# ArbiterMob/FluidSimulationCuda

Measured on AMD Instinct MI355X. Metric: Mcells/s per Jacobi iter, higher is better.
Workload: dtype f32

## Files before the change

fluidsimulationcuda_amd/capi.py:

```python
import ctypes as C
import os

import numpy as np

from ._build import LIB

OK, E_INVALID, E_NOMEM, E_HIP, E_COMM = 0, 1, 2, 3, 4
U, V, DENS, U_PREV, V_PREV, DENS_PREV, TMP0, TMP1, TMP2, TMP3, TMP4, TMP5 = range(12)
NFIELDS = 12
JACOBI_STREAM, JACOBI_LDS, JACOBI_NAIVE, JACOBI_TB = 0, 1, 2, 3
STORAGE_F32, STORAGE_F16 = 0, 1
PARAM_TB_MAX_SWEEPS, PARAM_TB_ROWS, PARAM_HALO, PARAM_TB_FAST_DIVISION, PARAM_TB_MIN_CELLS, PARAM_TB_EDGE_ROWS_PCT = 0, 1, 2, 3, 4, 5
PARAM_TB_LANE_COLUMNS = 6
PARAM_TB_T16_MIN_CELLS = 7
PARAM_TB_AUTOTUNE = 8
PARAM_FUSE_DIVERGENCE = 9
PARAM_SLAB_OVERLAP = 10
PARAM_EARLY_ADVECT = 11
PARAM_FUSE_ADD_SOURCE = 12
PARAM_XCHG_OVERLAP = 13
PARAM_F16_PRESSURE_SCALE = 14
PARAM_TB_FILL = 15
XCHG_HALO, XCHG_GATHER, XCHG_MAX, XCHG_MAX_BEGIN, XCHG_MAX_END = 0, 1, 2, 3, 4
RCCL_ID_BYTES = 128
FIELD_NAMES = ("u", "v", "dens", "u_prev", "v_prev", "dens_prev", "tmp0", "tmp1", "tmp2", "tmp3", "tmp4", "tmp5")


class FluidError(RuntimeError):
    def __init__(self, code, msg):
        super().__init__("libfluid_amd error %d: %s" % (code, msg))
        self.code = code


class Config(C.Structure):
    _fields_ = [("n", C.c_int), ("rank", C.c_int), ("nranks", C.c_int), ("halo", C.c_int),
                ("jacobi_variant", C.c_int), ("stream", C.c_void_p), ("arena", C.c_void_p),
                ("arena_bytes", C.c_size_t), ("storage", C.c_int)]


TIME_SOURCE, TIME_DIFFUSION, TIME_DIVERGENCE, TIME_PROJECTION, TIME_ADVECTION = range(5)
TIMING_CATEGORIES = ("source", "diffusion", "divergence", "projection", "advection")


class Timing(C.Structure):
    _fields_ = [("jacobi_ms", C.c_double), ("sweeps", C.c_longlong), ("solves", C.c_longlong),
                ("category_ms", C.c_double * 5), ("category_calls", C.c_longlong * 5),
                ("jacobi_launches", C.c_longlong), ("jacobi_field_launches", C.c_longlong),
                ("pressure_ms", C.c_double), ("pressure_sweeps", C.c_longlong)]


class RunPlan(C.Structure):
    _fields_ = [("iters", C.c_int), ("nsteps", C.c_int), ("use_sources", C.c_int), ("sources", C.c_void_p),
                ("every", C.c_int), ("fields", C.POINTER(C.c_int)), ("nfields", C.c_int),
                ("snapshots", C.c_void_p), ("capacity", C.c_size_t)]


EXCHANGE_FN = C.CFUNCTYPE(C.c_int, C.c_void_p, C.c_int, C.POINTER(C.c_int), C.c_int, C.c_int,
                          C.POINTER(C.c_float))

_HOSTF = np.ctypeslib.ndpointer(dtype=np.float32, flags="C_CONTIGUOUS")
_ctx = C.c_void_p
_i, _f = C.c_int, C.c_float
_MF = C.POINTER(C.c_float)

SIGNATURES = {
    "step": [_i, _f, _f, _f, _HOSTF, _HOSTF, _HOSTF],
    "step_src": [_i, _f, _f, _f, _i] + [_HOSTF] * 6,
    "fluid_release_cached": [],
    "fluid_coefficients": [_i, _f, _f, C.POINTER(_f), C.POINTER(_f)],
    "fluid_layout": [_i, C.POINTER(_i), C.POINTER(_i), C.POINTER(C.c_size_t)],
    "fluid_create": [_i, C.POINTER(_ctx)],
    "fluid_create_ex": [C.POINTER(Config), C.POINTER(_ctx)],
    "fluid_create_ensemble": [C.POINTER(Config), _i, C.POINTER(_ctx)],
    "fluid_members": [_ctx, C.POINTER(_i)],
    "fluid_upload_member": [_ctx, _i, _i, _HOSTF],
    "fluid_download_member": [_ctx, _i, _i, _HOSTF],
    "fluid_step_members": [_ctx, _MF, _MF, _MF, _i, _i, _i],
    "fluid_vel_step_members": [_ctx, _MF, _MF, _i],
    "fluid_dens_step_members": [_ctx, _MF, _MF, _i],
    "fluid_op_add_source_members": [_ctx, _i, _i, _MF],
    "fluid_op_jacobi_sweep_members": [_ctx, _i, _i, _i, _i, _MF, _MF],
    "fluid_op_diffuse_members": [_ctx, _i, _i, _i, _MF, _MF, _i],
    "fluid_op_advect_members": [_ctx, _i, _i, _i, _i, _i, _MF],
    "fluid_destroy": [_ctx],
    "fluid_synchronize": [_ctx],
    "fluid_owned_rows": [_ctx, C.POINTER(_i), C.POINTER(_i)],
    "fluid_field_ptr": [_ctx, _i, C.POINTER(C.c_void_p)],
    "fluid_scalar_ptr": [_ctx, C.POINTER(C.c_void_p)],
    "fluid_upload": [_ctx, _i, _HOSTF],
    "fluid_download": [_ctx, _i, _HOSTF],
    "fluid_upload_rows": [_ctx, _i, _HOSTF, _i, _i],
    "fluid_download_rows": [_ctx, _i, _HOSTF, _i, _i],
    "fluid_fill": [_ctx, _i, _f],
    "fluid_step": [_ctx, _f, _f, _f, _i, _i, _i],
    "fluid_vel_step": [_ctx, _f, _f, _i],
    "fluid_dens_step": [_ctx, _f, _f, _i],
    "fluid_op_set_bnd": [_ctx, _i, _i],
    "fluid_op_add_source": [_ctx, _i, _i, _f],
    "fluid_op_jacobi_sweep": [_ctx, _i, _i, _i, _i, _f, _f],
    "fluid_op_diffuse": [_ctx, _i, _i, _i, _f, _f, _i],
    "fluid_op_advect": [_ctx, _i, _i, _i, _i, _i, _f],
    "fluid_op_divergence": [_ctx, _i, _i, _i, _i],
    "fluid_op_subtract_gradient": [_ctx, _i, _i, _i],
    "fluid_residual": [_ctx, _i, _i, _f, _f, C.POINTER(_f)],
    "fluid_absmax_velocity": [_ctx, _i, _i, C.POINTER(_f)],
    "fluid_residual_members": [_ctx, _i, _i, _MF, _MF, _MF],
    "fluid_absmax_velocity_members": [_ctx, _i, _i, _MF],
    "fluid_member_moments": [_ctx, _i, C.POINTER(C.c_double), C.POINTER(C.c_double)],
    "fluid_ensemble_stats": [_ctx, _i, _MF, _MF],
    "fluid_ensemble_stats_ptr": [_ctx, C.POINTER(C.c_void_p), C.POINTER(C.c_void_p)],
    "fluid_pack_members": [_ctx, _i, _i, _i, C.c_void_p, C.c_size_t],
    "fluid_unpack_members": [_ctx, _i, _i, _i, C.c_void_p, C.c_size_t],
    "fluid_download_members": [_ctx, _i, _MF],
    "fluid_upload_members": [_ctx, _i, _MF],
    "fluid_run": [_ctx, _f, _f, _f, C.POINTER(RunPlan), C.POINTER(_i)],
    "fluid_run_members": [_ctx, _MF, _MF, _MF, C.POINTER(RunPlan), C.POINTER(_i)],
    "fluid_set_jacobi_variant": [_ctx, _i],
    "fluid_division_mode": [_ctx, _f, _f, C.POINTER(_i)],
    "fluid_autotune_pending": [_ctx, C.POINTER(_i)],
    "fluid_plan_sweeps": [_i, _i, _i, _i, _i, _i, _i, C.POINTER(_i), _i, C.POINTER(_i)],
    "fluid_set_param": [_ctx, _i, _i],
    "fluid_timing_enable": [_ctx, _i],
    "fluid_timing_read": [_ctx, C.POINTER(Timing), _i],
    "fluid_op_diffuse_tol": [_ctx, _i, _i, _i, _f, _f, _f, _i, _i, C.POINTER(_i), C.POINTER(_f)],
    "fluid_set_exchange": [_ctx, EXCHANGE_FN, C.c_void_p],
    "fluid_exchange_now": [_ctx, _i, C.POINTER(_i), _i, _i],
    "fluid_exchange_stream": [_ctx, C.POINTER(C.c_void_p)],
    "fluid_split_launches": [_ctx, C.POINTER(C.c_longlong)],
    "fluid_rccl_available": [],
    "fluid_rccl_unique_id": [C.c_void_p, C.c_size_t],
    "fluid_exchange_rccl_attach": [_ctx, C.c_void_p, C.c_size_t],
    "fluid_exchange_rccl_attach_comm": [_ctx, C.c_void_p],
    "fluid_exchange_rccl_detach": [_ctx],
    "fluid_exchange_rccl_calls": [_ctx, C.POINTER(C.c_longlong), C.POINTER(C.c_longlong), C.POINTER(C.c_longlong)],
}
OTHER_SYMBOLS = {"fluid_last_error": (C.c_char_p, []), "fluid_arena_bytes": (C.c_size_t, [_i]),
                 "fluid_arena_bytes_ex": (C.c_size_t, [_i, _i]),
                 "fluid_arena_bytes_ensemble": (C.c_size_t, [_i, _i, _i])}
MAX_MEMBERS = 21845

_lib = None


def lib():
    global _lib
    if _lib is None:
        if not os.path.exists(LIB):
            raise ImportError("%s not found: run `python -c 'import __graft_entry__ as g; g.build()'` "
                              "(hipcc --offload-arch=gfx950). There is no CPU fallback." % LIB)
        try:
            import torch
        except ImportError:
            pass
        L = C.CDLL(LIB)
        for name, args in SIGNATURES.items():
            fn = getattr(L, name)
            fn.restype, fn.argtypes = C.c_int, args
        for name, (res, args) in OTHER_SYMBOLS.items():
            fn = getattr(L, name)
            fn.restype, fn.argtypes = res, args
        _lib = L
    return _lib


def check(rc):
    if rc != OK:
        raise FluidError(rc, lib().fluid_last_error().decode(errors="replace"))
```

fluidsimulationcuda_amd/csrc/fluid_ctx.h:

```cpp
#pragma once
#include <hip/hip_runtime.h>

#include <string>
#include <utility>
#include <vector>

#include "../../include/fluid_amd.h"
#include "fluid_kernels.h"

namespace fluid_detail {
int fail(int code, const char* fmt, ...);
int materialize_zero(fluid_ctx* c, int f);
int refuse_ensemble(const fluid_ctx* c, const char* what);
struct RcclExchange;
void rccl_release(RcclExchange* x);
}

#define HIP_TRY(expr)                                                                                      \
    do {                                                                                                   \
        hipError_t e_ = (expr);                                                                            \
        if (e_ != hipSuccess)                                                                              \
            return fluid_detail::fail(e_ == hipErrorOutOfMemory ? FLUID_E_NOMEM : FLUID_E_HIP, "%s: %s",   \
                                      #expr, hipGetErrorString(e_));                                       \
    } while (0)

#define TRY(expr)                        \
    do {                                 \
        int rc_ = (expr);                \
        if (rc_ != FLUID_OK) return rc_; \
    } while (0)

class MemberVal {
    float s_;
    std::vector<float> v_;
    explicit MemberVal(std::vector<float>&& v) : s_(v[0]), v_(std::move(v)) {}

public:
    MemberVal(float v = 0.0f) : s_(v) {}
    MemberVal(const float* per_member, int members) : s_(per_member[0]), v_(per_member, per_member + members) {}
    bool uniform() const { return v_.empty(); }
    float at(int m) const { return v_.empty() ? s_ : v_[(size_t)m]; }
    const std::vector<float>& values() const { return v_; }
    bool operator==(const MemberVal& o) const { return s_ == o.s_ && v_ == o.v_; }
    template <class F>
    MemberVal map(const MemberVal& b, F f) const
    {
        if (uniform() && b.uniform()) return MemberVal(f(s_, b.s_));
        std::vector<float> r(uniform() ? b.v_.size() : v_.size());
        for (size_t m = 0; m < r.size(); ++m) r[m] = f(at((int)m), b.at((int)m));
        return MemberVal(std::move(r));
    }
    template <class F>
    MemberVal map(F f) const { return map(MemberVal(), [&](float x, float) { return f(x); }); }
};

struct FieldState {
    void* ptr = nullptr;
    int reach = 0;
    bool zero = false;
    bool pend = false;
    MemberVal pend_inc;
    int src_of = 0;
    MemberVal src_dt;
    float fscale = 1.0f;
};

struct ConstRing {
    char *dev = nullptr, *host = nullptr;
    size_t bytes = 0, head = 0;
    struct Blob { size_t off, len; unsigned long long hash; hipEvent_t copied; };
    std::vector<Blob> live;
    std::vector<hipEvent_t> free_events;
};

struct EnsembleReduce {
    unsigned int* d_max = nullptr;
    double2* d_moments = nullptr;
    double2* d_partials = nullptr;
    char* host = nullptr;
    float *d_mean = nullptr, *d_var = nullptr;
    bool have_stats = false;
};

struct MemberStage {
    float* dev = nullptr;
    int members = 0;
};

struct fluid_ctx {
    int n = 0, w = 0, pitch = 0;
    size_t field_floats = 0;
    int members = 1;
    char* arena = nullptr;
    bool own_arena = false;
    int st = fluid::STORAGE_F32;
    size_t esz = 4;
    hipStream_t stream = nullptr;
    bool own_stream = false;
    hipStream_t stream2 = nullptr;
    hipEvent_t ev_fork = nullptr, ev_join = nullptr;
    bool slab_overlap = true;
    hipStream_t xstream = nullptr;
    hipEvent_t ev_xbegin = nullptr, ev_xdone = nullptr;
    bool xchg_overlap = true;
    unsigned xowed = 0;
    long long split_launches = 0;
    bool early_advect = true;
    float vmax_prev[2] = {-1.0f, -1.0f};
    FieldState field[FLUID_NFIELDS];
    size_t field_bytes = 0;
    unsigned int* d_scalar = nullptr;
    float* d_partials = nullptr;
    ConstRing consts;
    EnsembleReduce red;
    MemberStage stage;
    unsigned int* tiles = nullptr;
    unsigned int* h_scalar = nullptr;
    hipEvent_t scalar_ready = nullptr;
    int variant = fluid::JACOBI_TB;
    int tb_max_t = 16, tb_rows = 0, num_cu = 256;
    long long tb_min_cells = 0;
    long long tb_t16_min_cells = -1;
    bool fuse_divergence = true;
    bool tb_fill = true;
    bool autotune = true;
    struct Trial { unsigned long long key; int cand; hipEvent_t a, b; };
    std::vector<Trial> trials;
    std::vector<hipEvent_t> free_events;
    bool defer_zero_source = true;
    bool in_halo_exchange = false;
    int tb_nv = 2;
    int tb_edge_pct = 40;
    int fast_div = 2;
    int rank = 0, nranks = 1, own0 = 1, own1 = 1, min_slab = 0, halo = 1;
    bool fuse_add_source = true;
    float pscale = 1.0f;
    fluid_exchange_fn xchg = nullptr;
    void* xchg_user = nullptr;
    fluid_detail::RcclExchange* rccl = nullptr;
    bool timing = false;
    struct Ev { hipEvent_t a, b; int cat; bool pressure; };
    std::vector<Ev> ev_pool;
    size_t ev_used = 0;
    double cat_ms[FLUID_TIMING_CATEGORIES] = {};
    long long cat_calls[FLUID_TIMING_CATEGORIES] = {};
    long long sweeps = 0, pending_sweeps = 0, launches = 0, field_launches = 0;
    double pressure_ms = 0.0;
    long long pressure_sweeps = 0, pending_pressure_sweeps = 0;
    bool in_pressure_solve = false;

    bool valid_field(int id) const { return id >= 0 && id < FLUID_NFIELDS; }
    void* ptr(int id) const { return field[id].ptr; }
    fluid::Members mb() const { return {members, field_floats}; }
    size_t all_bytes() const { return field_bytes * (size_t)members; }
    void* row(int id, int r) const { return static_cast<char*>(ptr(id)) + (size_t)r * pitch * esz; }
    int lo_all() const { return own0 - (rank == 0 ? 1 : 0); }
    int hi_all() const { return own1 + (rank == nranks - 1 ? 1 : 0); }
};
```

fluidsimulationcuda_amd/csrc/fluid_kernels.h:

```cpp
#pragma once
#include <hip/hip_runtime.h>

namespace fluid {

constexpr int XOFF = 63;

enum JacobiVariant { JACOBI_STREAM = 0, JACOBI_LDS = 1, JACOBI_NAIVE = 2, JACOBI_TB = 3, JACOBI_VARIANTS = 4 };

enum Storage { STORAGE_F32 = 0, STORAGE_F16 = 1 };
typedef _Float16 half_t;
inline size_t storage_bytes(int st) { return st == STORAGE_F16 ? 2 : 4; }

inline int pitch_for(int n) { return ((XOFF + 1 + 4 * ((n + 3) / 4) + 1) + 63) / 64 * 64; }

struct Members {
    int count = 1;
    size_t stride = 0;
};

struct TbMemberK {
    double yd;
    float alpha, beta, hi, lo;
    float x0_inc, div_scale;
    unsigned tile_thr, pad;
};

struct TbBatch {
    const void* x[3];
    const void* x0[3];
    void* out[3];
    float alpha[3], beta[3];
    double yd[3];
    float hi[3], lo[3];
    const unsigned* tiles[3];
    unsigned tile_thr[3];
    int tile_pitch;
    void* div[3];
    float div_scale;
    int b[3];
    int x_zero[3];
    float x0_inc[3];
    int count;
    int members;
    size_t mstride;
    size_t tile_mstride;
    const TbMemberK* mk;
};

void launch_set_bnd(hipStream_t s, int st, void* f, int pitch, int n, int b, Members mb = {});
void launch_add_source(hipStream_t s, int st, void* x, const void* src, int pitch, int row_lo, int row_hi, float dt, Members mb = {},
                       const float* mdt = nullptr);
void launch_jacobi(hipStream_t s, int st, int variant, const void* x, const void* x0, void* out, int pitch, int n,
                   int row_lo, int row_hi, float alpha, float beta, int b, Members mb = {}, const float2* mab = nullptr);
enum TbForm { TB_PLAIN = 0, TB_DIVSRC = 1, TB_ADDSRC = 2 };
struct TbShape { int T, divmode, nv, form; };
inline constexpr TbShape kTbShapes[] = {
    {2, 0, 2, TB_PLAIN},   {2, 2, 2, TB_PLAIN},   {2, 3, 2, TB_PLAIN},   {2, 4, 2, TB_PLAIN},   {2, 5, 2, TB_PLAIN},
    {2, 0, 4, TB_PLAIN},   {2, 2, 4, TB_PLAIN},   {2, 3, 4, TB_PLAIN},   {2, 4, 4, TB_PLAIN},   {2, 5, 4, TB_PLAIN},
    {4, 0, 2, TB_PLAIN},   {4, 2, 2, TB_PLAIN},   {4, 3, 2, TB_PLAIN},   {4, 4, 2, TB_PLAIN},   {4, 5, 2, TB_PLAIN},
    {4, 0, 4, TB_PLAIN},   {4, 2, 4, TB_PLAIN},   {4, 3, 4, TB_PLAIN},   {4, 4, 4, TB_PLAIN},   {4, 5, 4, TB_PLAIN},
    {8, 0, 2, TB_PLAIN},   {8, 2, 2, TB_PLAIN},   {8, 3, 2, TB_PLAIN},   {8, 4, 2, TB_PLAIN},   {8, 5, 2, TB_PLAIN},
    {8, 0, 4, TB_PLAIN},   {8, 2, 4, TB_PLAIN},   {8, 3, 4, TB_PLAIN},   {8, 4, 4, TB_PLAIN},   {8, 5, 4, TB_PLAIN},
    {12, 0, 2, TB_PLAIN},  {12, 2, 2, TB_PLAIN},  {12, 3, 2, TB_PLAIN},  {12, 4, 2, TB_PLAIN},  {12, 5, 2, TB_PLAIN},
    {16, 0, 2, TB_PLAIN},  {16, 2, 2, TB_PLAIN},  {16, 3, 2, TB_PLAIN},  {16, 4, 2, TB_PLAIN},  {16, 5, 2, TB_PLAIN},
    {8, 4, 2, TB_DIVSRC},  {12, 4, 2, TB_DIVSRC}, {16, 4, 2, TB_DIVSRC}, {8, 0, 2, TB_ADDSRC},  {8, 2, 2, TB_ADDSRC},  {8, 5, 2, TB_ADDSRC},
    {12, 0, 2, TB_ADDSRC}, {12, 2, 2, TB_ADDSRC}, {12, 5, 2, TB_ADDSRC}, {16, 0, 2, TB_ADDSRC}, {16, 2, 2, TB_ADDSRC}, {16, 5, 2, TB_ADDSRC},
};
constexpr int kTbShapeCount = sizeof(kTbShapes) / sizeof(kTbShapes[0]);
constexpr int jacobi_tb_index(int T, int divmode, int nv, int form)
{
    for (int i = 0; i < kTbShapeCount; ++i) {
        const TbShape& s = kTbShapes[i];
        if ((T < 0 || s.T == T) && (divmode < 0 || s.divmode == divmode) && s.nv == nv && s.form == form) return i;
    }
    return -1;
}
constexpr bool jacobi_tb_exists(int T, int divmode, int nv, int form) { return jacobi_tb_index(T, divmode, nv, form) >= 0; }
constexpr bool tb_shapes_unique(int i = 0)
{
    return i == kTbShapeCount || (jacobi_tb_index(kTbShapes[i].T, kTbShapes[i].divmode, kTbShapes[i].nv, kTbShapes[i].form) == i && tb_shapes_unique(i + 1));
}
static_assert(kTbShapeCount == 52 && tb_shapes_unique(), "52 distinct shapes: adding or removing one is a change of this table");
inline constexpr int kTbDepths[] = {16, 12, 8, 4, 2};
constexpr bool is_tb_depth(int T) { for (int d : kTbDepths) if (d == T) return true; return false; }
bool launch_jacobi_tb(hipStream_t s, int st, int T, int divmode, int nv, int form, const TbBatch& batch, int pitch, int n, int row_lo,
                      int row_hi, int rb, int rb_edge, int hole_lo = 0, int hole_hi = 0, bool fill = true);
constexpr int kTileRows = 32, kTileCols = 64;
inline int tile_rows(int n) { return (n + kTileRows - 1) / kTileRows; }
inline int tile_pitch(int n) { return (n + kTileCols - 1) / kTileCols; }
struct TileBatch {
    const void* field[3];
    unsigned* tiles[3];
    int count;
    size_t mstride, tile_mstride;
};
void launch_tile_min_abs(hipStream_t s, int st, const TileBatch& tb, int count, int pitch, int n, int row_lo, int row_hi, int tile_pitch,
                         Members mb = {}, size_t tile_mstride = 0);
void launch_validate_div(hipStream_t s, int divmode, float beta, float kbeta, double yd, float hi, float lo, unsigned long long* bad);
void launch_advect(hipStream_t s, int st, void* d, const void* d0, const void* u, const void* v, int pitch, int n,
                   int row_lo, int row_hi, float dt0, int b, Members mb = {}, const float* mdt0 = nullptr);
void launch_advect2(hipStream_t s, int st, void* da, const void* d0a, int ba, void* db, const void* d0b, int bb, const void* u,
                    const void* v, int pitch, int n, int row_lo, int row_hi, float dt0, Members mb = {}, const float* mdt0 = nullptr);
void launch_divergence(hipStream_t s, int st, const void* u, const void* v, void* p, void* div, int pitch, int n,
                       int row_lo, int row_hi, float h, int write_p, float pscale = 1.0f, Members mb = {});
void launch_scale(hipStream_t s, int st, void* x, int pitch, int row_lo, int row_hi, float factor, Members mb = {});
constexpr int kMaxPartials = 8192;
void launch_subtract_gradient(hipStream_t s, int st, void* u, void* v, const void* p, int pitch, int n, int row_lo,
                              int row_hi, float h, float* partials = nullptr, unsigned int* max_out = nullptr, float pinv = 1.0f,
                              Members mb = {});
void launch_gradient_advect(hipStream_t s, int st, void* u, void* v, const void* p, void* d, const void* d0, int pitch, int n,
                            int row_lo, int row_hi, float h, float dt0, int b, float pinv = 1.0f, Members mb = {},
                            const float* mdt0 = nullptr);
void launch_absmax2(hipStream_t s, int st, const void* u, const void* v, int pitch, int n, int row_lo, int row_hi,
                    unsigned int* result, Members mb = {}, int rstride = 0);
void launch_residual(hipStream_t s, int st, const void* x, const void* x0, int pitch, int n, int row_lo, int row_hi,
                     float alpha, float beta, unsigned int* result, Members mb = {}, int rstride = 0, const float2* mab = nullptr);
constexpr int kMomentBlocks = 4096;
int moment_blocks(int n, int members);
void launch_member_moments(hipStream_t s, int st, const void* x, int pitch, int n, Members mb, double2* partials, double2* out);
void launch_ensemble_stats(hipStream_t s, int st, const void* x, int pitch, int n, Members mb, float* mean, float* var);
void launch_pack_members(hipStream_t s, int st, const void* x, int pitch, int n, Members mb, float inv, float* dense, size_t dstride);
void launch_unpack_members(hipStream_t s, int st, void* x, int pitch, int n, Members mb, const float* dense, size_t dstride);

}
```

fluidsimulationcuda_amd/csrc/fluid_kernels.hip:

```cpp
#include <hip/hip_runtime.h>
#include <stdint.h>

#include <algorithm>
#include <array>
#include <cstdlib>
#include <utility>

#include "fluid_kernels.h"

namespace fluid {

__device__ __forceinline__ float flip_if(bool c, float v) { return c ? -v : v; }

__device__ __forceinline__ float keep_f32(float v) { asm("" : "+v"(v)); return v; }
__device__ __forceinline__ float ld1(const float* p) { return *p; }
__device__ __forceinline__ float ld1(const half_t* p) { return keep_f32((float)*p); }
__device__ __forceinline__ void st1(float* p, float v) { *p = v; }
__device__ __forceinline__ void st1(half_t* p, float v) { *p = (half_t)keep_f32(v); }
template <typename S>
__device__ __forceinline__ float as_stored(float v)
{
    if constexpr (sizeof(S) == 2) return keep_f32((float)(S)keep_f32(v));
    else return v;
}
typedef half_t half4_t __attribute__((ext_vector_type(4)));
__device__ __forceinline__ float4 ld4(const float* p) { return *reinterpret_cast<const float4*>(p); }
__device__ __forceinline__ float4 ld4(const half_t* p)
{
    const half4_t h = *reinterpret_cast<const half4_t*>(p);
    return make_float4(keep_f32((float)h.x), keep_f32((float)h.y), keep_f32((float)h.z), keep_f32((float)h.w));
}
__device__ __forceinline__ void st4(float* p, const float4& v) { *reinterpret_cast<float4*>(p) = v; }
__device__ __forceinline__ void st4(half_t* p, const float4& v)
{
    half4_t h;
    h.x = (half_t)keep_f32(v.x); h.y = (half_t)keep_f32(v.y); h.z = (half_t)keep_f32(v.z); h.w = (half_t)keep_f32(v.w);
    *reinterpret_cast<half4_t*>(p) = h;
}

constexpr unsigned kBufOff = 0x80000000u;
typedef unsigned uint4_t __attribute__((ext_vector_type(4)));
typedef unsigned uint2_t __attribute__((ext_vector_type(2)));

__device__ __forceinline__ float from_lane_below(float v, float edge)
{
    int r = __builtin_amdgcn_update_dpp(__float_as_int(edge), __float_as_int(v),
                                        0x138 , 0xf, 0xf, false);
    return __int_as_float(r);
}
__device__ __forceinline__ float from_lane_above(float v, float edge)
{
    int r = __builtin_amdgcn_update_dpp(__float_as_int(edge), __float_as_int(v),
                                        0x130 , 0xf, 0xf, false);
    return __int_as_float(r);
}

__device__ __forceinline__ float lane_below0(float v)
{
    return __int_as_float(__builtin_amdgcn_update_dpp(0, __float_as_int(v), 0x138, 0xf, 0xf, true));
}
__device__ __forceinline__ float lane_above0(float v)
{
    return __int_as_float(__builtin_amdgcn_update_dpp(0, __float_as_int(v), 0x130, 0xf, 0xf, true));
}

template <typename S>
__device__ __forceinline__ void emit_ghosts(S* __restrict__ f, size_t pitch, int n, int b, int j, int i, float val)
{
    const bool nx = (b == 1), ny = (b == 2);
    const bool left = (j == 1), right = (j == n), top = (i == 1), bot = (i == n);
    if (!(left | right | top | bot)) return;
    const float gx = flip_if(nx, val);
    const float gy = flip_if(ny, val);
    const float corner = 0.5f * (gy + gx);
    S* r0 = f + XOFF;
    S* ri = f + (size_t)i * pitch + XOFF;
    S* rn = f + (size_t)(n + 1) * pitch + XOFF;
    if (left) st1(ri, gx);
    if (right) st1(ri + n + 1, gx);
    if (top) st1(r0 + j, gy);
    if (bot) st1(rn + j, gy);
    if (top & left) st1(r0, corner);
    if (top & right) st1(r0 + n + 1, corner);
    if (bot & left) st1(rn, corner);
    if (bot & right) st1(rn + n + 1, corner);
}

template <typename S>
__global__ __launch_bounds__(256) void k_set_bnd(S* __restrict__ f, int pitch, int n, int b, size_t ms)
{
    const int k = 1 + blockIdx.x * 256 + threadIdx.x;
    if (k > n) return;
    f += blockIdx.y * ms;
    const size_t P = (size_t)pitch;
    const bool nx = (b == 1), ny = (b == 2);
    S* r0 = f + XOFF;
    S* rk = f + (size_t)k * P + XOFF;
    S* r1 = f + P + XOFF;
    S* rN = f + (size_t)n * P + XOFF;
    S* rn = f + (size_t)(n + 1) * P + XOFF;
    const float gl = flip_if(nx, ld1(rk + 1));
    const float gr = flip_if(nx, ld1(rk + n));
    const float gt = flip_if(ny, ld1(r1 + k));
    const float gb = flip_if(ny, ld1(rN + k));
    st1(rk, gl);
    st1(rk + n + 1, gr);
    st1(r0 + k, gt);
    st1(rn + k, gb);
    if (k == 1) {
        st1(r0, 0.5f * (gt + gl));
        st1(rn, 0.5f * (gb + flip_if(nx, ld1(rN + 1))));
    }
    if (k == n) {
        st1(r0 + n + 1, 0.5f * (gt + flip_if(nx, ld1(r1 + n))));
        st1(rn + n + 1, 0.5f * (gb + gr));
    }
}

template <typename S>
__global__ __launch_bounds__(256) void k_add_source(S* __restrict__ x, const S* __restrict__ s, int pitch, int row_lo,
                                                    int row_hi, float dt, size_t ms, const float* __restrict__ mdt)
{
    if (mdt) dt = mdt[blockIdx.y];
    const int nvec = pitch >> 2;
    const size_t total = (size_t)(row_hi - row_lo) * nvec;
    S* xv = x + blockIdx.y * ms + (size_t)row_lo * pitch;
    const S* sv = s + blockIdx.y * ms + (size_t)row_lo * pitch;
    for (size_t t = (size_t)blockIdx.x * 256 + threadIdx.x; t < total; t += (size_t)gridDim.x * 256) {
        float4 a = ld4(xv + 4 * t);
        const float4 c = ld4(sv + 4 * t);
        a.x = a.x + dt * c.x;
        a.y = a.y + dt * c.y;
        a.z = a.z + dt * c.z;
        a.w = a.w + dt * c.w;
        st4(xv + 4 * t, a);
    }
}

template <typename S>
__global__ __launch_bounds__(256) void k_add_zero_source(S* __restrict__ x, int pitch, int row_lo, int row_hi, float inc, size_t ms,
                                                         const float* __restrict__ minc)
{
    if (minc) inc = minc[blockIdx.y];
    const int nvec = pitch >> 2;
    const size_t total = (size_t)(row_hi - row_lo) * nvec;
    S* xv = x + blockIdx.y * ms + (size_t)row_lo * pitch;
    for (size_t t = (size_t)blockIdx.x * 256 + threadIdx.x; t < total; t += (size_t)gridDim.x * 256) {
        float4 a = ld4(xv + 4 * t);
        a.x = a.x + inc;
        a.y = a.y + inc;
        a.z = a.z + inc;
        a.w = a.w + inc;
        st4(xv + 4 * t, a);
    }
}

template <typename S>
__global__ __launch_bounds__(256) void k_scale(S* __restrict__ x, int pitch, int row_lo, int row_hi, float factor, size_t ms)
{
    const int nvec = pitch >> 2;
    const size_t total = (size_t)(row_hi - row_lo) * nvec;
    S* xv = x + blockIdx.y * ms + (size_t)row_lo * pitch;
    for (size_t t = (size_t)blockIdx.x * 256 + threadIdx.x; t < total; t += (size_t)gridDim.x * 256) {
        float4 a = ld4(xv + 4 * t);
        a.x = a.x * factor;
        a.y = a.y * factor;
        a.z = a.z * factor;
        a.w = a.w * factor;
        st4(xv + 4 * t, a);
    }
}


template <typename S>
__global__ __launch_bounds__(256) void k_jacobi_naive(const S* __restrict__ x, const S* __restrict__ x0,
// ... 164 lines not shown
        const uint4_t u = __builtin_amdgcn_raw_buffer_load_b128(r, off, 0, 0);
        v.c[0] = __uint_as_float(u.x); v.c[1] = __uint_as_float(u.y); v.c[2] = __uint_as_float(u.z); v.c[3] = __uint_as_float(u.w);
    } else {
        const uint2_t u = __builtin_amdgcn_raw_buffer_load_b64(r, off, 0, 0);
        v.c[0] = __uint_as_float(u.x); v.c[1] = __uint_as_float(u.y);
    }
    return v;
}
template <int NV>
__device__ __forceinline__ Vec<NV> buf_ldv(const half_t*, __amdgpu_buffer_rsrc_t r, unsigned off)
{
    Vec<NV> v;
    if constexpr (NV == 4) {
        const uint2_t u = __builtin_amdgcn_raw_buffer_load_b64(r, off, 0, 0);
        half4_t h;
        __builtin_memcpy(&h, &u, 8);
        v.c[0] = keep_f32((float)h.x); v.c[1] = keep_f32((float)h.y); v.c[2] = keep_f32((float)h.z); v.c[3] = keep_f32((float)h.w);
    } else {
        const unsigned u = __builtin_amdgcn_raw_buffer_load_b32(r, off, 0, 0);
        half2_t h;
        __builtin_memcpy(&h, &u, 4);
        v.c[0] = keep_f32((float)h.x); v.c[1] = keep_f32((float)h.y);
    }
    return v;
}
template <int NV>
__device__ __forceinline__ void buf_stv(float*, __amdgpu_buffer_rsrc_t r, unsigned off, const Vec<NV>& v)
{
    if constexpr (NV == 4) {
        uint4_t u;
        u.x = __float_as_uint(v.c[0]); u.y = __float_as_uint(v.c[1]); u.z = __float_as_uint(v.c[2]); u.w = __float_as_uint(v.c[3]);
        __builtin_amdgcn_raw_buffer_store_b128(u, r, off, 0, 0);
    } else {
        uint2_t u;
        u.x = __float_as_uint(v.c[0]); u.y = __float_as_uint(v.c[1]);
        __builtin_amdgcn_raw_buffer_store_b64(u, r, off, 0, 0);
    }
}
template <int NV>
__device__ __forceinline__ void buf_stv(half_t*, __amdgpu_buffer_rsrc_t r, unsigned off, const Vec<NV>& v)
{
    if constexpr (NV == 4) {
        half4_t h;
        h.x = (half_t)keep_f32(v.c[0]); h.y = (half_t)keep_f32(v.c[1]); h.z = (half_t)keep_f32(v.c[2]); h.w = (half_t)keep_f32(v.c[3]);
        uint2_t u;
        __builtin_memcpy(&u, &h, 8);
        __builtin_amdgcn_raw_buffer_store_b64(u, r, off, 0, 0);
    } else {
        half2_t h;
        h.x = (half_t)keep_f32(v.c[0]); h.y = (half_t)keep_f32(v.c[1]);
        unsigned u;
        __builtin_memcpy(&u, &h, 4);
        __builtin_amdgcn_raw_buffer_store_b32(u, r, off, 0, 0);
    }
}

struct DivK {
    float beta;
    double yd;
    float hi, lo;
};
constexpr float kDiv5NegScale = -0x1p24f;

template <typename S, int NV>
struct TbArgs {
    const S* xc;
    const S* rc;
    S* oc;
    __amdgpu_buffer_rsrc_t bx, br, bo;
    unsigned ld_off;
    unsigned st_off;
    unsigned row_bytes;
    unsigned m_lg;
    unsigned m_r[NV];
    int n, q_lo, q_hi, cg;
    float alpha;
    DivK k;
    S* dc;
    __amdgpu_buffer_rsrc_t bd;
    float div_scale;
    int s_lo, s_hi;
    unsigned sx, sy;
    float x0_inc;
    bool st_rg_lane, is_lg;
    bool fill;
};

__device__ __forceinline__ float fxor(float v, unsigned m) { return __uint_as_float(__float_as_uint(v) ^ m); }
template <int NV>
__device__ __forceinline__ Vec<NV> fxorv(const Vec<NV>& v, unsigned m)
{
    Vec<NV> o;
#pragma unroll
    for (int c = 0; c < NV; ++c) o.c[c] = fxor(v.c[c], m);
    return o;
}

template <int DIVMODE>
__device__ __forceinline__ float tb_div(float num, const DivK& k)
{
    if (DIVMODE == 0) return num / k.beta;
    if (DIVMODE == 4) return num * k.beta;
    if (DIVMODE == 3) return __builtin_fmaf(num, k.hi, num * k.lo);
    if (DIVMODE == 5) {
        const float q0 = num * k.beta;
        const float e = __builtin_fmaf(q0, k.hi, num * kDiv5NegScale);
        return __builtin_fmaf(e, k.lo, q0);
    }
    return (float)((double)num * k.yd);
}
template <int DIVMODE>
__device__ __forceinline__ v2f tb_div2(v2f num, const DivK& k)
{
    if constexpr (DIVMODE == 4) return num * k.beta;
    else if constexpr (DIVMODE == 3) {
        const v2f p = num * k.lo;
        return __builtin_elementwise_fma(num, (v2f){k.hi, k.hi}, p);
    } else if constexpr (DIVMODE == 5) {
        const v2f ds = num * kDiv5NegScale;
        const v2f q0 = num * k.beta;
        const v2f e = __builtin_elementwise_fma(q0, (v2f){k.hi, k.hi}, ds);
        return __builtin_elementwise_fma(e, (v2f){k.lo, k.lo}, q0);
    } else return (v2f){tb_div<DIVMODE>(num.x, k), tb_div<DIVMODE>(num.y, k)};
}

template <int DIVMODE, int NV>
__device__ __forceinline__ Vec<NV> tb_stencil(const Vec<NV>& up, const Vec<NV>& me, const Vec<NV>& dn, const Vec<NV>& r,
                                              float alpha, const DivK& k)
{
    float h[NV];
    h[0] = lane_below0(me.c[NV - 1]) + me.c[1];
#pragma unroll
    for (int c = 1; c < NV - 1; ++c) h[c] = me.c[c - 1] + me.c[c + 1];
    h[NV - 1] = me.c[NV - 2] + lane_above0(me.c[0]);
    Vec<NV> G;
#pragma unroll
    for (int p = 0; p < NV; p += 2) {
        v2f s = {h[p], h[p + 1]};
        s = s + (v2f){up.c[p], up.c[p + 1]};
        s = s + (v2f){dn.c[p], dn.c[p + 1]};
        if constexpr (DIVMODE != 4) s = s * alpha;
        s = (v2f){r.c[p], r.c[p + 1]} + s;
        s = tb_div2<DIVMODE>(s, k);
        G.c[p] = s.x;
        G.c[p + 1] = s.y;
    }
    return G;
}

template <int DIVMODE>
__global__ __launch_bounds__(256) void k_validate_div(float beta, DivK k, unsigned long long* __restrict__ bad)
{
    unsigned long long n = 0;
    const unsigned long long stride = (unsigned long long)gridDim.x * 256;
    auto differs = [](float got, float ref) { return (ref != ref) ? !(got != got) : (__float_as_uint(got) != __float_as_uint(ref)); };
    DivK k2 = k;
    for (unsigned long long i = (unsigned long long)blockIdx.x * 256 + threadIdx.x; i < (1ull << 32); i += stride) {
        const float a = __uint_as_float((unsigned)i);
        const float ref = a / beta;
        if constexpr (DIVMODE == 3) {
            const bool in_range = a == 0.0f || !(__builtin_fabsf(a) < beta * 0x1p-98f);
            n += differs(tb_div<2>(a, k2), ref) || (in_range && differs(tb_div<3>(a, k), ref));
        } else if constexpr (DIVMODE == 5) {
            const float got = tb_div<5>(a, k);
            const bool finite = __builtin_fabsf(got) < __builtin_inff();
            const bool must_be_exact = __builtin_fabsf(a) < 0x1p100f;
            n += differs(got, ref) && (finite || must_be_exact);
        } else {
            n += differs(tb_div<DIVMODE>(a, k), ref);
        }
    }
    if (n) atomicAdd(bad, n);
}

__device__ __forceinline__ float bitsel(unsigned mask, float a, float b)
{
    return __uint_as_float((__float_as_uint(a) & mask) | (__float_as_uint(b) & ~mask));
}

template <typename S, int NV>
__device__ __forceinline__ void tb_fix_columns(Vec<NV>& G, const TbArgs<S, NV>& a, float& v1, float& vn, bool need_corners)
{
    float o[NV];
#pragma unroll
    for (int c = 0; c < NV; ++c) o[c] = G.c[c];
    const float from_right = lane_above0(o[0]);
    const float from_left = lane_below0(o[NV - 1]);
    G.c[0] = bitsel(a.m_r[0], fxor(from_left, a.sx), o[0]);
#pragma unroll
    for (int c = 1; c < NV - 1; ++c) G.c[c] = bitsel(a.m_r[c], fxor(o[c - 1], a.sx), o[c]);
    G.c[NV - 1] = bitsel(a.m_lg, fxor(from_right, a.sx), bitsel(a.m_r[NV - 1], fxor(o[NV - 2], a.sx), o[NV - 1]));
    if (need_corners) {
        v1 = from_right;
        unsigned bits = __float_as_uint(from_left) & a.m_r[0];
#pragma unroll
        for (int c = 1; c < NV; ++c) bits |= __float_as_uint(o[c - 1]) & a.m_r[c];
        vn = __uint_as_float(bits);
    }
}

template <bool EDGE, bool WALL, typename S, int NV>
__device__ __forceinline__ void tb_store_to(S* oc, __amdgpu_buffer_rsrc_t bo, const Vec<NV>& G, int q, bool mine, const TbArgs<S, NV>& a,
                                            float v1, float vn)
{
    auto on = [](bool c, unsigned off) { return c ? off : kBufOff; };
    buf_stv<NV>(oc, bo, on(mine, a.st_off) + (unsigned)q * a.row_bytes, G);
    if (WALL) {
        Vec<NV> g = fxorv<NV>(G, a.sy);
        if (EDGE) {
            const float cl = 0.5f * (fxor(v1, a.sy) + fxor(v1, a.sx));
            const float cr = 0.5f * (fxor(vn, a.sy) + fxor(vn, a.sx));
            if (a.is_lg) g.c[NV - 1] = cl;
#pragma unroll
            for (int c = 0; c < NV; ++c)
                if (a.st_rg_lane && a.cg == c) g.c[c] = cr;
        }
        buf_stv<NV>(oc, bo, on(mine & (q == 1), a.st_off), g);
        buf_stv<NV>(oc, bo, on(mine & (q == a.n), a.st_off) + (unsigned)(a.n + 1) * a.row_bytes, g);
    }
}
template <bool EDGE, bool WALL, typename S, int NV>
__device__ __forceinline__ void tb_store(const Vec<NV>& G, int q, bool mine, const TbArgs<S, NV>& a, float v1, float vn)
{
    tb_store_to<EDGE, WALL, S, NV>(a.oc, a.bo, G, q, mine, a, v1, vn);
}

template <int NV>
__device__ __forceinline__ Vec<NV> tb_divergence(const Vec<NV>& u, const Vec<NV>& v_up, const Vec<NV>& v_dn, float scale)
{
    float g[NV];
#pragma unroll
    for (int c = 0; c < NV; ++c) {
        const float ur = c < NV - 1 ? u.c[c + 1] : lane_above0(u.c[0]);
        const float ul = c > 0 ? u.c[c - 1] : lane_below0(u.c[NV - 1]);
        g[c] = ur - ul;
    }
    Vec<NV> d;
#pragma unroll
    for (int p = 0; p < NV; p += 2) {
        v2f s = {g[p], g[p + 1]};
        s = s + (v2f){v_dn.c[p], v_dn.c[p + 1]};
        s = s - (v2f){v_up.c[p], v_up.c[p + 1]};
        s = s * scale;
        d.c[p] = s.x;
        d.c[p + 1] = s.y;
    }
    return d;
}

template <int NV>
__device__ __forceinline__ Vec<NV> take(const Vec<NV>& v)
{
    Vec<NV> o;
#pragma unroll
    for (int p = 0; p < NV; p += 2) {
        v2f in = {v.c[p], v.c[p + 1]}, out;
        asm("v_mov_b64 %0, %1" : "=v"(out) : "v"(in));
        o.c[p] = out.x;
        o.c[p + 1] = out.y;
    }
    return o;
}

template <int K, int N, int NV>
__device__ __forceinline__ void tb_qshift(Vec<NV> (&Q)[N])
{
    if constexpr (K >= 1) {
        Q[K] = Q[K - 1];
        tb_qshift<K - 1, N, NV>(Q);
    }
}

template <int DIVMODE, int NV>
__device__ __forceinline__ void tb_sticky(const Vec<NV>& G, v2f& nf)
{
    if constexpr (DIVMODE == 5) {
#pragma unroll
        for (int p = 0; p < NV; p += 2) nf = __builtin_elementwise_fma((v2f){G.c[p], G.c[p + 1]}, (v2f){0.f, 0.f}, nf);
    }
}

template <int T, int DIVMODE, bool EDGE, bool WALL, bool GEN, int PH, typename S, int NV, bool DIVSRC = false, bool ADDSRC = false,
          bool PART = false>
__device__ __forceinline__ void tb_step(int t, Vec<NV> (&W)[T][3], Vec<NV> (&Q)[T + 1], Vec<NV> (&PX)[3], Vec<NV> (&PQ)[3],
                                        const TbArgs<S, NV>& a, Vec<NV> (&UR)[3], Vec<NV> (&VR)[3], v2f& nf, int smax = T)
{
    static_assert(!(PART && GEN), "the general body runs every stage");
    constexpr int UP = PH % 3, ME = (PH + 1) % 3, FR = (PH + 2) % 3;
    __builtin_amdgcn_sched_barrier(0);
    if constexpr (DIVSRC) {
        UR[FR] = take<NV>(PX[PH]);
        VR[FR] = take<NV>(PQ[PH]);
    } else {
        W[0][FR] = take<NV>(PX[PH]);
        Q[0] = take<NV>(PQ[PH]);
        if constexpr (ADDSRC) {
#pragma unroll
            for (int p = 0; p < NV; p += 2) {
                const v2f ds = (v2f){W[0][FR].c[p], W[0][FR].c[p + 1]} * a.div_scale;
                const v2f q = (v2f){Q[0].c[p], Q[0].c[p + 1]} + ds;
                Q[0].c[p] = as_stored<S>(q.x);
                Q[0].c[p + 1] = as_stored<S>(q.y);
            }
            buf_stv<NV>(a.dc, a.bd, (((t >= a.s_lo) & (t < a.s_hi)) ? a.st_off : kBufOff) + (unsigned)t * a.row_bytes, Q[0]);
        } else {
#pragma unroll
            for (int p = 0; p < NV; p += 2) {
                const v2f q = (v2f){Q[0].c[p], Q[0].c[p + 1]} + a.x0_inc;
                Q[0].c[p] = q.x;
                Q[0].c[p + 1] = q.y;
            }
        }
    }
    {
        const unsigned off = a.ld_off + (unsigned)(t + 3) * a.row_bytes;
        PX[PH] = buf_ldv<NV>(a.xc, a.bx, off);
        PQ[PH] = buf_ldv<NV>(a.rc, a.br, off);
    }
    __builtin_amdgcn_sched_barrier(0);
    if constexpr (DIVSRC) {
        const int q = t - 1;
        Vec<NV> D = tb_divergence<NV>(UR[ME], VR[UP], VR[FR], a.div_scale);
#pragma unroll
        for (int c = 0; c < NV; ++c) D.c[c] = as_stored<S>(D.c[c]);
        Q[1] = D;
        float v1 = 0.f, vn = 0.f;
        if (EDGE) tb_fix_columns<S, NV>(D, a, v1, vn, WALL);
        tb_store_to<EDGE, (WALL || GEN), S, NV>(a.dc, a.bd, D, q, (q >= 1) & (q <= a.n) & (q >= a.q_lo) & (q < a.q_hi), a, v1, vn);
    }
    if constexpr (!GEN) {
#pragma unroll
        for (int s = 1; s <= T; ++s) {
            const bool run = !PART || s <= smax;
            const int q = t - s;
            Vec<NV> G;
            float v1 = 0.f, vn = 0.f;
            if (run) {
                G = tb_stencil<DIVMODE, NV>(W[s - 1][UP], W[s - 1][ME], W[s - 1][FR], Q[s], a.alpha, a.k);
                if (EDGE) tb_fix_columns<S, NV>(G, a, v1, vn, WALL && s == T);
                if (s == T) tb_sticky<DIVMODE, NV>(G, nf);
            } else {
#pragma unroll
                for (int c = 0; c < NV; ++c) G.c[c] = __builtin_nondeterministic_value(W[s - 1][FR].c[c]);
            }
            if (s < T) W[s][FR] = G;
            else tb_store<EDGE, WALL, S, NV>(G, q, run & (q >= a.q_lo) & (q < a.q_hi), a, v1, vn);
        }
    } else {
#pragma unroll
        for (int s = 1; s <= T; ++s) {
            const int q = t - s;
            const bool interior = (q >= 1 && q <= a.n);
            Vec<NV> G = tb_stencil<DIVMODE, NV>(W[s - 1][UP], W[s - 1][ME], W[s - 1][FR], Q[s], a.alpha, a.k);
            float v1 = 0.f, vn = 0.f;
            if (EDGE) tb_fix_columns<S, NV>(G, a, v1, vn, s == T);
            if (s < T) {
                const Vec<NV> me = W[s][ME];
                const Vec<NV> flipped_me = fxorv<NV>(me, a.sy);
                const Vec<NV> flipped_g = fxorv<NV>(G, a.sy);
                const bool bot_ghost = (q == a.n + 1), top_ghost = (q == 1);
#pragma unroll
                for (int c = 0; c < NV; ++c) {
                    W[s][FR].c[c] = bot_ghost ? flipped_me.c[c] : G.c[c];
                    W[s][ME].c[c] = top_ghost ? flipped_g.c[c] : me.c[c];
                }
            } else {
                tb_sticky<DIVMODE, NV>(G, nf);
                tb_store<EDGE, true, S, NV>(G, q, interior & (q >= a.q_lo) & (q < a.q_hi), a, v1, vn);
            }
        }
    }
    tb_qshift<T, T + 1, NV>(Q);
}

template <int T, int DIVMODE, bool EDGE, bool WALL, typename S, int NV, bool DIVSRC = false, bool ADDSRC = false>
__device__ __forceinline__ bool tb_march(int t0, int t1, const TbArgs<S, NV>& a)
{
    Vec<NV> W[T][3], Q[T + 1], PX[3], PQ[3], UR[3], VR[3];
    v2f nf = {0.f, 0.f};
    Vec<NV> zero;
#pragma unroll
    for (int c = 0; c < NV; ++c) zero.c[c] = 0.f;
#pragma unroll
    for (int s = 0; s < T; ++s) { W[s][0] = zero; W[s][1] = zero; W[s][2] = zero; }
#pragma unroll
    for (int s = 0; s <= T; ++s) Q[s] = zero;
#pragma unroll
    for (int d = 0; d < 3; ++d) { UR[d] = zero; VR[d] = zero; }
#pragma unroll
    for (int d = 0; d < 3; ++d) {
        const unsigned off = a.ld_off + (unsigned)(t0 + d) * a.row_bytes;
        PX[d] = buf_ldv<NV>(a.xc, a.bx, off);
        PQ[d] = buf_ldv<NV>(a.rc, a.br, off);
        buf_stv<NV>(a.oc, a.bo, kBufOff, zero);
        if constexpr (DIVSRC || ADDSRC) buf_stv<NV>(a.dc, a.bd, kBufOff, zero);
        __builtin_amdgcn_sched_barrier(0);
    }
    int t = t0;
    if constexpr (WALL) {
        for (; t <= t1 && t < T + 1; t += 3) {
            tb_step<T, DIVMODE, EDGE, WALL, true, 0, S, NV, DIVSRC, ADDSRC>(t, W, Q, PX, PQ, a, UR, VR, nf);
            tb_step<T, DIVMODE, EDGE, WALL, true, 1, S, NV, DIVSRC, ADDSRC>(t + 1, W, Q, PX, PQ, a, UR, VR, nf);
            tb_step<T, DIVMODE, EDGE, WALL, true, 2, S, NV, DIVSRC, ADDSRC>(t + 2, W, Q, PX, PQ, a, UR, VR, nf);
        }
    }
    const int fill_end = (a.fill && t0 == a.q_lo - T) ? t0 + 3 * ((2 * T + 2) / 3) : t0;
    const int full_end = a.fill ? t1 - 2 : t1;
    auto stages = [&](int u) { return u > t1 ? 0 : u < fill_end ? (u - t0) >> 1 : T; };
    for (; t <= t1 && t < fill_end && (!WALL || t + 1 <= a.n); t += 3) {
        tb_step<T, DIVMODE, EDGE, WALL, false, 0, S, NV, DIVSRC, ADDSRC, true>(t, W, Q, PX, PQ, a, UR, VR, nf, stages(t));
        tb_step<T, DIVMODE, EDGE, WALL, false, 1, S, NV, DIVSRC, ADDSRC, true>(t + 1, W, Q, PX, PQ, a, UR, VR, nf, stages(t + 1));
        tb_step<T, DIVMODE, EDGE, WALL, false, 2, S, NV, DIVSRC, ADDSRC, true>(t + 2, W, Q, PX, PQ, a, UR, VR, nf, stages(t + 2));
    }
    for (; t <= full_end && (!WALL || t + 1 <= a.n); t += 3) {
        tb_step<T, DIVMODE, EDGE, WALL, false, 0, S, NV, DIVSRC, ADDSRC>(t, W, Q, PX, PQ, a, UR, VR, nf);
        tb_step<T, DIVMODE, EDGE, WALL, false, 1, S, NV, DIVSRC, ADDSRC>(t + 1, W, Q, PX, PQ, a, UR, VR, nf);
        tb_step<T, DIVMODE, EDGE, WALL, false, 2, S, NV, DIVSRC, ADDSRC>(t + 2, W, Q, PX, PQ, a, UR, VR, nf);
    }
    for (; t <= t1 && (!WALL || t + 1 <= a.n); t += 3) {
        tb_step<T, DIVMODE, EDGE, WALL, false, 0, S, NV, DIVSRC, ADDSRC, true>(t, W, Q, PX, PQ, a, UR, VR, nf, stages(t));
        tb_step<T, DIVMODE, EDGE, WALL, false, 1, S, NV, DIVSRC, ADDSRC, true>(t + 1, W, Q, PX, PQ, a, UR, VR, nf, stages(t + 1));
        tb_step<T, DIVMODE, EDGE, WALL, false, 2, S, NV, DIVSRC, ADDSRC, true>(t + 2, W, Q, PX, PQ, a, UR, VR, nf, stages(t + 2));
    }
    if constexpr (WALL) {
        for (; t <= t1; t += 3) {
            tb_step<T, DIVMODE, EDGE, WALL, true, 0, S, NV, DIVSRC, ADDSRC>(t, W, Q, PX, PQ, a, UR, VR, nf);
            tb_step<T, DIVMODE, EDGE, WALL, true, 1, S, NV, DIVSRC, ADDSRC>(t + 1, W, Q, PX, PQ, a, UR, VR, nf);
            tb_step<T, DIVMODE, EDGE, WALL, true, 2, S, NV, DIVSRC, ADDSRC>(t + 2, W, Q, PX, PQ, a, UR, VR, nf);
        }
    }
    if constexpr (DIVMODE == 5) return __builtin_amdgcn_ballot_w64((nf.x != nf.x) | (nf.y != nf.y)) != 0ull;
    else return false;
}

template <int T, int DIVMODE, typename S, int NV, bool DIVSRC = false, bool ADDSRC = false>
__device__ __forceinline__ bool tb_march_any(bool edge, bool wall, int t0, int t1, const TbArgs<S, NV>& a)
{
    if (edge) {
        if (wall) return tb_march<T, DIVMODE, true, true, S, NV, DIVSRC, ADDSRC>(t0, t1, a);
        return tb_march<T, DIVMODE, true, false, S, NV, DIVSRC, ADDSRC>(t0, t1, a);
    }
    if (wall) return tb_march<T, DIVMODE, false, true, S, NV, DIVSRC, ADDSRC>(t0, t1, a);
    return tb_march<T, DIVMODE, false, false, S, NV, DIVSRC, ADDSRC>(t0, t1, a);
}

struct TbGrid {
    int inner_wins, inner_blocks, edge_wins, edge_blocks, first_right;
    int hole_lo, hole_hi;
};

constexpr int tb_waves_per_simd(int T, int NV) { return NV == 2 ? (T <= 8 ? 4 : T <= 12 ? 3 : 2) : (T <= 4 ? 3 : 2); }

template <int T, int DIVMODE, int NV, typename S, bool DIVSRC = false, bool ADDSRC = false>
__global__ __launch_bounds__(256, tb_waves_per_simd(T, NV)) void k_jacobi_tb(TbBatch batch, int pitch, int n, int row_lo,
                                                                             int row_hi, int rb, int rb_edge, TbGrid g, int fill)
{
    static_assert(!DIVSRC || DIVMODE == 4, "the divergence-sourced launch is the first launch of a pressure solve");
    static_assert(!(DIVSRC && ADDSRC) && (!ADDSRC || DIVMODE != 3), "one second store per launch; mode 3's tiles are taken from the summed field");
    const unsigned per_xcd = gridDim.x >> 3;
    unsigned vid = (blockIdx.x & 7u) * per_xcd + (blockIdx.x >> 3);
    if (vid >= (unsigned)(g.inner_blocks + g.edge_blocks)) return;
    int win, strip_group;
    if (vid < (unsigned)g.inner_blocks) {
        win = 1 + (int)(vid % (unsigned)g.inner_wins);
        strip_group = (int)(vid / (unsigned)g.inner_wins);
    } else {
        vid -= (unsigned)g.inner_blocks;
        const int e = (int)(vid % (unsigned)g.edge_wins);
        strip_group = (int)(vid / (unsigned)g.edge_wins);
        win = e == 0 ? 0 : g.first_right + e - 1;
    }
    const unsigned member = batch.count == 3 ? blockIdx.z / 3u : batch.count == 2 ? blockIdx.z >> 1 : blockIdx.z;
    const unsigned sv = blockIdx.z - member * (unsigned)batch.count;
    const size_t mofs = (size_t)member * batch.mstride;
    const S* __restrict__ x = static_cast<const S*>(batch.x[sv]) + mofs;
    const S* __restrict__ x0 = static_cast<const S*>(batch.x0[sv]) + mofs;
    S* __restrict__ out = static_cast<S*>(batch.out[sv]) + mofs;
    float alpha = batch.alpha[sv], beta = batch.beta[sv];
    double yd = batch.yd[sv];
    float k_hi = batch.hi[sv], k_lo = batch.lo[sv], x0_inc = batch.x0_inc[sv], div_scale = batch.div_scale;
    unsigned tile_thr = batch.tile_thr[sv];
    if (batch.mk != nullptr) {
        typedef const TbMemberK __attribute__((address_space(4))) * MemberKPtr;
        const MemberKPtr mk = (MemberKPtr)(uintptr_t)batch.mk + ((size_t)sv * (unsigned)batch.members + member);
        alpha = mk->alpha;
        beta = mk->beta;
        yd = mk->yd;
        k_hi = mk->hi;
        k_lo = mk->lo;
        x0_inc = mk->x0_inc;
        if (ADDSRC) div_scale = mk->div_scale;
        if (DIVMODE == 3) tile_thr = mk->tile_thr;
    }
    const int b = batch.b[sv];
    constexpr int HL = (T + NV - 1) / NV;
    constexpr int VS = 64 - 2 * HL;
    constexpr int C0 = (XOFF + 1) / NV;
    static_assert((XOFF + 1) % NV == 0 && HL <= C0, "window overlap must fit the row's left pad");
    const int lane = threadIdx.x & 63;
    const int strip = strip_group * 4 + __builtin_amdgcn_readfirstlane(threadIdx.x >> 6);
    const int kg = n / NV;
    const bool left_edge = (win == 0);
    const bool right_edge = (kg >= win * VS - HL) && (kg < win * VS - HL + 64);
    const bool edge = left_edge || right_edge;
    const int rbw = edge ? rb_edge : rb;
    TbArgs<S, NV> a;
    a.k.yd = yd;
    a.k.lo = k_lo;
    a.k.hi = k_hi;
    a.x0_inc = x0_inc;
    int seg_hi = row_hi;
    a.q_lo = row_lo + strip * rbw;
    if (g.hole_lo < g.hole_hi) {
        const int top = (g.hole_lo - row_lo + rbw - 1) / rbw;
        if (strip < top) seg_hi = g.hole_lo;
        else a.q_lo = g.hole_hi + (strip - top) * rbw;
    }
    if (a.q_lo >= seg_hi) return;
    a.q_hi = min(a.q_lo + rbw, seg_hi);
    a.s_lo = a.q_lo == 1 ? 0 : a.q_lo;
    a.s_hi = a.q_hi == n + 1 ? n + 2 : a.q_hi;
    const int k = win * VS - HL + lane;
    const int nvec = (n + NV - 1) / NV;
    const bool ld_ok = k <= pitch / NV - C0 - 1;
    const ptrdiff_t cofs = (ptrdiff_t)(XOFF + 1) + NV * (ptrdiff_t)(ld_ok ? k : 0);
    a.xc = x + cofs;
    a.rc = x0 + cofs;
    a.oc = out + cofs;
    {
        const unsigned field_bytes = (unsigned)((size_t)(n + 2) * (size_t)pitch * sizeof(S));
        a.bx = __builtin_amdgcn_make_buffer_rsrc(const_cast<S*>(x), 0, (batch.x_zero[sv] && !DIVSRC) ? 0u : field_bytes, 0x00020000);
        a.br = __builtin_amdgcn_make_buffer_rsrc(const_cast<S*>(x0), 0, field_bytes, 0x00020000);
        a.bo = __builtin_amdgcn_make_buffer_rsrc(out, 0, field_bytes, 0x00020000);
        S* dv = (DIVSRC || ADDSRC) ? static_cast<S*>(batch.div[sv]) + mofs : out;
        a.dc = dv + cofs;
        a.bd = __builtin_amdgcn_make_buffer_rsrc(dv, 0, field_bytes, 0x00020000);
        a.div_scale = div_scale;
        a.row_bytes = (unsigned)((size_t)pitch * sizeof(S));
        const unsigned col = (unsigned)((XOFF + 1 + NV * (ptrdiff_t)k) * (ptrdiff_t)sizeof(S));
        a.ld_off = ld_ok ? col : kBufOff;
    }
    a.n = n;
    a.cg = n % NV;
    a.is_lg = (k == -1);
    const bool is_rg = (k == kg);
    const bool own = (lane >= HL) && (lane < 64 - HL);
    const bool st_int = own && k >= 0 && k < nvec;
    a.st_rg_lane = is_rg && (own || k == nvec);
    a.m_lg = a.is_lg ? 0xFFFFFFFFu : 0u;
#pragma unroll
    for (int c = 0; c < NV; ++c) a.m_r[c] = (is_rg && a.cg == c) ? 0xFFFFFFFFu : 0u;
    a.st_off = (ld_ok && (st_int || a.is_lg || a.st_rg_lane)) ? a.ld_off : kBufOff;
    a.sx = (b == 1) ? 0x80000000u : 0u;
    a.sy = (b == 2) ? 0x80000000u : 0u;
    a.alpha = alpha;
    a.k.beta = beta;
    a.fill = fill != 0;
    const int t0 = max(0, a.q_lo - T), t1 = a.q_hi - 1 + T;
    const bool wall = (a.q_lo < T) || (a.q_hi - 1 + T > n + 1);
    constexpr int DM = DIVMODE == 3 ? 2 : DIVMODE;
    bool two_term = false;
    if constexpr (DIVMODE == 3) {
        const unsigned* __restrict__ tiles = batch.tiles[sv] ? batch.tiles[sv] + (size_t)member * batch.tile_mstride : nullptr;
        const unsigned thr = tile_thr;
        const int tr0 = (max(1, a.q_lo - T + 1) - 1) / kTileRows, tr1 = (min(n, a.q_hi + T - 2) - 1) / kTileRows;
        const int c0 = max(1, 1 + NV * (win * VS - HL)), c1 = min(n, NV * (win * VS - HL + 64));
        const int tc0 = (c0 - 1) / kTileCols, tc1 = (c1 - 1) / kTileCols, ntc = tc1 - tc0 + 1;
        const int count = (tr1 - tr0 + 1) * ntc;
        bool low = false;
        if (tiles != nullptr)
            for (int i = lane; i < count; i += 64)
                low |= tiles[(size_t)(tr0 + i / ntc) * batch.tile_pitch + (tc0 + i % ntc)] < thr;
        two_term = tiles != nullptr && __builtin_amdgcn_ballot_w64(low) == 0ull;
    }
    if (two_term) {
        tb_march_any<T, DIVMODE, S, NV>(edge, wall, t0, t1, a);
    } else {
        const bool again = tb_march_any<T, DM, S, NV, DIVSRC, ADDSRC>(edge, wall, t0, t1, a);
        if constexpr (DIVMODE == 5) {
            if (again) tb_march_any<T, 2, S, NV, false, ADDSRC>(edge, wall, t0, t1, a);
        }
    }
}

template <typename S>
__global__ __launch_bounds__(256) void k_tile_min_abs(TileBatch tb, int pitch, int n, int row_lo, int row_hi, int tile_row0, int tile_pitch)
{
    const unsigned member = blockIdx.z / (unsigned)tb.count, sv = blockIdx.z - member * (unsigned)tb.count;
    const S* __restrict__ f = static_cast<const S*>(tb.field[sv]) + (size_t)member * tb.mstride;
    unsigned* __restrict__ out = tb.tiles[sv] + (size_t)member * tb.tile_mstride;
    const int lane = threadIdx.x & 63, wave = threadIdx.x >> 6;
    const int tr = tile_row0 + blockIdx.y;
    const int j = 1 + 4 * (lane + 64 * (blockIdx.x * 4 + wave));
    const int i0 = max(row_lo, 1 + tr * kTileRows), i1 = min(row_hi, 1 + (tr + 1) * kTileRows);
    const size_t P = (size_t)pitch;
    float m = __builtin_inff();
    if (j <= n)
        for (int i = i0; i < i1; ++i) {
            const float4 v = ld4(f + (size_t)i * P + XOFF + j);
            m = fminf(m, fabsf(v.x));
            if (j + 1 <= n) m = fminf(m, fabsf(v.y));
            if (j + 2 <= n) m = fminf(m, fabsf(v.z));
            if (j + 3 <= n) m = fminf(m, fabsf(v.w));
        }
#pragma unroll
    for (int off = 8; off > 0; off >>= 1) m = fminf(m, __shfl_xor(m, off, 16));
    const bool whole = row_lo <= 1 + tr * kTileRows && row_hi >= min(n + 1, 1 + (tr + 1) * kTileRows);
    if ((lane & 15) == 0 && j <= n) out[(size_t)tr * tile_pitch + (j - 1) / kTileCols] = whole ? __float_as_uint(m) : 0u;
}

template <typename S, typename IDX>
__device__ __forceinline__ const S* at(const S* base, IDX byte_off) { return reinterpret_cast<const S*>(reinterpret_cast<const char*>(base) + byte_off); }
template <typename S, typename IDX>
__device__ __forceinline__ S* at(S* base, IDX byte_off) { return reinterpret_cast<S*>(reinterpret_cast<char*>(base) + byte_off); }

template <typename IDX>
struct AdvectTap {
    IDX o;
    float s0, s1, t0, t1;
};

template <typename IDX>
__device__ __forceinline__ AdvectTap<IDX> advect_trace(int j, int i, float uu, float vv, float dt0, int n, IDX P, IDX E)
{
    float px = (float)j - dt0 * uu;
    float py = (float)i - dt0 * vv;
    const float hi = (float)n + 0.5f;
    px = __builtin_fminf(__builtin_fmaxf(px, 0.5f), hi);
    py = __builtin_fminf(__builtin_fmaxf(py, 0.5f), hi);
    const int j0 = (int)px, i0 = (int)py;
    AdvectTap<IDX> t;
    t.s1 = px - (float)j0;
    t.s0 = 1.0f - t.s1;
    t.t1 = py - (float)i0;
    t.t0 = 1.0f - t.t1;
    t.o = (IDX)i0 * P + (IDX)(XOFF + j0) * E;
    return t;
}

struct __attribute__((packed, aligned(4))) FloatPair { float a, b; };
__device__ __forceinline__ void ld_pair(const float* p, float& a, float& b)
{
    const FloatPair v = *reinterpret_cast<const FloatPair*>(p);
    a = v.a;
    b = v.b;
}
__device__ __forceinline__ void ld_pair(const half_t* p, float& a, float& b)
{
    a = ld1(p);
    b = ld1(p + 1);
}

template <typename S, typename IDX>
__device__ __forceinline__ float advect_sample(const S* __restrict__ d0, IDX P, const AdvectTap<IDX>& t)
{
    float q00, q10, q01, q11;
    ld_pair(at(d0, t.o), q00, q10);
    ld_pair(at(d0, t.o + P), q01, q11);
    const float a = t.t0 * q00 + t.t1 * q01;
    const float e = t.t0 * q10 + t.t1 * q11;
    return t.s0 * a + t.s1 * e;
// ... 484 lines not shown
            f[0] = a.x; f[1] = a.y; f[2] = a.z; f[3] = a.w;
        } else {
            typedef half_t half8_t __attribute__((ext_vector_type(8)));
            const half8_t h = *reinterpret_cast<const half8_t*>(x + at);
#pragma unroll
            for (int e = 0; e < VW; ++e) f[e] = keep_f32((float)h[e]) * inv;
        }
#pragma unroll
        for (int e = 0; e < VW; e += 4) {
            dense4_t d;
            d.x = f[e]; d.y = f[e + 1]; d.z = f[e + 2]; d.w = f[e + 3];
            *reinterpret_cast<dense4_t*>(dense + (I)(dat + (I)e)) = d;
        }
    } else {
#pragma unroll
        for (int e = 0; e < VW; ++e)
            if ((valid >> e) & 1) {
                if constexpr (sizeof(S) == 4) dense[(I)(dat + (I)e)] = x[(I)(at + (I)e)];
                else dense[(I)(dat + (I)e)] = ld1(x + (I)(at + (I)e)) * inv;
            }
    }
}

template <typename S, typename I>
__global__ __launch_bounds__(256) void k_unpack_members(S* __restrict__ x, int pitch, int n, size_t ms, int vecs,
                                                        const float* __restrict__ dense, size_t dstride)
{
    constexpr int VW = StatsVec<S>::VW;
    I at, dat;
    int valid;
    if (!member_vector<S, I>(pitch, n, vecs, &at, &dat, &valid)) return;
    x += blockIdx.y * ms;
    dense += blockIdx.y * dstride;
    if (valid == (1 << VW) - 1) {
        float f[VW];
#pragma unroll
        for (int e = 0; e < VW; e += 4) {
            const dense4_t d = *reinterpret_cast<const dense4_t*>(dense + (I)(dat + (I)e));
            f[e] = d.x; f[e + 1] = d.y; f[e + 2] = d.z; f[e + 3] = d.w;
        }
        if constexpr (sizeof(S) == 4) {
            *reinterpret_cast<float4*>(x + at) = make_float4(f[0], f[1], f[2], f[3]);
        } else {
            typedef half_t half8_t __attribute__((ext_vector_type(8)));
            half8_t h;
#pragma unroll
            for (int e = 0; e < VW; ++e) h[e] = (half_t)keep_f32(f[e]);
            *reinterpret_cast<half8_t*>(x + at) = h;
        }
    } else {
#pragma unroll
        for (int e = 0; e < VW; ++e)
            if ((valid >> e) & 1) st1(x + (I)(at + (I)e), dense[(I)(dat + (I)e)]);
    }
}

static inline unsigned cdiv(unsigned a, unsigned b) { return (a + b - 1) / b; }

static inline bool narrow_index(int st, int pitch, int n) { return (size_t)(n + 2) * (size_t)pitch * storage_bytes(st) < (1ull << 32); }

#define FLUID_BY_STORAGE(st, ...)             \
    do {                                      \
        if ((st) == STORAGE_F16) {            \
            using S = half_t;                 \
            __VA_ARGS__;                      \
        } else {                              \
            using S = float;                  \
            __VA_ARGS__;                      \
        }                                     \
    } while (0)
#define FLUID_BY_STORAGE_INDEX(st, pitch, n, ...)                                                  \
    do {                                                                                           \
        if (narrow_index(st, pitch, n)) { using I = unsigned; FLUID_BY_STORAGE(st, __VA_ARGS__); } \
        else { using I = size_t; FLUID_BY_STORAGE(st, __VA_ARGS__); }                              \
    } while (0)

static inline unsigned stride_blocks(int pitch, int row_lo, int row_hi)
{
    return (unsigned)std::clamp<size_t>(((size_t)(row_hi - row_lo) * (pitch >> 2) + 255) / 256, 1, 8192);
}

void launch_set_bnd(hipStream_t s, int st, void* f, int pitch, int n, int b, Members mb)
{
    FLUID_BY_STORAGE(st, hipLaunchKernelGGL(k_set_bnd<S>, dim3(cdiv(n, 256), mb.count), dim3(256), 0, s, (S*)f, pitch, n, b, mb.stride));
}

void launch_add_source(hipStream_t s, int st, void* x, const void* src, int pitch, int row_lo, int row_hi, float dt, Members mb,
                       const float* mdt)
{
    const dim3 grid(stride_blocks(pitch, row_lo, row_hi), mb.count);
    if (!src) {
        FLUID_BY_STORAGE(st, hipLaunchKernelGGL(k_add_zero_source<S>, grid, dim3(256), 0, s, (S*)x, pitch, row_lo, row_hi, dt, mb.stride, mdt));
        return;
    }
    FLUID_BY_STORAGE(st, hipLaunchKernelGGL(k_add_source<S>, grid, dim3(256), 0, s, (S*)x, (const S*)src, pitch, row_lo, row_hi, dt, mb.stride,
                                            mdt));
}

void launch_scale(hipStream_t s, int st, void* x, int pitch, int row_lo, int row_hi, float factor, Members mb)
{
    FLUID_BY_STORAGE(st, hipLaunchKernelGGL(k_scale<S>, dim3(stride_blocks(pitch, row_lo, row_hi), mb.count), dim3(256), 0, s, (S*)x, pitch,
                                            row_lo, row_hi, factor, mb.stride));
}

void launch_jacobi(hipStream_t s, int st, int variant, const void* x, const void* x0, void* out, int pitch, int n,
                   int row_lo, int row_hi, float alpha, float beta, int b, Members mb, const float2* mab)
{
    const int rows = row_hi - row_lo;
    if (rows <= 0) return;
    switch (variant) {
    case JACOBI_NAIVE:
        FLUID_BY_STORAGE(st, hipLaunchKernelGGL(k_jacobi_naive<S>, dim3(cdiv(n, 64), cdiv(rows, 4), mb.count), dim3(256), 0, s,
                                                (const S*)x, (const S*)x0, (S*)out, pitch, n, row_lo, row_hi, alpha,
                                                beta, b, mb.stride, mab));
        break;
    case JACOBI_LDS:
        FLUID_BY_STORAGE(st, hipLaunchKernelGGL(k_jacobi_lds<S>, dim3(cdiv(n, LT_X), cdiv(rows, LT_Y), mb.count), dim3(256), 0, s,
                                                (const S*)x, (const S*)x0, (S*)out, pitch, n, row_lo, row_hi, alpha,
                                                beta, b, mb.stride, mab));
        break;
    default: {
        constexpr int RB = 8;
        const unsigned nvec = (n + 3) / 4;
        FLUID_BY_STORAGE(st, hipLaunchKernelGGL((k_jacobi_stream<RB, S>), dim3(cdiv(nvec, 256), cdiv(rows, RB), mb.count), dim3(256),
                                                0, s, (const S*)x, (const S*)x0, (S*)out, pitch, n, row_lo, row_hi,
                                                alpha, beta, b, mb.stride, mab));
    }
    }
}

using TbKernel = void (*)(TbBatch, int, int, int, int, int, int, TbGrid, int);
template <typename S, size_t... I>
static std::array<TbKernel, kTbShapeCount> tb_kernels(std::index_sequence<I...>)
{
    return {&k_jacobi_tb<kTbShapes[I].T, kTbShapes[I].divmode, kTbShapes[I].nv, S, kTbShapes[I].form == TB_DIVSRC,
                         kTbShapes[I].form == TB_ADDSRC>...};
}

bool launch_jacobi_tb(hipStream_t s, int st, int T, int divmode, int nv, int form, const TbBatch& batch, int pitch, int n, int row_lo,
                      int row_hi, int rb, int rb_edge, int hole_lo, int hole_hi, bool fill)
{
    static const auto f32 = tb_kernels<float>(std::make_index_sequence<kTbShapeCount>());
    static const auto f16 = tb_kernels<half_t>(std::make_index_sequence<kTbShapeCount>());
    const int shape = jacobi_tb_index(T, divmode, nv, form);
    if (shape < 0) return false;
    const int rows = row_hi - row_lo;
    if (rows <= 0 || batch.count <= 0 || batch.members <= 0) return true;
    if (hole_lo < row_lo) hole_lo = row_lo;
    if (hole_hi > row_hi) hole_hi = row_hi;
    const bool hole = hole_lo < hole_hi;
    if (hole && hole_lo == row_lo && hole_hi == row_hi) return true;
    const int HL = (T + nv - 1) / nv, VS = 64 - 2 * HL;
    const unsigned nvec = (n + nv - 1) / nv;
    rb_edge = rb_edge < 1 ? rb : (rb_edge > rb ? rb : rb_edge);
    const int nwin = (int)cdiv(nvec, VS), kg = n / nv;
    int first_right = nwin - 1;
    while (first_right > 1 && kg < (first_right - 1) * VS - HL + 64) --first_right;
    if (first_right < 1) first_right = 1;
    TbGrid g;
    g.first_right = first_right;
    g.inner_wins = first_right - 1;
    g.edge_wins = 1 + (nwin - first_right);
    auto strips = [&](int r) { return hole ? cdiv(hole_lo - row_lo, r) + cdiv(row_hi - hole_hi, r) : cdiv(rows, r); };
    g.hole_lo = hole ? hole_lo : 0;
    g.hole_hi = hole ? hole_hi : 0;
    g.inner_blocks = g.inner_wins * (int)cdiv(strips(rb), 4);
    g.edge_blocks = g.edge_wins * (int)cdiv(strips(rb_edge), 4);
    const dim3 grid(8 * cdiv(g.inner_blocks + g.edge_blocks, 8), 1, batch.count * batch.members), block(256);
    const TbKernel k = (st == STORAGE_F16 ? f16 : f32)[shape];
    hipLaunchKernelGGL(k, grid, block, 0, s, batch, pitch, n, row_lo, row_hi, rb, rb_edge, g, fill ? 1 : 0);
    return true;
}

void launch_tile_min_abs(hipStream_t s, int st, const TileBatch& tiles, int count, int pitch, int n, int row_lo, int row_hi, int tile_pitch,
                         Members mb, size_t tile_mstride)
{
    if (row_lo < 1) row_lo = 1;
    if (row_hi > n + 1) row_hi = n + 1;
    if (row_hi <= row_lo || count <= 0) return;
    const int tr0 = (row_lo - 1) / kTileRows, tr1 = (row_hi - 2) / kTileRows;
    const dim3 grid(cdiv(cdiv(n, 4), 256), tr1 - tr0 + 1, count * mb.count);
    TileBatch tb = tiles;
    tb.count = count;
    tb.mstride = mb.stride;
    tb.tile_mstride = tile_mstride;
    FLUID_BY_STORAGE(st, hipLaunchKernelGGL(k_tile_min_abs<S>, grid, dim3(256), 0, s, tb, pitch, n, row_lo, row_hi, tr0, tile_pitch));
}

void launch_validate_div(hipStream_t s, int divmode, float beta, float kbeta, double yd, float hi, float lo, unsigned long long* bad)
{
    DivK k;
    k.beta = kbeta;
    k.yd = yd;
    k.hi = hi;
    k.lo = lo;
    const auto f = divmode == 4 ? k_validate_div<4> : divmode == 5 ? k_validate_div<5> : divmode == 3 ? k_validate_div<3> : k_validate_div<2>;
    hipLaunchKernelGGL(f, dim3(8192), dim3(256), 0, s, beta, k, bad);
}

void launch_advect(hipStream_t s, int st, void* d, const void* d0, const void* u, const void* v, int pitch, int n,
                   int row_lo, int row_hi, float dt0, int b, Members mb, const float* mdt0)
{
    if (row_hi <= row_lo) return;
    const dim3 grid(cdiv(n, 1024), row_hi - row_lo, mb.count);
    FLUID_BY_STORAGE_INDEX(st, pitch, n, hipLaunchKernelGGL((k_advect<S, I>), grid, dim3(256), 0, s, (S*)d, (const S*)d0, (const S*)u,
                                                            (const S*)v, pitch, n, row_lo, row_hi, dt0, b, mb.stride, mdt0));
}

void launch_advect2(hipStream_t s, int st, void* da, const void* d0a, int ba, void* db, const void* d0b, int bb, const void* u,
                    const void* v, int pitch, int n, int row_lo, int row_hi, float dt0, Members mb, const float* mdt0)
{
    if (row_hi <= row_lo) return;
    const dim3 grid(cdiv(n, 1024), row_hi - row_lo, mb.count);
    FLUID_BY_STORAGE_INDEX(st, pitch, n, hipLaunchKernelGGL((k_advect2<S, I>), grid, dim3(256), 0, s, (S*)da, (const S*)d0a, ba, (S*)db,
                                                            (const S*)d0b, bb, (const S*)u, (const S*)v, pitch, n, row_lo, row_hi, dt0, mb.stride,
                                                            mdt0));
}

void launch_divergence(hipStream_t s, int st, const void* u, const void* v, void* p, void* div, int pitch, int n,
                       int row_lo, int row_hi, float h, int write_p, float pscale, Members mb)
{
    if (row_hi <= row_lo) return;
    FLUID_BY_STORAGE(st, hipLaunchKernelGGL(k_divergence<S>, dim3(cdiv(n, 256), row_hi - row_lo, mb.count), dim3(256), 0, s,
                                            (const S*)u, (const S*)v, (S*)p, (S*)div, pitch, n, row_lo, row_hi, h,
                                            write_p, pscale, mb.stride));
}

void launch_subtract_gradient(hipStream_t s, int st, void* u, void* v, const void* p, int pitch, int n, int row_lo,
                              int row_hi, float h, float* partials, unsigned int* max_out, float pinv, Members mb)
{
    if (row_hi <= row_lo) return;
    if (max_out && mb.count == 1) {
        const unsigned per_col = cdiv(n, 256), rows = (unsigned)(row_hi - row_lo);
        const unsigned gy = std::max(1u, std::min(rows, (unsigned)kMaxPartials / per_col));
        FLUID_BY_STORAGE(st, hipLaunchKernelGGL(k_subtract_gradient_max<S>, dim3(per_col, gy), dim3(256), 0, s, (S*)u, (S*)v,
                                                (const S*)p, pitch, n, row_lo, row_hi, h, partials, pinv));
        hipLaunchKernelGGL(k_max_partials, dim3(1), dim3(256), 0, s, partials, (int)(per_col * gy), max_out);
        return;
    }
    FLUID_BY_STORAGE(st, hipLaunchKernelGGL(k_subtract_gradient<S>, dim3(cdiv(n, 256), row_hi - row_lo, mb.count), dim3(256), 0, s,
                                            (S*)u, (S*)v, (const S*)p, pitch, n, row_lo, row_hi, h, pinv, mb.stride));
}

void launch_gradient_advect(hipStream_t s, int st, void* u, void* v, const void* p, void* d, const void* d0, int pitch, int n,
                            int row_lo, int row_hi, float h, float dt0, int b, float pinv, Members mb, const float* mdt0)
{
    if (row_hi <= row_lo) return;
    const dim3 grid(cdiv(n, 1024), row_hi - row_lo, mb.count);
    FLUID_BY_STORAGE_INDEX(st, pitch, n, hipLaunchKernelGGL((k_gradient_advect<S, I>), grid, dim3(256), 0, s, (S*)u, (S*)v, (const S*)p,
                                                            (S*)d, (const S*)d0, pitch, n, row_lo, row_hi, h, dt0, b, pinv, mb.stride,
                                                            mdt0));
}

// ... 64 lines not shown
```

fluidsimulationcuda_amd/csrc/fluid_solver.hip:

```cpp
#include <hip/hip_runtime.h>

#include <algorithm>
#include <cmath>
#include <cstdarg>
#include <cstdio>
#include <cstring>
#include <functional>
#include <mutex>
#include <new>
#include <string>
#include <unordered_map>
#include <vector>

#include "fluid_ctx.h"

namespace fluid_detail {

thread_local std::string g_err;

int fail(int code, const char* fmt, ...)
{
    char buf[512];
    va_list ap;
    va_start(ap, fmt);
    vsnprintf(buf, sizeof buf, fmt, ap);
    va_end(ap);
    g_err = buf;
    return code;
}

int materialize_zero(fluid_ctx* c, int f)
{
    if (!c->field[f].zero) return FLUID_OK;
    HIP_TRY(hipMemsetAsync(c->ptr(f), 0, c->all_bytes(), c->stream));
    c->field[f].zero = false;
    return FLUID_OK;
}

int refuse_ensemble(const fluid_ctx* c, const char* what)
{
    if (c && c->members > 1) return fail(FLUID_E_INVALID, "%s: not available on an ensemble (this context has %d members)", what, c->members);
    return FLUID_OK;
}

}

namespace {

using fluid_detail::fail;
using fluid_detail::g_err;
using fluid_detail::materialize_zero;

constexpr size_t kControlBytes = 256;
constexpr int kMaxMembers = 21845;
constexpr int kMaxN = 65533;

}

namespace {

using fluid::XOFF;

int check_ctx(const fluid_ctx* c)
{
    if (!c) return fail(FLUID_E_INVALID, "null context");
    return FLUID_OK;
}

int check_fields(const fluid_ctx* c, std::initializer_list<int> ids)
{
    for (int id : ids)
        if (!c->valid_field(id)) return fail(FLUID_E_INVALID, "bad field id %d", id);
    return FLUID_OK;
}

int check_iters(int iters)
{
    if (iters < 0 || (iters & 1)) return fail(FLUID_E_INVALID, "sweep count must be even and >= 0 (got %d)", iters);
    return FLUID_OK;
}

int check_b(int b)
{
    if (b < 0 || b > 2) return fail(FLUID_E_INVALID, "b must be 0, 1 or 2");
    return FLUID_OK;
}

constexpr size_t kConstAlign = 256, kConstSlots = 8, kConstBlobs = 64;
size_t const_pad(size_t len) { return (len + kConstAlign - 1) / kConstAlign * kConstAlign; }

// ... 185 lines not shown

struct DivPlan {
    int mode = 0;
    float arg = 0.f;
    float hi = 0.f, lo = 0.f;
    unsigned tile_thr = 0;
    double yd = 0.0;
};

float round_down_to_float(double v)
{
    float f = (float)v;
    if ((double)f > v) f = std::nextafterf(f, -INFINITY);
    return f;
}

DivPlan division_mode(fluid_ctx* c, float beta, float alpha, int force = 0)
{
    DivPlan plan;
    plan.arg = beta;
    plan.yd = 1.0 / (double)beta;
    if (c->fast_div == 0 || !(beta > 0.f) || !std::isfinite(beta)) return plan;
    int e2 = 0;
    const float rbeta = 1.0f / beta;
    const bool pow2 = std::frexp(beta, &e2) == 0.5f && std::isnormal(rbeta) && rbeta * beta == 1.0f;
    const float hi = round_down_to_float(plan.yd), lo = (float)(plan.yd - (double)hi);
    const bool two_term = c->fast_div == 1 && c->tiles && beta >= 1.0f && beta <= 0x1p24f && std::isnormal(hi) && std::isnormal(lo) && lo > 0.f;
    const bool residual = c->fast_div == 2 && beta >= 0x1p-60f && beta <= 0x1p60f;
    const float r5_hi = beta * 0x1p24f, r5_lo = -(rbeta * 0x1p-24f);
    int want = force ? force : (pow2 && alpha == 1.0f) ? 4 : two_term ? 3 : residual ? 5 : 2;
    unsigned bits;
    std::memcpy(&bits, &beta, sizeof bits);
    int dev = 0;
    (void)hipGetDevice(&dev);
    DivProofs& proofs = div_proofs();
    std::lock_guard<std::mutex> lock(proofs.mu);
    int mode = 0;
    while (want != 0) {
        const unsigned long long key = ((unsigned long long)(dev & 0xFF) << 40) | ((unsigned long long)want << 32) | bits;
        auto it = proofs.proven.find(key);
        if (it != proofs.proven.end()) {
            mode = it->second;
        } else {
            unsigned long long* bad = reinterpret_cast<unsigned long long*>(c->d_scalar) + 1;
            unsigned long long* hbad = reinterpret_cast<unsigned long long*>(c->h_scalar) + 1;
            if (hipMemsetAsync(bad, 0, sizeof *bad, c->stream) != hipSuccess) return plan;
            fluid::launch_validate_div(c->stream, want, beta, (want == 4 || want == 5) ? rbeta : beta, plan.yd, want == 5 ? r5_hi : hi,
                                       want == 5 ? r5_lo : lo, bad);
            if (hipMemcpyAsync(hbad, bad, sizeof *bad, hipMemcpyDeviceToHost, c->stream) != hipSuccess ||
                hipStreamSynchronize(c->stream) != hipSuccess)
                return plan;
            mode = *hbad == 0 ? want : 0;
            proofs.proven.emplace(key, mode);
        }
        if (mode != 0) break;
        want = want == 2 ? 0 : 2;
    }
    plan.mode = mode;
    if (mode == 4 || mode == 5) plan.arg = rbeta;
    if (mode == 5) {
        plan.hi = r5_hi;
        plan.lo = r5_lo;
    }
    if (mode == 3) {
        plan.hi = hi;
        plan.lo = lo;
        const float thr = beta * 0x1p-72f;
        std::memcpy(&plan.tile_thr, &thr, sizeof thr);
    }
    return plan;
}

constexpr int kEverywhere = 1 << 28;

int exchange_cap(const fluid_ctx* c) { return c->min_slab - 1; }

void wrote(fluid_ctx* c, int f, int reach)
{
    c->field[f].reach = c->nranks > 1 ? reach : kEverywhere;
    c->field[f].zero = false;
    c->field[f].pend = false;
    c->field[f].src_of = 0;
    c->field[f].fscale = 1.0f;
}

void trade(fluid_ctx* c, int a, int b) { std::swap(c->field[a], c->field[b]); }

int need_list(fluid_ctx* c, const std::vector<int>& fields, int reach, bool async = false)
{
    if (c->nranks == 1 || reach <= 0) return FLUID_OK;
    if (reach > exchange_cap(c)) return fail(FLUID_E_COMM, "halo of %d rows exceeds the slab height", reach);
    std::vector<int> ids;
    for (int f : fields)
        if (c->field[f].reach < reach) ids.push_back(f);
    if (ids.empty()) return FLUID_OK;
    if (!c->xchg) return fail(FLUID_E_COMM, "multi-GPU context without an exchange callback");
    std::sort(ids.begin(), ids.end());
    ids.erase(std::unique(ids.begin(), ids.end()), ids.end());
    c->in_halo_exchange = true;
    const int rc = call_exchange(c, FLUID_XCHG_HALO, ids.data(), (int)ids.size(), reach, nullptr, async);
    c->in_halo_exchange = false;
    if (rc != 0) return fail(FLUID_E_COMM, "halo exchange failed (rc %d)", rc);
    for (int f : ids) c->field[f].reach = reach;
    return FLUID_OK;
}

int need(fluid_ctx* c, std::initializer_list<int> fields, int reach, bool async = false)
{
    return need_list(c, std::vector<int>(fields), reach, async);
}

void rows(const fluid_ctx* c, int reach, int* lo, int* hi)
{
    *lo = std::max(1, c->own0 - reach);
    *hi = std::min(c->n + 1, c->own1 + reach);
}

void rows_with_walls(const fluid_ctx* c, int reach, int* lo, int* hi)
{
    rows(c, reach, lo, hi);
    if (*lo == 1) *lo = 0;
    if (*hi == c->n + 1) *hi = c->n + 2;
}

int settle_source(fluid_ctx* c, int f);

int unscale(fluid_ctx* c, int f)
{
    if (c->field[f].fscale == 1.0f) return FLUID_OK;
    const float inv = 1.0f / c->field[f].fscale;
    c->field[f].fscale = 1.0f;
    if (c->field[f].zero) return FLUID_OK;
    fluid::launch_scale(c->stream, c->st, c->ptr(f), c->pitch, 0, c->n + 2, inv, c->mb());
    return FLUID_OK;
}

int add_source_now(fluid_ctx* c, int x, const void* src, int lo, int hi, const MemberVal& amount)
{
    const float* per_member = nullptr;
    TRY(member_floats(c, amount, &per_member));
    TIMED(c, FLUID_TIME_SOURCE,
          fluid::launch_add_source(c->stream, c->st, c->ptr(x), src, c->pitch, lo, hi, amount.at(0), c->mb(), per_member));
    return FLUID_OK;
}

int settle(fluid_ctx* c, int f, bool keep_scale = false)
{
    if (!keep_scale) TRY(unscale(c, f));
    if (c->field[f].src_of) return settle_source(c, f);
    if (!c->field[f].pend) return FLUID_OK;
    const int reach = c->nranks > 1 ? std::min(c->field[f].reach, exchange_cap(c)) : 0;
    int lo, hi;
    rows_with_walls(c, reach, &lo, &hi);
    TRY(add_source_now(c, f, nullptr, lo, hi, c->field[f].pend_inc));
    c->field[f].pend = false;
    return FLUID_OK;
}

int settle_source(fluid_ctx* c, int f)
{
    if (!c->field[f].src_of) return FLUID_OK;
    const int s = c->field[f].src_of - 1;
    const int reach = c->nranks > 1 ? std::min({c->field[f].reach, c->field[s].reach, exchange_cap(c)}) : 0;
    int lo, hi;
    rows_with_walls(c, reach, &lo, &hi);
    TRY(add_source_now(c, f, c->ptr(s), lo, hi, c->field[f].src_dt));
    wrote(c, f, reach);
    return FLUID_OK;
}

int materialize(fluid_ctx* c, int f, bool keep_scale = false)
{
    TRY(materialize_zero(c, f));
    return settle(c, f, keep_scale);
}

int materialize(fluid_ctx* c, std::initializer_list<int> fs)
{
    for (int f : fs) TRY(materialize(c, f));
    return FLUID_OK;
}

void mark_zero(fluid_ctx* c, int f) { wrote(c, f, kEverywhere); c->field[f].zero = true; }

int op_add_source(fluid_ctx* c, int x, int s, const MemberVal& dt, bool defer = false)
{
    const int reach = c->nranks > 1 ? std::min({c->field[x].reach, c->field[s].reach, exchange_cap(c)}) : 0;
    int lo, hi;
    rows_with_walls(c, reach, &lo, &hi);
    TRY(materialize(c, x));
    if (c->field[s].zero) {
        volatile float z = 0.0f;
        const MemberVal inc = dt.map([&](float d) { return d * z; });
        if (c->variant == fluid::JACOBI_TB && c->defer_zero_source) {
            c->field[x].pend = true;
            c->field[x].pend_inc = inc;
            return FLUID_OK;
        }
        TRY(add_source_now(c, x, nullptr, lo, hi, inc));
    } else {
        TRY(settle(c, s));
        if (defer && c->fuse_add_source && c->variant == fluid::JACOBI_TB && fluid::jacobi_tb_exists(-1, -1, c->tb_nv, fluid::TB_ADDSRC)) {
            c->field[x].src_of = 1 + s;
            c->field[x].src_dt = dt;
            return FLUID_OK;
        }
        TRY(add_source_now(c, x, c->ptr(s), lo, hi, dt));
    }
    wrote(c, x, reach);
    return FLUID_OK;
}

struct RbTuner {
    struct Entry {
        std::vector<int> cand;
        std::vector<float> best_ms;
        std::vector<int> samples, issued;
        int fixed = 0;
        std::string what;
    };
    std::mutex mu;
    std::unordered_map<unsigned long long, Entry> table;
};
RbTuner& rb_tuner()
{
    static RbTuner t;
    return t;
}
constexpr int kTuneSamples = 2;

// ... 95 lines not shown
            *ev = c->free_events.back();
            c->free_events.pop_back();
        } else {
            HIP_TRY(hipEventCreate(ev));
        }
    }
    HIP_TRY(hipEventRecord(tr.a, c->stream));
    c->trials.push_back(tr);
    return FLUID_OK;
}

int tune_end(fluid_ctx* c)
{
    HIP_TRY(hipEventRecord(c->trials.back().b, c->stream));
    return FLUID_OK;
}

struct SweepShape {
    bool canonical, small;
    long long slab_cells;
};

SweepShape sweep_shape(const fluid_ctx* c, int count)
{
    const bool canonical = c->st == fluid::STORAGE_F16;
    const long long slab_cells = (long long)(c->nranks > 1 ? c->min_slab : c->n) * c->n;
    return {canonical, (canonical ? (long long)c->n * c->n : slab_cells * count) < c->tb_min_cells, slab_cells};
}

int pick_sweeps(const fluid_ctx* c, int remaining, int room, const SweepShape& shape, bool all_mode4)
{
    const long long slab_cells = shape.slab_cells;
    if (c->variant != fluid::JACOBI_TB || shape.small || c->field_bytes >= 0x7F000000ull) return 1;
    room = std::min(room, remaining);
    const int greedy = (room >= 8 && c->tb_max_t >= 8) ? 8 : (room >= 4 && c->tb_max_t >= 4) ? 4 : room >= 2 ? 2 : 1;
    if (shape.canonical || !fluid::jacobi_tb_exists(12, -1, c->tb_nv, fluid::TB_PLAIN) || c->tb_max_t < 12 || room < 12 || (remaining & 1)) return greedy;
    const bool forced = c->tb_t16_min_cells >= 0;
    const bool big = forced ? slab_cells >= c->tb_t16_min_cells : slab_cells >= (8ll << 20);
    if (!big) return greedy;
    const long long slab_rows = slab_cells / std::max(c->n, 1);
    const bool pays16 = forced || ((all_mode4 || (unsigned long long)slab_cells * c->esz > (96ull << 20)) && slab_rows >= 3000);
    const int* depth = fluid::kTbDepths;
    constexpr int nd = (int)std::size(fluid::kTbDepths);
    static const double per_sweep[] = {1.00, 1.04, 1.30, 2.6, 5.0};
    static_assert(std::size(per_sweep) == nd, "one cost per depth");
    const double per_launch = 0.5;
    bool allowed[nd];
    for (int k = 0; k < nd; ++k)
        allowed[k] = depth[k] <= c->tb_max_t && (depth[k] != 16 || pays16) && fluid::jacobi_tb_exists(depth[k], -1, c->tb_nv, fluid::TB_PLAIN);
    std::vector<double> cost(remaining + 1, 1e300);
    cost[0] = 0.0;
    for (int r = 2; r <= remaining; r += 2)
        for (int k = 0; k < nd; ++k) {
            if (!allowed[k] || depth[k] > r) continue;
            const double v = cost[r - depth[k]] + depth[k] * per_sweep[k] + per_launch;
            if (v < cost[r] - 1e-9) cost[r] = v;
        }
    int best = 0;
    for (int r = remaining; r > 0;) {
        int pickd = 0;
        for (int k = 0; k < nd && !pickd; ++k)
            if (allowed[k] && depth[k] <= r && std::fabs(cost[r - depth[k]] + depth[k] * per_sweep[k] + per_launch - cost[r]) < 1e-9)
                pickd = depth[k];
        if (!pickd) break;
        if (pickd <= room) best = std::max(best, pickd);
        r -= pickd;
    }
    return best ? best : greedy;
}

struct Coeffs {
    MemberVal alpha, beta;
};

struct Solve {
    int b, x, x0;
    const Coeffs* k;
};

struct DivSource {
    int u, v;
    float scale;
};

struct Batch {
    const Solve* sv;
    int count, iters, final_reach;
    const DivSource* ds;
    int scratch_base;
    const int* scratch;
    const int* sum;
    int cur[3], nxt[3];
    std::vector<DivPlan> plan[3];
    bool same_mode, all_mode4, add_src;
    float out_scale[3];
    SweepShape shape;
};

size_t tile_words(const fluid_ctx* c) { return (size_t)fluid::tile_rows(c->n) * fluid::tile_pitch(c->n); }
unsigned* solve_tiles(const fluid_ctx* c, int slot) { return c->tiles + (size_t)slot * c->members * tile_words(c); }

void plan_members(fluid_ctx* c, const Coeffs& k, std::vector<DivPlan>& out)
{
    const int M = c->members;
    const MemberVal &alpha = k.alpha, &beta = k.beta;
    out.resize(M);
    bool same = true;
    for (int m = 0; m < M; ++m) {
        out[m] = (m > 0 && beta.at(m) == beta.at(m - 1) && alpha.at(m) == alpha.at(m - 1)) ? out[m - 1] : division_mode(c, beta.at(m), alpha.at(m));
        same = same && out[m].mode == out[0].mode;
    }
    if (same) return;
    bool all2 = true;
    for (int m = 0; m < M; ++m) {
        out[m] = division_mode(c, beta.at(m), alpha.at(m), 2);
        all2 = all2 && out[m].mode == 2;
    }
    if (all2) return;
    for (int m = 0; m < M; ++m) {
        out[m] = DivPlan{};
        out[m].arg = beta.at(m);
        out[m].yd = 1.0 / (double)beta.at(m);
    }
}

int batch_prepare(fluid_ctx* c, Batch& B)
{
    static const int kScratch[3] = {FLUID_TMP0, FLUID_TMP1, FLUID_TMP2};
    static const int kSum[3] = {FLUID_TMP3, FLUID_TMP4, FLUID_TMP5};
    const Solve* sv = B.sv;
    if (B.scratch_base < 0 || B.scratch_base + B.count > 3) return fail(FLUID_E_INVALID, "a batch holds 1 to 3 solves");
    B.scratch = kScratch + B.scratch_base;
    B.sum = kSum + B.scratch_base;
    TRY(check_iters(B.iters));
    if (B.count < 1 || B.count > 3) return fail(FLUID_E_INVALID, "a batch holds 1 to 3 solves");
    for (int k = 0; k < B.count; ++k) {
        if (sv[k].x == sv[k].x0 || sv[k].x >= FLUID_TMP0 || sv[k].x0 >= FLUID_TMP0)
            return fail(FLUID_E_INVALID, "diffuse: x and x0 must be distinct non-scratch fields");
        for (int j = 0; j < k; ++j)
            if (sv[j].x == sv[k].x || sv[j].x == sv[k].x0 || sv[j].x0 == sv[k].x)
                return fail(FLUID_E_INVALID, "diffuse: the solves of a batch must not share fields");
    }
    for (int k = 0; k < B.count; ++k) {
        const FieldState &x = c->field[sv[k].x], &x0 = c->field[sv[k].x0];
        if ((x.zero ? x0.fscale : x.fscale) != x0.fscale || x0.src_of) {
            if (x.fscale != 1.0f || x0.fscale != 1.0f) TRY(xchg_join(c));
            TRY(unscale(c, sv[k].x));
            TRY(unscale(c, sv[k].x0));
        }
        B.out_scale[k] = x0.fscale;
    }
    if (B.iters == 0) {
        TRY(xchg_join(c));
        for (int k = 0; k < B.count; ++k) TRY(settle_source(c, sv[k].x0));
        return FLUID_OK;
    }
    for (int k = 0; k < B.count; ++k) TRY(materialize_zero(c, sv[k].x0));
    for (int k = 0; k < B.count; ++k)
        if (c->field[sv[k].x].pend) {
            TRY(xchg_join(c));
            TRY(settle(c, sv[k].x, true));
        }
    return FLUID_OK;
}

int batch_plan(fluid_ctx* c, Batch& B)
{
    const Solve* sv = B.sv;
    B.same_mode = B.all_mode4 = true;
    for (int k = 0; k < B.count; ++k) {
        B.cur[k] = sv[k].x;
// ... 57 lines not shown
    const DivPlan& p = B.plan[j][B.plan[j].size() > 1 ? (size_t)m : 0];
    return {p.yd, B.sv[j].k->alpha.at(m), p.arg, p.hi, p.lo, x0_inc.at(m), div_scale.at(m), p.tile_thr, 0};
}

int fill_batch(fluid_ctx* c, const Batch& B, int first, int last, bool divsrc, bool addsrc, fluid::TbBatch* out)
{
    static const MemberVal nothing_pending(-0.0f);
    const MemberVal own_scale(divsrc ? B.ds->scale : 0.0f);
    const MemberVal& div_scale = addsrc ? c->field[B.sv[first].x0].src_dt : own_scale;
    const MemberVal* x0_inc[3];
    fluid::TbBatch bt{};
    bool per_member = !div_scale.uniform();
    for (int j = first; j < last; ++j) {
        const int q = j - first;
        const FieldState& x0 = c->field[B.sv[j].x0];
        x0_inc[q] = x0.pend && !addsrc && !divsrc ? &x0.pend_inc : &nothing_pending;
        per_member = per_member || B.plan[j].size() > 1 || !x0_inc[q]->uniform();
        const fluid::TbMemberK k0 = solve_constants(B, j, 0, *x0_inc[q], div_scale);
        bt.x[q] = c->ptr(B.cur[j]);
        bt.x0[q] = x0.ptr;
        bt.out[q] = c->ptr(B.nxt[j]);
        bt.alpha[q] = k0.alpha;
        bt.beta[q] = k0.beta;
        bt.yd[q] = k0.yd;
        bt.hi[q] = k0.hi;
        bt.lo[q] = k0.lo;
        bt.tiles[q] = B.plan[j][0].mode == 3 ? solve_tiles(c, B.scratch_base + j) : nullptr;
        bt.tile_thr[q] = k0.tile_thr;
        bt.b[q] = B.sv[j].b;
        bt.x_zero[q] = c->field[B.cur[j]].zero ? 1 : 0;
        bt.x0_inc[q] = k0.x0_inc;
        if (addsrc) bt.div[q] = c->ptr(B.sum[j]);
    }
    bt.count = last - first;
    bt.members = c->members;
    bt.mstride = c->field_floats;
    bt.tile_mstride = tile_words(c);
    bt.tile_pitch = fluid::tile_pitch(c->n);
    bt.div_scale = div_scale.at(0);
    if (divsrc) {
        bt.x[0] = c->ptr(B.ds->u);
        bt.x0[0] = c->ptr(B.ds->v);
        bt.div[0] = c->ptr(B.sv[0].x0);
    }
    if (per_member && c->members > 1) {
        const int M = c->members;
        std::vector<fluid::TbMemberK> rec((size_t)bt.count * M);
        for (int j = first; j < last; ++j)
            for (int m = 0; m < M; ++m) rec[(size_t)(j - first) * M + m] = solve_constants(B, j, m, *x0_inc[j - first], div_scale);
        const void* dev = nullptr;
        TRY(member_consts(c, rec.data(), rec.size() * sizeof rec[0], &dev));
        bt.mk = static_cast<const fluid::TbMemberK*>(dev);
    }
    *out = bt;
    return FLUID_OK;
}

int edge_rows(const fluid_ctx* c, int T, int rb) { return std::max(2 * T, rb * (c->tb_edge_pct > 0 ? c->tb_edge_pct : 100) / 100); }

int strip_rows(const fluid_ctx* c, int T, int m, long long rows_n)
{
    const int nv = c->tb_nv;
    const int HL = (T + nv - 1) / nv, VS = 64 - 2 * HL;
    const long long windows = ((c->n + nv - 1) / nv + VS - 1) / VS;
    const long long inner = windows > 2 ? windows - 2 : 0, outer = windows - inner;
    const int resident = nv == 2 ? (T >= 16 ? 2 : 4) : (T >= 8 ? 2 : 3);
    const long long room = (long long)c->num_cu * resident * 92 / 100;
    const int cap = T >= 16 ? 192 : (T >= 8 ? 80 : 96) * (m > 1 ? 2 : 1);
    int rb = c->tb_fill ? T : 2 * T;
    auto fits = [&](int r) {
        const long long si = (rows_n + r - 1) / r, se = (rows_n + edge_rows(c, T, r) - 1) / edge_rows(c, T, r);
        return (inner * ((si + 3) / 4) + outer * ((se + 3) / 4)) * m <= room;
    };
    for (; rb < cap; rb += 2)
        if (fits(rb)) break;
    if (rows_n <= 1100) {
        const int low = std::max(2, std::min(rb, (int)(rows_n / 64) & ~1));
        if (c->members == 1 || fits(low)) rb = low;
        else rb = (int)std::min<long long>(rb, std::max<long long>(low, (rows_n + 1) & ~1ll));
    }
    return rb;
}

int launch_fused(fluid_ctx* c, const fluid::TbBatch& bt, int T, int divmode, bool divsrc, bool addsrc, int lo, int hi)
{
    const bool owed = c->nranks > 1 && (c->xowed & stream_bit(c));
    const int in_lo = owed && c->rank > 0 ? std::max(lo, c->own0 + T) : lo;
    const int in_hi = owed && c->rank < c->nranks - 1 ? std::min(hi, c->own1 - T) : hi;
    const bool split = owed && in_hi - in_lo >= 2 * T && (in_lo > lo || in_hi < hi);
    const int form = divsrc ? fluid::TB_DIVSRC : addsrc ? fluid::TB_ADDSRC : fluid::TB_PLAIN;
    for (int part = split ? 0 : 1; part < 2; ++part) {
        const int plo = part ? lo : in_lo, phi = part ? hi : in_hi;
        const int hole_lo = part && split ? in_lo : 0, hole_hi = part && split ? in_hi : 0;
        if (part) TRY(xchg_join(c));
        const long long rows_n = (phi - plo) - std::max(0, hole_hi - hole_lo);
        int rb = c->tb_rows > 0 ? c->tb_rows : strip_rows(c, T, bt.count * c->members, rows_n);
        int trial = -1;
        unsigned long long key = 0;
        if (c->tb_rows <= 0 && c->autotune) {
            key = tune_key(c, T, bt.count + (divsrc ? 8 : 0) + (addsrc ? 16 : 0) + (hole_hi > hole_lo ? 32 : 0), divmode, rows_n);
            rb = tune_pick(c, key, rb, T, rows_n, &trial, bt.count, form, divmode);
        }
        if (trial >= 0) TRY(tune_begin(c, key, trial));
        if (!fluid::launch_jacobi_tb(c->stream, c->st, T, divmode, c->tb_nv, form, bt, c->pitch, c->n, plo, phi, rb,
                                     std::min(rb, edge_rows(c, T, rb)), hole_lo, hole_hi, c->tb_fill))
            return fail(FLUID_E_INVALID, "no fused Jacobi kernel: %d sweeps, division mode %d, %d-column lanes, form %d", T, divmode, c->tb_nv, form);
        if (trial >= 0) TRY(tune_end(c));
    }
    if (split) c->split_launches += 1;
    return FLUID_OK;
}

void commit_launch(fluid_ctx* c, Batch& B, bool first, int r)
{
    if (B.ds && first && c->nranks > 1)
        c->field[B.sv[0].x0].reach = std::max(0, std::min(c->field[B.sv[0].x0].reach, r));
    if (B.add_src && first) {
        for (int j = 0; j < B.count; ++j) {
            trade(c, B.sv[j].x0, B.sum[j]);
            wrote(c, B.sum[j], 0);
            wrote(c, B.sv[j].x0, std::max(0, r));
        }
        B.add_src = false;
    }
    for (int j = 0; j < B.count; ++j) {
        c->field[B.cur[j]].zero = false;
        wrote(c, B.nxt[j], r);
        std::swap(B.cur[j], B.nxt[j]);
    }
}

int batch_sweep(fluid_ctx* c, Batch& B)
{
    const Solve* sv = B.sv;
    const bool multi = c->nranks > 1, canonical = B.shape.canonical;
    int r = multi ? batch_reach(c, B) : kEverywhere;
    for (int k = 0; k < B.iters;) {
        const int remaining = B.iters - k;
        const int wantT = canonical ? pick_sweeps(c, remaining, remaining, B.shape, B.all_mode4) : 1;
        if (r < wantT) {
            const int depth = std::max(wantT, std::min(c->halo, remaining + B.final_reach));
            std::vector<int> ids;
            for (int j = 0; j < B.count; ++j) {
                ids.push_back(B.cur[j]);
                if (c->field[sv[j].x0].reach < depth - 1) ids.push_back(sv[j].x0);
            }
            TRY(xchg_join(c));
            TRY(need_list(c, ids, depth, true));
            r = batch_reach(c, B);
        }
        const int T = canonical ? wantT : pick_sweeps(c, remaining, std::min(r, remaining), B.shape, B.all_mode4);
        if (B.add_src && k == 0 && !fluid::jacobi_tb_exists(T, B.plan[0][0].mode, c->tb_nv, fluid::TB_ADDSRC)) {
            B.add_src = false;
            TRY(xchg_join(c));
            for (int j = 0; j < B.count; ++j) TRY(settle_source(c, sv[j].x0));
        }
        int lo, hi;
        rows(c, multi ? std::min(r - T, exchange_cap(c)) : 0, &lo, &hi);
        if (T == 1) {
            const int v = c->variant == fluid::JACOBI_TB ? (B.shape.small ? fluid::JACOBI_NAIVE : fluid::JACOBI_STREAM) : c->variant;
            TRY(xchg_join(c));
            for (int j = 0; j < B.count; ++j) TRY(materialize(c, B.cur[j], true));
            for (int j = 0; j < B.count; ++j) TRY(settle(c, sv[j].x0, true));
            for (int j = 0; j < B.count; ++j) {
                const float2* mab = nullptr;
                TRY(member_pairs(c, sv[j].k->alpha, sv[j].k->beta, &mab));
                fluid::launch_jacobi(c->stream, c->st, v, c->ptr(B.cur[j]), c->ptr(sv[j].x0), c->ptr(B.nxt[j]), c->pitch, c->n, lo, hi,
                                     sv[j].k->alpha.at(0), sv[j].k->beta.at(0), sv[j].b, c->mb(), mab);
            }
            if (c->timing) {
                c->launches += B.count;
                c->field_launches += (long long)B.count * c->members;
            }
        } else {
            for (int first = 0, last; first < B.count; first = last) {
                last = B.same_mode ? B.count : first + 1;
                const bool divsrc = B.ds != nullptr && k == 0, addsrc = B.add_src && k == 0;
                fluid::TbBatch bt;
                TRY(fill_batch(c, B, first, last, divsrc, addsrc, &bt));
                TRY(launch_fused(c, bt, T, B.plan[first][0].mode, divsrc, addsrc, lo, hi));
                if (c->timing) {
                    c->launches += 1;
                    c->field_launches += (long long)(last - first) * c->members;
                }
            }
        }
        r = multi ? std::min(r - T, exchange_cap(c)) : kEverywhere;
        commit_launch(c, B, k == 0, r);
        k += T;
    }
    return FLUID_OK;
}

int op_diffuse_batch(fluid_ctx* c, const Solve* sv, int count, int iters, int final_reach = 0, const DivSource* ds = nullptr,
                     int scratch_base = 0)
{
    Batch B{sv, count, iters, final_reach, ds, scratch_base};
    TRY(batch_prepare(c, B));
    if (iters == 0) return FLUID_OK;
    hipEvent_t stop;
    TRY(timing_begin(c, FLUID_TIME_DIFFUSION, &stop));
    TRY(batch_plan(c, B));
    TRY(batch_sweep(c, B));
    HIP_TRY(hipGetLastError());
    for (int j = 0; j < count; ++j) {
        if (B.cur[j] != sv[j].x) trade(c, sv[j].x, B.scratch[j]);
        wrote(c, B.scratch[j], 0);
        c->field[sv[j].x].fscale = B.out_scale[j];
    }
    return timing_end(c, stop, iters * count * c->members);
}

int op_diffuse(fluid_ctx* c, int b, int x, int x0, const Coeffs& k, int iters, int final_reach = 0, const DivSource* ds = nullptr)
{
    const Solve one{b, x, x0, &k};
    return op_diffuse_batch(c, &one, 1, iters, final_reach, ds);
}

int vmax_begin(fluid_ctx* c, int u, int v, bool have_max = false)
{
    if (c->nranks == 1) return FLUID_OK;
    if (!have_max) {
        TRY(materialize(c, {u, v}));
        HIP_TRY(hipMemsetAsync(c->d_scalar, 0, sizeof(unsigned), c->stream));
        fluid::launch_absmax2(c->stream, c->st, c->ptr(u), c->ptr(v), c->pitch, c->n, c->own0, c->own1, c->d_scalar, c->mb());
    }
    TRY(exchange(c, FLUID_XCHG_MAX_BEGIN, {}, 0));
    HIP_TRY(hipMemcpyAsync(c->h_scalar, c->d_scalar, sizeof(unsigned), hipMemcpyDeviceToHost, c->stream));
    HIP_TRY(hipEventRecord(c->scalar_ready, c->stream));
    return FLUID_OK;
}

int advect_rows(fluid_ctx* c, std::initializer_list<int> sources, float dt0, int have, float* vmax, bool* fetched)
{
    HIP_TRY(hipEventSynchronize(c->scalar_ready));
    std::memcpy(vmax, c->h_scalar, sizeof *vmax);
    TRY(exchange(c, FLUID_XCHG_MAX_END, {}, 0, vmax));
    const double reach = std::ceil((double)std::fabs(dt0) * (double)*vmax) + 2.0;
    *fetched = !(have > 0 && reach <= (double)have);
    if (!*fetched) return FLUID_OK;
    if (reach <= (double)exchange_cap(c)) return need(c, sources, (int)reach);
    TRY(exchange(c, FLUID_XCHG_GATHER, sources, 0));
    for (int f : sources) c->field[f].reach = kEverywhere;
    return FLUID_OK;
}

int advect_bounded(fluid_ctx* c, int slot, std::initializer_list<int> sources, float dt0, const std::function<int()>& run)
{
    if (c->nranks == 1) return run();
    int guess = 0;
    const float prev = c->vmax_prev[slot];
    if (c->early_advect && prev >= 0.0f) {
        const double g = std::ceil((double)std::fabs(dt0) * (double)prev * 1.25) + 2.0;
        if (g <= (double)exchange_cap(c)) {
            guess = (int)g;
            TRY(need(c, sources, guess));
            TRY(run());
        }
    }
    float vmax = 0.f;
    bool fetched = false;
    TRY(advect_rows(c, sources, dt0, guess, &vmax, &fetched));
    c->vmax_prev[slot] = std::isfinite(vmax) ? vmax : -1.0f;
    return fetched ? run() : FLUID_OK;
}

int member_dt0(fluid_ctx* c, const MemberVal& dt, const float** dev)
{
    return member_floats(c, dt.map([&](float d) { return d * (float)c->n; }), dev);
}

int op_advect(fluid_ctx* c, int b, int d, int d0, int u, int v, const MemberVal& dt)
{
    if (d == d0 || d == u || d == v) return fail(FLUID_E_INVALID, "advect: output must not alias an input");
    const float dt0 = dt.at(0) * (float)c->n;
    TRY(materialize(c, {d0, u, v}));
    const float* mdt0 = nullptr;
    TRY(member_dt0(c, dt, &mdt0));
    TIMED(c, FLUID_TIME_ADVECTION,
          fluid::launch_advect(c->stream, c->st, c->ptr(d), c->ptr(d0), c->ptr(u), c->ptr(v), c->pitch, c->n, c->own0, c->own1, dt0, b, c->mb(),
                               mdt0));
    wrote(c, d, 0);
    return FLUID_OK;
}

int op_advect2(fluid_ctx* c, int ba, int da, int d0a, int bb, int db, int d0b, int u, int v, const MemberVal& dt)
{
    for (int d : {da, db})
        if (d == d0a || d == d0b || d == u || d == v) return fail(FLUID_E_INVALID, "advect: output must not alias an input");
    if (da == db) return fail(FLUID_E_INVALID, "advect: outputs must be distinct");
    const float dt0 = dt.at(0) * (float)c->n;
    TRY(materialize(c, {d0a, d0b, u, v}));
    const float* mdt0 = nullptr;
    TRY(member_dt0(c, dt, &mdt0));
    TIMED(c, FLUID_TIME_ADVECTION,
          fluid::launch_advect2(c->stream, c->st, c->ptr(da), c->ptr(d0a), ba, c->ptr(db), c->ptr(d0b), bb, c->ptr(u), c->ptr(v), c->pitch,
                                c->n, c->own0, c->own1, dt0, c->mb(), mdt0));
    wrote(c, da, 0);
    wrote(c, db, 0);
    return FLUID_OK;
}

int op_divergence(fluid_ctx* c, int u, int v, int p, int div, int want = 0, float pscale = 1.0f)
{
    if (p == u || p == v || div == u || div == v || p == div)
        return fail(FLUID_E_INVALID, "divergence: outputs must not alias inputs");
    const float h = 1.0f / (float)c->n;
    int reach = 0;
    TRY(materialize(c, {u, v}));
    if (c->nranks > 1) {
        reach = std::max(0, std::min(want, exchange_cap(c) - 1));
        TRY(need(c, {u, v}, reach + 1));
    }
    int lo, hi;
    rows(c, reach, &lo, &hi);
    TIMED(c, FLUID_TIME_DIVERGENCE,
          fluid::launch_divergence(c->stream, c->st, c->ptr(u), c->ptr(v), c->ptr(p), c->ptr(div), c->pitch, c->n, lo, hi, h,
                                   0, pscale, c->mb()));
    wrote(c, div, reach);
    c->field[div].fscale = pscale;
    mark_zero(c, p);
    return FLUID_OK;
}

int op_subtract_gradient(fluid_ctx* c, int u, int v, int p, bool with_max = false)
{
    if (p == u || p == v || u == v) return fail(FLUID_E_INVALID, "subtract_gradient: fields must be distinct");
    const float h = 1.0f / (float)c->n;
    TRY(materialize(c, {u, v}));
    TRY(materialize(c, p, true));
    TRY(need(c, {p}, 1));
    with_max = with_max && c->nranks > 1 && c->d_partials;
    TIMED(c, FLUID_TIME_PROJECTION,
          fluid::launch_subtract_gradient(c->stream, c->st, c->ptr(u), c->ptr(v), c->ptr(p), c->pitch, c->n, c->own0, c->own1, h,
                                          c->d_partials, with_max ? c->d_scalar : nullptr, 1.0f / c->field[p].fscale, c->mb()));
    wrote(c, u, 0);
    wrote(c, v, 0);
    return FLUID_OK;
}

int op_gradient_advect(fluid_ctx* c, int u, int v, int p, int b, int d, int d0, const MemberVal& dt)
{
    if (p == u || p == v || u == v) return fail(FLUID_E_INVALID, "subtract_gradient: fields must be distinct");
    if (d == d0 || d == u || d == v || d == p || d0 == u || d0 == v)
        return fail(FLUID_E_INVALID, "advect: output must not alias an input");
    if (c->nranks != 1) return fail(FLUID_E_INVALID, "op_gradient_advect is a one-GPU operator");
    const float h = 1.0f / (float)c->n;
    TRY(materialize(c, {u, v, d0}));
    TRY(materialize(c, p, true));
    const float* mdt0 = nullptr;
    TRY(member_dt0(c, dt, &mdt0));
    TIMED(c, FLUID_TIME_PROJECTION,
          fluid::launch_gradient_advect(c->stream, c->st, c->ptr(u), c->ptr(v), c->ptr(p), c->ptr(d), c->ptr(d0), c->pitch, c->n, c->own0,
                                        c->own1, h, dt.at(0) * (float)c->n, b, 1.0f / c->field[p].fscale, c->mb(), mdt0));
    wrote(c, u, 0);
    wrote(c, v, 0);
    wrote(c, d, 0);
    return FLUID_OK;
}

void coefficients(int n, float dt, float coef, float* alpha, float* beta)
{
    volatile float a = dt * coef;
    a = a * (float)n;
    a = a * (float)n;
    volatile float four_a = 4.0f * a;
    *alpha = a;
    *beta = 1.0f + four_a;
}

Coeffs diffusion_coeffs(const fluid_ctx* c, const MemberVal& dt, const MemberVal& coef)
{
    auto part = [&](bool want_beta) {
        return dt.map(coef, [&](float d, float k) {
            float alpha, beta;
            coefficients(c->n, d, k, &alpha, &beta);
            return want_beta ? beta : alpha;
        });
    };
    return {part(false), part(true)};
}

struct AdvectAfter {
    int b, d, d0;
    const MemberVal& dt;
};

bool divergence_fuses(fluid_ctx* c, int iters, int reach)
{
    if (c->variant != fluid::JACOBI_TB || !c->fuse_divergence) return false;
    const SweepShape shape = sweep_shape(c, 1);
    if (shape.small) return false;
    const int room = c->nranks > 1 ? std::min(reach + 1, iters) : iters;
    if (!fluid::jacobi_tb_exists(pick_sweeps(c, iters, room, shape, true), 4, c->tb_nv, fluid::TB_DIVSRC)) return false;
    return division_mode(c, 4.0f, 1.0f).mode == 4;
}

int project(fluid_ctx* c, int u, int v, int p, int div, int iters, const AdvectAfter* then_advect = nullptr, bool with_max = false)
{
    const int reach = c->nranks > 1 ? std::max(0, std::min(std::min(iters, c->halo - 1), exchange_cap(c) - 1)) : 0;
    const bool fused = divergence_fuses(c, iters, reach);
    const DivSource ds{u, v, (-0.5f * (1.0f / (float)c->n)) * c->pscale};
    if (fused) {
        if (p == u || p == v || div == u || div == v || p == div)
            return fail(FLUID_E_INVALID, "divergence: outputs must not alias inputs");
        TRY(materialize(c, {u, v}));
        if (c->nranks > 1) TRY(need(c, {u, v}, reach + 1, true));
        mark_zero(c, p);
        wrote(c, div, reach);
        c->field[div].fscale = c->pscale;
    } else {
        TRY(op_divergence(c, u, v, p, div, std::min(iters, c->halo - 1), c->pscale));
    }
    c->in_pressure_solve = true;
    const Coeffs pressure{1.0f, 4.0f};
    const int rc_solve = op_diffuse(c, 0, p, div, pressure, iters, 1, fused ? &ds : nullptr);
    c->in_pressure_solve = false;
    TRY(rc_solve);
    if (fused) {
        TRY(xchg_join(c));
        wrote(c, div, 0);
        c->field[div].fscale = c->pscale;
    }
    if (then_advect) return op_gradient_advect(c, u, v, p, then_advect->b, then_advect->d, then_advect->d0, then_advect->dt);
    return op_subtract_gradient(c, u, v, p, with_max);
}

int vel_step(fluid_ctx* c, const MemberVal& dt, const MemberVal& visc, int iters)
{
    const int U = FLUID_U, V = FLUID_V, U0 = FLUID_U_PREV, V0 = FLUID_V_PREV;
    TRY(op_add_source(c, U, U0, dt, true));
    TRY(op_add_source(c, V, V0, dt, true));
    const Coeffs cv = diffusion_coeffs(c, dt, visc);
    const int h = std::min(iters, c->halo);
    TRY(need(c, {U, V, U0, V0}, h, true));
    const Solve uv[2] = {{1, U0, U, &cv}, {2, V0, V, &cv}};
    TRY(op_diffuse_batch(c, uv, 2, iters));
    TRY(xchg_join(c));
    TRY(project(c, U0, V0, U, V, iters, nullptr, true));
    const float dt0 = dt.at(0) * (float)c->n;
    TRY(vmax_begin(c, U0, V0, true));
    TRY(advect_bounded(c, 0, {U0, V0}, dt0, [&] { return op_advect2(c, 1, U, U0, 2, V, V0, U0, V0, dt); }));
    return project(c, U, V, U0, V0, iters);
}

int dens_step(fluid_ctx* c, const MemberVal& dt, const MemberVal& diff, int iters)
{
    const int X = FLUID_DENS, X0 = FLUID_DENS_PREV;
    TRY(op_add_source(c, X, X0, dt, true));
    const Coeffs cd = diffusion_coeffs(c, dt, diff);
    const Solve one{0, X0, X, &cd};
    TRY(op_diffuse_batch(c, &one, 1, iters));
    TRY(vmax_begin(c, FLUID_U, FLUID_V));
    return advect_bounded(c, 1, {X0}, dt.at(0) * (float)c->n, [&] { return op_advect(c, 0, X, X0, FLUID_U, FLUID_V, dt); });
}

int full_step(fluid_ctx* c, const MemberVal& dt, const MemberVal& diff, const MemberVal& visc, int iters)
{
    const int U = FLUID_U, V = FLUID_V, D = FLUID_DENS, U0 = FLUID_U_PREV, V0 = FLUID_V_PREV, D0 = FLUID_DENS_PREV;
    TRY(op_add_source(c, U, U0, dt, true));
    TRY(op_add_source(c, V, V0, dt, true));
    TRY(op_add_source(c, D, D0, dt, true));
    TRY(need(c, {U, V, D, U0, V0, D0}, std::min(iters, c->halo), true));
    const Coeffs cv = diffusion_coeffs(c, dt, visc), cd = diffusion_coeffs(c, dt, diff);
    const float dt0 = dt.at(0) * (float)c->n;
    const Solve all[3] = {{1, U0, U, &cv}, {2, V0, V, &cv}, {0, D0, D, &cd}};
    if (c->nranks == 1) {
        TRY(op_diffuse_batch(c, all, 3, iters));
        TRY(project(c, U0, V0, U, V, iters));
        TRY(op_advect2(c, 1, U, U0, 2, V, V0, U0, V0, dt));
        const AdvectAfter dens{0, D, D0, dt};
        return project(c, U, V, U0, V0, iters, &dens);
    }
    int fill1 = 0, fill2 = 0;
    {
        const SweepShape shape = sweep_shape(c, 1);
        std::vector<int> launches;
        for (int left = iters; left > 0;) {
            launches.push_back(pick_sweeps(c, left, left, shape, false));
            left -= launches.back();
        }
        for (int* fill : {&fill2, &fill1})
            while (*fill < 8 && !launches.empty()) {
                *fill += launches.back();
                launches.pop_back();
            }
        if (fill1 == 0) std::swap(fill1, fill2);
    }
    if (c->stream2 && c->slab_overlap && std::min(iters, c->halo) >= iters) {
        HIP_TRY(hipEventRecord(c->ev_fork, c->stream));
        HIP_TRY(hipStreamWaitEvent(c->stream2, c->ev_fork, 0));
        c->xowed = (c->xowed & 1u) ? 3u : 0u;
        hipStream_t main_stream = c->stream;
        c->stream = c->stream2;
        const int rc_dens = op_diffuse_batch(c, all + 2, 1, iters, 0, nullptr, 2);
        hipError_t e_join = rc_dens == FLUID_OK ? hipEventRecord(c->ev_join, c->stream2) : hipSuccess;
        c->stream = main_stream;
        TRY(rc_dens);
        HIP_TRY(e_join);
        TRY(op_diffuse_batch(c, all, 2, iters));
        TRY(project(c, U0, V0, U, V, iters, nullptr, true));
        TRY(vmax_begin(c, U0, V0, true));
        TRY(advect_bounded(c, 0, {U0, V0}, dt0, [&] { return op_advect2(c, 1, U, U0, 2, V, V0, U0, V0, dt); }));
        TRY(project(c, U, V, U0, V0, iters, nullptr, true));
        TRY(vmax_begin(c, U, V, true));
        HIP_TRY(hipStreamWaitEvent(c->stream, c->ev_join, 0));
        return advect_bounded(c, 1, {D0}, dt0, [&] { return op_advect(c, 0, D, D0, U, V, dt); });
    }
    const int rest = fill1 + fill2, head = iters - rest;
    if (head > 0) TRY(op_diffuse_batch(c, all, 3, head));
    if (rest > 0) TRY(op_diffuse_batch(c, all, 2, rest));
    TRY(xchg_join(c));
    TRY(project(c, U0, V0, U, V, iters, nullptr, true));
    TRY(vmax_begin(c, U0, V0, true));
    if (fill1 > 0) TRY(op_diffuse_batch(c, all + 2, 1, fill1));
    TRY(advect_bounded(c, 0, {U0, V0}, dt0, [&] { return op_advect2(c, 1, U, U0, 2, V, V0, U0, V0, dt); }));
    TRY(project(c, U, V, U0, V0, iters, nullptr, true));
    TRY(vmax_begin(c, U, V, true));
    if (fill2 > 0) TRY(op_diffuse_batch(c, all + 2, 1, fill2));
    return advect_bounded(c, 1, {D0}, dt0, [&] { return op_advect(c, 0, D, D0, U, V, dt); });
}

int zero_sources(fluid_ctx* c)
{
    for (int id : {FLUID_U_PREV, FLUID_V_PREV, FLUID_DENS_PREV}) mark_zero(c, id);
    return FLUID_OK;
}

int copy_rows(fluid_ctx* c, int field, float* host, const float* chost, int row_lo, int row_hi, bool to_device, bool wait = true,
              int member = 0)
{
    if (row_lo < 0 || row_hi > c->w || row_lo > row_hi) return fail(FLUID_E_INVALID, "bad row range");
    if (row_lo == row_hi) return FLUID_OK;
    const float host_scale = (!to_device && c->st != fluid::STORAGE_F32) ? 1.0f / c->field[field].fscale : 1.0f;
    TRY(materialize(c, field, host_scale != 1.0f));
    char* dev = static_cast<char*>(c->row(field, row_lo)) + (size_t)member * c->field_bytes + (size_t)XOFF * c->esz;
    const size_t rows = (size_t)(row_hi - row_lo), w = (size_t)c->w;
    const size_t dp = (size_t)c->pitch * c->esz;
    if (to_device) c->field[field].reach = 0;
    if (c->st == fluid::STORAGE_F32) {
        const size_t hp = w * sizeof(float);
        if (to_device)
            HIP_TRY(hipMemcpy2DAsync(dev, dp, chost + (size_t)row_lo * w, hp, hp, rows, hipMemcpyHostToDevice, c->stream));
        else
            HIP_TRY(hipMemcpy2DAsync(host + (size_t)row_lo * w, hp, dev, dp, hp, rows, hipMemcpyDeviceToHost, c->stream));
        if (wait) HIP_TRY(hipStreamSynchronize(c->stream));
        return FLUID_OK;
    }
    std::vector<fluid::half_t> stage(rows * w);
    const size_t hp = w * sizeof(fluid::half_t);
    if (to_device) {
// ... 156 lines not shown
}

int fluid_create(int N, fluid_ctx** out)
{
    fluid_config cfg;
    std::memset(&cfg, 0, sizeof cfg);
    cfg.n = N;
    cfg.nranks = 1;
    cfg.jacobi_variant = FLUID_JACOBI_TB;
    return fluid_create_ex(&cfg, out);
}

int fluid_destroy(fluid_ctx* c)
{
    if (!c) return FLUID_OK;
    if (c->stream) (void)hipStreamSynchronize(c->stream);
    if (c->stream2) (void)hipStreamSynchronize(c->stream2);
    if (c->xstream) (void)hipStreamSynchronize(c->xstream);
    for (auto& p : c->ev_pool) {
        (void)hipEventDestroy(p.a);
        (void)hipEventDestroy(p.b);
    }
    if (!c->trials.empty()) {
        RbTuner& t = rb_tuner();
        std::lock_guard<std::mutex> lock(t.mu);
        for (auto& tr : c->trials) {
            auto it = t.table.find(tr.key);
            if (it != t.table.end() && !it->second.fixed && it->second.issued[tr.cand] > 0) it->second.issued[tr.cand] -= 1;
            (void)hipEventDestroy(tr.a);
            (void)hipEventDestroy(tr.b);
        }
    }
    for (hipEvent_t ev : c->free_events) (void)hipEventDestroy(ev);
    fluid_detail::rccl_release(c->rccl);
    c->rccl = nullptr;
    if (c->h_scalar) (void)hipHostFree(c->h_scalar);
    if (c->tiles) (void)hipFree(c->tiles);
    for (auto& b : c->consts.live) (void)hipEventDestroy(b.copied);
    for (hipEvent_t ev : c->consts.free_events) (void)hipEventDestroy(ev);
    if (c->consts.dev) (void)hipFree(c->consts.dev);
    if (c->consts.host) (void)hipHostFree(c->consts.host);
    if (c->red.d_max) (void)hipFree(c->red.d_max);
    if (c->red.d_moments) (void)hipFree(c->red.d_moments);
    if (c->red.d_partials) (void)hipFree(c->red.d_partials);
    if (c->red.host) (void)hipHostFree(c->red.host);
    if (c->red.d_mean) (void)hipFree(c->red.d_mean);
    if (c->red.d_var) (void)hipFree(c->red.d_var);
    if (c->stage.dev) (void)hipFree(c->stage.dev);
    if (c->d_partials) (void)hipFree(c->d_partials);
    if (c->scalar_ready) (void)hipEventDestroy(c->scalar_ready);
    if (c->own_arena && c->arena) (void)hipFree(c->arena);
    if (c->stream2) (void)hipStreamDestroy(c->stream2);
    if (c->xstream) (void)hipStreamDestroy(c->xstream);
    if (c->ev_xbegin) (void)hipEventDestroy(c->ev_xbegin);
    if (c->ev_xdone) (void)hipEventDestroy(c->ev_xdone);
    if (c->ev_fork) (void)hipEventDestroy(c->ev_fork);
    if (c->ev_join) (void)hipEventDestroy(c->ev_join);
    if (c->own_stream && c->stream) (void)hipStreamDestroy(c->stream);
    if (g_cached == c) g_cached = nullptr;
    delete c;
    return FLUID_OK;
}

int fluid_synchronize(fluid_ctx* c)
{
    TRY(check_ctx(c));
    HIP_TRY(hipStreamSynchronize(c->stream));
    return FLUID_OK;
}

int fluid_exchange_stream(fluid_ctx* c, void** stream)
{
    TRY(check_ctx(c));
    if (!stream) return fail(FLUID_E_INVALID, "null pointer");
    *stream = c->stream;
    return FLUID_OK;
}

int fluid_split_launches(fluid_ctx* c, long long* count)
{
    TRY(check_ctx(c));
    if (!count) return fail(FLUID_E_INVALID, "null pointer");
    *count = c->split_launches;
    return FLUID_OK;
}

int fluid_owned_rows(fluid_ctx* c, int* row_lo, int* row_hi)
{
    TRY(check_ctx(c));
    if (row_lo) *row_lo = c->own0;
    if (row_hi) *row_hi = c->own1;
    return FLUID_OK;
}

int fluid_field_ptr(fluid_ctx* c, int field, void** dev_ptr)
{
    TRY(check_ctx(c));
    TRY(check_fields(c, {field}));
    if (!dev_ptr) return fail(FLUID_E_INVALID, "null pointer");
    if (c->in_halo_exchange) TRY(materialize_zero(c, field));
    else TRY(materialize(c, field));
    *dev_ptr = c->ptr(field);
    return FLUID_OK;
}

int fluid_scalar_ptr(fluid_ctx* c, void** dev_ptr)
{
    TRY(check_ctx(c));
    if (!dev_ptr) return fail(FLUID_E_INVALID, "null pointer");
    *dev_ptr = c->d_scalar;
    return FLUID_OK;
}

int fluid_members(fluid_ctx* c, int* members)
{
    TRY(check_ctx(c));
    if (!members) return fail(FLUID_E_INVALID, "null pointer");
    *members = c->members;
    return FLUID_OK;
}

static int refuse_plain_copy(const fluid_ctx* c, const char* what)
{
    if (c->members > 1)
        return fail(FLUID_E_INVALID, "%s: this context has %d members -- use fluid_upload_member / fluid_download_member", what, c->members);
    return FLUID_OK;
}

static int check_member(const fluid_ctx* c, int member)
{
    if (member < 0 || member >= c->members) return fail(FLUID_E_INVALID, "member %d outside [0, %d)", member, c->members);
    return FLUID_OK;
}

int fluid_upload_member(fluid_ctx* c, int member, int field, const float* host)
{
    TRY(check_ctx(c));
    TRY(check_fields(c, {field}));
    TRY(check_member(c, member));
    if (!host) return fail(FLUID_E_INVALID, "null host pointer");
    return copy_rows(c, field, nullptr, host, 0, c->w, true, true, member);
}

int fluid_download_member(fluid_ctx* c, int member, int field, float* host)
{
    TRY(check_ctx(c));
    TRY(check_fields(c, {field}));
    TRY(check_member(c, member));
    if (!host) return fail(FLUID_E_INVALID, "null host pointer");
    return copy_rows(c, field, host, nullptr, 0, c->w, false, true, member);
}

int fluid_upload_rows(fluid_ctx* c, int field, const float* host, int row_lo, int row_hi)
{
    TRY(check_ctx(c));
    TRY(refuse_plain_copy(c, "fluid_upload_rows"));
    TRY(check_fields(c, {field}));
    if (!host) return fail(FLUID_E_INVALID, "null host pointer");
    return copy_rows(c, field, nullptr, host, row_lo, row_hi, true);
}

int fluid_download_rows(fluid_ctx* c, int field, float* host, int row_lo, int row_hi)
{
    TRY(check_ctx(c));
    TRY(refuse_plain_copy(c, "fluid_download_rows"));
    TRY(check_fields(c, {field}));
    if (!host) return fail(FLUID_E_INVALID, "null host pointer");
    return copy_rows(c, field, host, nullptr, row_lo, row_hi, false);
}

int fluid_upload(fluid_ctx* c, int field, const float* host)
{
    TRY(check_ctx(c));
    TRY(refuse_plain_copy(c, "fluid_upload"));
    return fluid_upload_rows(c, field, host, 0, c->w);
}

int fluid_download(fluid_ctx* c, int field, float* host)
{
    TRY(check_ctx(c));
    TRY(refuse_plain_copy(c, "fluid_download"));
    return fluid_download_rows(c, field, host, 0, c->w);
}

int fluid_fill(fluid_ctx* c, int field, float value)
{
    TRY(check_ctx(c));
    TRY(check_fields(c, {field}));
    if (value == 0.0f && !std::signbit(value)) {
        HIP_TRY(hipMemsetAsync(c->ptr(field), 0, c->all_bytes(), c->stream));
        wrote(c, field, kEverywhere);
        return FLUID_OK;
    }
    std::vector<float> row((size_t)c->w * c->w, value);
    for (int m = 0; m < c->members; ++m) TRY(fluid_upload_member(c, m, field, row.data()));
    wrote(c, field, kEverywhere);
    return FLUID_OK;
}

int fluid_set_jacobi_variant(fluid_ctx* c, int variant)
{
    TRY(check_ctx(c));
    if (variant < 0 || variant >= fluid::JACOBI_VARIANTS) return fail(FLUID_E_INVALID, "unknown Jacobi variant %d", variant);
    c->variant = variant;
    return FLUID_OK;
}

int fluid_set_param(fluid_ctx* c, int key, int value)
{
    TRY(check_ctx(c));
    switch (key) {
    case FLUID_PARAM_TB_MAX_SWEEPS:
        if (!fluid::is_tb_depth(value)) return fail(FLUID_E_INVALID, "TB_MAX_SWEEPS must be 16, 12, 8, 4 or 2");
        c->tb_max_t = value;
        return FLUID_OK;
    case FLUID_PARAM_TB_ROWS:
        if (value < 0) return fail(FLUID_E_INVALID, "TB_ROWS must be >= 0");
        c->tb_rows = value;
        return FLUID_OK;
    case FLUID_PARAM_TB_EDGE_ROWS_PCT:
        if (value < 0 || value > 100) return fail(FLUID_E_INVALID, "TB_EDGE_ROWS_PCT must be in [0,100]");
        c->tb_edge_pct = value;
        return FLUID_OK;
    case FLUID_PARAM_TB_MIN_CELLS:
        if (value < 0) return fail(FLUID_E_INVALID, "TB_MIN_CELLS must be >= 0");
        c->tb_min_cells = value;
        return FLUID_OK;
    case FLUID_PARAM_TB_FAST_DIVISION:
        if (value < 0 || value > 3) return fail(FLUID_E_INVALID, "TB_FAST_DIVISION must be 0, 1, 2 or 3");
        c->fast_div = value;
        return FLUID_OK;
    case FLUID_PARAM_TB_AUTOTUNE:
        c->autotune = value != 0;
        return FLUID_OK;
    case FLUID_PARAM_TB_FILL:
        c->tb_fill = value != 0;
        return FLUID_OK;
    case FLUID_PARAM_SLAB_OVERLAP:
        c->slab_overlap = value != 0;
        return FLUID_OK;
    case FLUID_PARAM_FUSE_DIVERGENCE:
        c->fuse_divergence = value != 0;
        return FLUID_OK;
    case FLUID_PARAM_EARLY_ADVECT:
        c->early_advect = value != 0;
        return FLUID_OK;
    case FLUID_PARAM_FUSE_ADD_SOURCE:
        c->fuse_add_source = value != 0;
        return FLUID_OK;
    case FLUID_PARAM_F16_PRESSURE_SCALE: {
        for (int f = 0; f < FLUID_NFIELDS; ++f) TRY(unscale(c, f));
        int e = 0;
        (void)std::frexp((float)c->n, &e);
        c->pscale = (value != 0 && c->st == fluid::STORAGE_F16 && c->n >= 16) ? std::ldexp(1.0f, e - 3) : 1.0f;
        return FLUID_OK;
    }
    case FLUID_PARAM_XCHG_OVERLAP:
        TRY(xchg_join(c));
        c->xchg_overlap = value != 0;
        return FLUID_OK;
    case FLUID_PARAM_TB_T16_MIN_CELLS:
        if (value < -1) return fail(FLUID_E_INVALID, "TB_T16_MIN_CELLS must be >= 0, or -1 for the default rule");
        c->tb_t16_min_cells = value;
        return FLUID_OK;
    case FLUID_PARAM_TB_LANE_COLUMNS:
        if (value != 2 && value != 4) return fail(FLUID_E_INVALID, "TB_LANE_COLUMNS must be 2 or 4");
        c->tb_nv = value;
        return FLUID_OK;
    case FLUID_PARAM_HALO:
        if (value < 1) return fail(FLUID_E_INVALID, "HALO must be >= 1");
        c->halo = c->nranks > 1 ? std::max(c->st == fluid::STORAGE_F16 ? 8 : 1, std::min(value, c->min_slab - 1)) : 1;
        return FLUID_OK;
    default:
        return fail(FLUID_E_INVALID, "unknown parameter %d", key);
    }
}

int fluid_plan_sweeps(int N, int rows, int storage, int pressure_form, int iters, int max_sweeps, int t16_min_cells, int* depths,
                      int capacity, int* count)
{
    if (N < 1 || N > kMaxN || rows < 1 || rows > N || iters < 0 || (iters & 1) || !depths || !count || capacity < 0)
        return fail(FLUID_E_INVALID, "fluid_plan_sweeps: bad argument");
    if (storage != FLUID_STORAGE_F32 && storage != FLUID_STORAGE_F16) return fail(FLUID_E_INVALID, "unknown storage type %d", storage);
    if (!fluid::is_tb_depth(max_sweeps)) return fail(FLUID_E_INVALID, "max_sweeps must be 16, 12, 8, 4 or 2");
    fluid_ctx c;
    c.n = N;
    c.st = storage;
    c.esz = fluid::storage_bytes(storage);
    c.field_bytes = (size_t)(N + 2) * fluid::pitch_for(N) * c.esz;
    c.tb_max_t = max_sweeps;
    c.tb_t16_min_cells = t16_min_cells;
    const SweepShape shape{storage == FLUID_STORAGE_F16, false, (long long)rows * N};
    int k = 0;
    for (int left = iters; left > 0;) {
        const int t = pick_sweeps(&c, left, left, shape, pressure_form != 0);
        if (k < capacity) depths[k] = t;
        ++k;
        left -= t;
    }
    *count = k;
    return FLUID_OK;
}

int fluid_autotune_pending(fluid_ctx* c, int* shapes_open)
{
    TRY(check_ctx(c));
    if (!shapes_open) return fail(FLUID_E_INVALID, "null pointer");
    tune_harvest(c);
    RbTuner& t = rb_tuner();
    std::lock_guard<std::mutex> lock(t.mu);
    int open = 0;
    for (auto& kv : t.table) open += kv.second.fixed ? 0 : 1;
    *shapes_open = open;
    return FLUID_OK;
}

int fluid_division_mode(fluid_ctx* c, float alpha, float beta, int* mode)
{
    TRY(check_ctx(c));
    if (!mode) return fail(FLUID_E_INVALID, "null pointer");
    *mode = c->variant == fluid::JACOBI_TB ? division_mode(c, beta, alpha).mode : 0;
    return FLUID_OK;
}

int fluid_set_exchange(fluid_ctx* c, fluid_exchange_fn fn, void* user)
{
    TRY(check_ctx(c));
    TRY(fluid_detail::refuse_ensemble(c, "fluid_set_exchange"));
    c->xchg = fn;
    c->xchg_user = user;
    return FLUID_OK;
}
// ... 140 lines not shown
int fluid_op_jacobi_sweep_members(fluid_ctx* c, int b, int x, int x0, int out, const float* alpha, const float* beta)
{
    TRY(check_member_args(c, "fluid_op_jacobi_sweep_members", {{"alpha", alpha}, {"beta", beta}}));
    if (c->members == 1) return fluid_op_jacobi_sweep(c, b, x, x0, out, alpha[0], beta[0]);
    TRY(ensure_consts(c));
    return jacobi_sweep_body(c, b, x, x0, out, {alpha, c->members}, {beta, c->members});
}

static int diffuse_body(fluid_ctx* c, int b, int x, int x0, const Coeffs& k, int iters)
{
    TRY(check_ctx(c));
    TRY(check_fields(c, {x, x0}));
    TRY(check_b(b));
    return op_diffuse(c, b, x, x0, k, iters);
}

int fluid_op_diffuse(fluid_ctx* c, int b, int x, int x0, float alpha, float beta, int iters) { return diffuse_body(c, b, x, x0, {alpha, beta}, iters); }

int fluid_op_diffuse_members(fluid_ctx* c, int b, int x, int x0, const float* alpha, const float* beta, int iters)
{
    TRY(check_member_args(c, "fluid_op_diffuse_members", {{"alpha", alpha}, {"beta", beta}}));
    if (c->members == 1) return fluid_op_diffuse(c, b, x, x0, alpha[0], beta[0], iters);
    TRY(ensure_consts(c));
    return diffuse_body(c, b, x, x0, {{alpha, c->members}, {beta, c->members}}, iters);
}

static int advect_body(fluid_ctx* c, int b, int d, int d0, int u, int v, const MemberVal& dt)
{
    TRY(check_ctx(c));
    TRY(check_fields(c, {d, d0, u, v}));
    TRY(check_b(b));
    if (d == d0 || d == u || d == v) return fail(FLUID_E_INVALID, "advect: output must not alias an input");
    if (c->nranks > 1) {
        float vmax = 0.f;
        bool fetched = false;
        TRY(vmax_begin(c, u, v));
        TRY(advect_rows(c, {d0}, dt.at(0) * (float)c->n, 0, &vmax, &fetched));
    }
    TRY(op_advect(c, b, d, d0, u, v, dt));
    HIP_TRY(hipGetLastError());
    return FLUID_OK;
}

int fluid_op_advect(fluid_ctx* c, int b, int d, int d0, int u, int v, float dt) { return advect_body(c, b, d, d0, u, v, dt); }

int fluid_op_advect_members(fluid_ctx* c, int b, int d, int d0, int u, int v, const float* dt)
{
    TRY(check_member_args(c, "fluid_op_advect_members", {{"dt", dt}}));
    if (c->members == 1) return fluid_op_advect(c, b, d, d0, u, v, dt[0]);
    TRY(ensure_consts(c));
    return advect_body(c, b, d, d0, u, v, {dt, c->members});
}

int fluid_op_set_bnd(fluid_ctx* c, int b, int x)
{
    TRY(check_ctx(c));
    TRY(check_fields(c, {x}));
    TRY(check_b(b));
    if (c->nranks != 1) return fail(FLUID_E_INVALID, "fluid_op_set_bnd is a whole-grid operator (1 GPU)");
    TRY(materialize(c, x));
    fluid::launch_set_bnd(c->stream, c->st, c->ptr(x), c->pitch, c->n, b, c->mb());
    HIP_TRY(hipGetLastError());
    return FLUID_OK;
}

int fluid_op_divergence(fluid_ctx* c, int u, int v, int p, int div)
{
    TRY(check_ctx(c));
    TRY(check_fields(c, {u, v, p, div}));
    TRY(op_divergence(c, u, v, p, div));
    HIP_TRY(hipGetLastError());
    return FLUID_OK;
}

int fluid_op_subtract_gradient(fluid_ctx* c, int u, int v, int p)
{
    TRY(check_ctx(c));
    TRY(check_fields(c, {u, v, p}));
    TRY(op_subtract_gradient(c, u, v, p));
    HIP_TRY(hipGetLastError());
    return FLUID_OK;
}

int fluid_residual(fluid_ctx* c, int x, int x0, float alpha, float beta, float* out)
{
    TRY(check_ctx(c));
    TRY(check_fields(c, {x, x0}));
    if (!out) return fail(FLUID_E_INVALID, "null pointer");
    TRY(materialize(c, {x, x0}));
    TRY(need(c, {x}, 1));
    HIP_TRY(hipMemsetAsync(c->d_scalar, 0, sizeof(unsigned), c->stream));
    fluid::launch_residual(c->stream, c->st, c->ptr(x), c->ptr(x0), c->pitch, c->n, c->own0, c->own1, alpha, beta, c->d_scalar,
                           c->mb());
    TRY(reduce_to_host(c, out));
    return exchange(c, FLUID_XCHG_MAX, {}, 0, out);
}

int fluid_absmax_velocity(fluid_ctx* c, int u, int v, float* out)
{
    TRY(check_ctx(c));
    TRY(check_fields(c, {u, v}));
    if (!out) return fail(FLUID_E_INVALID, "null pointer");
    TRY(materialize(c, {u, v}));
    HIP_TRY(hipMemsetAsync(c->d_scalar, 0, sizeof(unsigned), c->stream));
    fluid::launch_absmax2(c->stream, c->st, c->ptr(u), c->ptr(v), c->pitch, c->n, c->own0, c->own1, c->d_scalar, c->mb());
    TRY(reduce_to_host(c, out));
    return exchange(c, FLUID_XCHG_MAX, {}, 0, out);
}

static int ensure_member_results(fluid_ctx* c)
{
    EnsembleReduce& r = c->red;
    if (r.d_max) return FLUID_OK;
    const size_t m = (size_t)c->members;
    const size_t parts = m * (size_t)fluid::moment_blocks(c->n, c->members);
    unsigned int* d_max = nullptr;
    double2 *d_mom = nullptr, *d_part = nullptr;
    char* host = nullptr;
    hipError_t e = hipMalloc((void**)&d_max, m * sizeof(unsigned));
    if (e == hipSuccess) e = hipMalloc((void**)&d_mom, m * sizeof(double2));
    if (e == hipSuccess) e = hipMalloc((void**)&d_part, parts * sizeof(double2));
    if (e == hipSuccess) e = hipHostMalloc((void**)&host, m * sizeof(double2), hipHostMallocDefault);
    if (e != hipSuccess) {
        if (d_max) (void)hipFree(d_max);
        if (d_mom) (void)hipFree(d_mom);
        if (d_part) (void)hipFree(d_part);
        (void)hipGetLastError();
        return fail(e == hipErrorOutOfMemory ? FLUID_E_NOMEM : FLUID_E_HIP, "ensemble diagnostics: allocating the results of %d members: %s",
                    c->members, hipGetErrorString(e));
    }
    r.d_max = d_max;
    r.d_moments = d_mom;
    r.d_partials = d_part;
    r.host = host;
    return FLUID_OK;
}

static int ensure_stats(fluid_ctx* c)
{
    EnsembleReduce& r = c->red;
    if (r.d_mean) return FLUID_OK;
    const size_t bytes = c->field_floats * sizeof(float);
    float *mean = nullptr, *var = nullptr;
    hipError_t e = hipMalloc((void**)&mean, bytes);
    if (e == hipSuccess) e = hipMalloc((void**)&var, bytes);
    if (e == hipSuccess) e = hipMemsetAsync(mean, 0, bytes, c->stream);
    if (e == hipSuccess) e = hipMemsetAsync(var, 0, bytes, c->stream);
    if (e != hipSuccess) {
        if (mean) (void)hipFree(mean);
        if (var) (void)hipFree(var);
        (void)hipGetLastError();
        return fail(e == hipErrorOutOfMemory ? FLUID_E_NOMEM : FLUID_E_HIP, "fluid_ensemble_stats: allocating two fields of %zu bytes: %s", bytes,
                    hipGetErrorString(e));
    }
    r.d_mean = mean;
    r.d_var = var;
    return FLUID_OK;
}

static int member_words_to_host(fluid_ctx* c, float* out)
{
    const size_t bytes = (size_t)c->members * sizeof(unsigned);
    HIP_TRY(hipMemcpyAsync(c->red.host, c->red.d_max, bytes, hipMemcpyDeviceToHost, c->stream));
    HIP_TRY(hipStreamSynchronize(c->stream));
    std::memcpy(out, c->red.host, bytes);
    return FLUID_OK;
// ... 419 lines not shown
```

fluidsimulationcuda_amd/solver.py:

```python
import ctypes as C
import sys

import numpy as np

from . import capi

DT, VIS, DIFF, ITERS = 0.016, 0.0025, 0.1, 40

_ID = {name: k for k, name in enumerate(capi.FIELD_NAMES)}


def _fid(f):
    if isinstance(f, str):
        return _ID[f]
    return int(f)


def _host(a, n):
    a = np.ascontiguousarray(a, dtype=np.float32)
    if a.shape != (n + 2, n + 2):
        raise ValueError("field must have shape (%d, %d), got %s" % (n + 2, n + 2, a.shape))
    return a


# ... 135 lines not shown
                out = torch.empty((count, len(ids), self.members, w, w), dtype=torch.float32, device="cuda")
            capacity = device_floats(out, count * len(ids) * self.members * w * w)
        plan = capi.RunPlan(iters=int(iters), nsteps=nsteps, use_sources=1 if use_sources else 0,
                            sources=device_address(sources) if sources is not None else None, every=every,
                            fields=(C.c_int * len(ids))(*ids) if ids else None, nfields=len(ids),
                            snapshots=device_address(out) if every > 0 else None, capacity=capacity)
        written = C.c_int()
        mv = member_values(self.members, dt=dt, diff=diff, visc=visc)
        self._handover(wait)
        if mv is None:
            capi.check(capi.lib().fluid_run(self._h, dt, diff, visc, C.byref(plan), C.byref(written)))
        else:
            capi.check(capi.lib().fluid_run_members(self._h, *[_mf(a) for a in mv.values()], C.byref(plan), C.byref(written)))
        if wait:
            self.synchronize()
        return (out if every > 0 else None), written.value

    def member_count(self):
        m = C.c_int()
        capi.check(capi.lib().fluid_members(self._h, C.byref(m)))
        return m.value

    def upload_rows(self, field, arr, row_lo, row_hi):
        capi.check(capi.lib().fluid_upload_rows(self._h, _fid(field), _host(arr, self.n), row_lo, row_hi))

    def download(self, field, out=None, member=None):
        if out is None:
            out = np.empty((self.n + 2, self.n + 2), dtype=np.float32)
        if member is None:
            capi.check(capi.lib().fluid_download(self._h, _fid(field), _host(out, self.n)))
        else:
            capi.check(capi.lib().fluid_download_member(self._h, int(member), _fid(field), _host(out, self.n)))
        return out

    def download_rows(self, field, out, row_lo, row_hi):
        capi.check(capi.lib().fluid_download_rows(self._h, _fid(field), out, row_lo, row_hi))
        return out

    def fill(self, field, value=0.0):
        capi.check(capi.lib().fluid_fill(self._h, _fid(field), value))

    def synchronize(self):
        capi.check(capi.lib().fluid_synchronize(self._h))

    def field_ptr(self, field):
        p = C.c_void_p()
        capi.check(capi.lib().fluid_field_ptr(self._h, _fid(field), C.byref(p)))
        return p.value

    def scalar_ptr(self):
        p = C.c_void_p()
        capi.check(capi.lib().fluid_scalar_ptr(self._h, C.byref(p)))
        return p.value

    def set_bnd(self, b, x):
        capi.check(capi.lib().fluid_op_set_bnd(self._h, b, _fid(x)))

    def _call(self, name, before, params, after=()):
        mv = member_values(self.members, **params)
        if mv is None:
            fn, values = getattr(capi.lib(), "fluid_" + name), params.values()
        else:
            fn, values = getattr(capi.lib(), "fluid_" + name + "_members"), [_mf(a) for a in mv.values()]
        capi.check(fn(self._h, *before, *values, *after))

    def add_source(self, x, s, dt=DT):
        self._call("op_add_source", (_fid(x), _fid(s)), dict(dt=dt))

    def jacobi_sweep(self, b, x, x0, out, alpha, beta):
        self._call("op_jacobi_sweep", (b, _fid(x), _fid(x0), _fid(out)), dict(alpha=alpha, beta=beta))

    def diffuse(self, b, x, x0, alpha, beta, iters=ITERS):
        self._call("op_diffuse", (b, _fid(x), _fid(x0)), dict(alpha=alpha, beta=beta), (iters,))

    def advect(self, b, d, d0, u, v, dt=DT):
        self._call("op_advect", (b, _fid(d), _fid(d0), _fid(u), _fid(v)), dict(dt=dt))

    def computeDivergenceAndPressure(self, u, v, p, div):
        capi.check(capi.lib().fluid_op_divergence(self._h, _fid(u), _fid(v), _fid(p), _fid(div)))

    def lastProject(self, u, v, p, div=None):
        capi.check(capi.lib().fluid_op_subtract_gradient(self._h, _fid(u), _fid(v), _fid(p)))

    def vel_step(self, visc=VIS, dt=DT, iters=ITERS):
        self._call("vel_step", (), dict(dt=dt, visc=visc), (iters,))

    def dens_step(self, diff=DIFF, dt=DT, iters=ITERS):
        self._call("dens_step", (), dict(dt=dt, diff=diff), (iters,))

    def step(self, nsteps=1, use_sources=False, dt=DT, diff=DIFF, visc=VIS, iters=ITERS):
        self._call("step", (), dict(dt=dt, diff=diff, visc=visc), (iters, nsteps, 1 if use_sources else 0))

    def residual(self, x, x0, alpha, beta):
        out = C.c_float()
        capi.check(capi.lib().fluid_residual(self._h, _fid(x), _fid(x0), alpha, beta, C.byref(out)))
        return out.value

    def absmax_velocity(self, u="u", v="v"):
        out = C.c_float()
        capi.check(capi.lib().fluid_absmax_velocity(self._h, _fid(u), _fid(v), C.byref(out)))
        return out.value

    def residual_members(self, x, x0, alpha, beta):
        mv = member_values(self.members, alpha=alpha, beta=beta)
        if mv is None:
            mv = {"alpha": np.full(self.members, alpha, np.float32), "beta": np.full(self.members, beta, np.float32)}
        out = np.empty(self.members, np.float32)
        capi.check(capi.lib().fluid_residual_members(self._h, _fid(x), _fid(x0), _mf(mv["alpha"]), _mf(mv["beta"]), _mf(out)))
        return out

    def absmax_velocity_members(self, u="u", v="v"):
        out = np.empty(self.members, np.float32)
        capi.check(capi.lib().fluid_absmax_velocity_members(self._h, _fid(u), _fid(v), _mf(out)))
        return out

    def member_moments(self, field):
        s, q = np.empty(self.members, np.float64), np.empty(self.members, np.float64)
        dp = C.POINTER(C.c_double)
        capi.check(capi.lib().fluid_member_moments(self._h, _fid(field), s.ctypes.data_as(dp), q.ctypes.data_as(dp)))
        return s, q

    def ensemble_stats(self, field, mean=True, variance=True):
        w = self.n + 2
        mu = np.empty((w, w), np.float32) if mean else None
        var = np.empty((w, w), np.float32) if variance else None
        capi.check(capi.lib().fluid_ensemble_stats(self._h, _fid(field), _mf(mu) if mean else None, _mf(var) if variance else None))
        return mu, var

    def ensemble_stats_ptr(self):
        mu, var = C.c_void_p(), C.c_void_p()
        capi.check(capi.lib().fluid_ensemble_stats_ptr(self._h, C.byref(mu), C.byref(var)))
        return mu.value, var.value

    def set_jacobi_variant(self, variant):
        capi.check(capi.lib().fluid_set_jacobi_variant(self._h, variant))

    def division_mode(self, alpha, beta):
        m = C.c_int()
        capi.check(capi.lib().fluid_division_mode(self._h, alpha, beta, C.byref(m)))
        return m.value

    def autotune_pending(self):
        m = C.c_int()
        capi.check(capi.lib().fluid_autotune_pending(self._h, C.byref(m)))
        return m.value

    def set_param(self, key, value):
        capi.check(capi.lib().fluid_set_param(self._h, key, value))

    def timing_enable(self, on=True):
        capi.check(capi.lib().fluid_timing_enable(self._h, 1 if on else 0))

    def timing_read(self, reset=True):
        t = capi.Timing()
        capi.check(capi.lib().fluid_timing_read(self._h, C.byref(t), 1 if reset else 0))
        out = {"jacobi_ms": t.jacobi_ms, "sweeps": t.sweeps, "solves": t.solves,
               "jacobi_launches": t.jacobi_launches, "jacobi_field_launches": t.jacobi_field_launches,
               "pressure_ms": t.pressure_ms, "pressure_sweeps": t.pressure_sweeps}
        for k, name in enumerate(capi.TIMING_CATEGORIES):
            out[name + "_ms"] = t.category_ms[k]
            out[name + "_calls"] = t.category_calls[k]
        return out

    def diffuse_tol(self, b, x, x0, alpha, beta, tol, max_iters=10000, check_every=8):
        it, res = C.c_int(), C.c_float()
        capi.check(capi.lib().fluid_op_diffuse_tol(self._h, b, _fid(x), _fid(x0), alpha, beta, tol, max_iters,
                                                   check_every, C.byref(it), C.byref(res)))
        return it.value, res.value

    def split_launches(self):
        m = C.c_longlong()
        capi.check(capi.lib().fluid_split_launches(self._h, C.byref(m)))
        return m.value

    def exchange_stream(self):
        p = C.c_void_p()
        capi.check(capi.lib().fluid_exchange_stream(self._h, C.byref(p)))
        return p.value or 0

    def set_exchange(self, fn):
        if fn is None:
            self._cb = None
            capi.check(capi.lib().fluid_set_exchange(self._h, C.cast(None, capi.EXCHANGE_FN), None))
            return

        def tramp(_user, kind, fields, nfields, depth, scalar):
            try:
                ids = [fields[k] for k in range(nfields)]
                if kind in (capi.XCHG_MAX, capi.XCHG_MAX_END):
                    scalar[0] = float(fn(kind, ids, depth, float(scalar[0])))
                else:
                    fn(kind, ids, depth, None)
                return 0
            except Exception:
                import traceback
                traceback.print_exc()
                return 1

        self._cb = capi.EXCHANGE_FN(tramp)
        capi.check(capi.lib().fluid_set_exchange(self._h, self._cb, None))


def coefficients(n, dt, coef):
    a, b = C.c_float(), C.c_float()
    capi.check(capi.lib().fluid_coefficients(n, dt, coef, C.byref(a), C.byref(b)))
    return a.value, b.value


def step(N, dt, diff, visc, u, v, dens):
    for a in (u, v, dens):
        if a.dtype != np.float32 or not a.flags.c_contiguous or a.shape != (N + 2, N + 2):
            raise ValueError("fields must be C-contiguous float32 of shape (N+2, N+2)")
    capi.check(capi.lib().step(N, dt, diff, visc, u, v, dens))


def step_src(N, dt, diff, visc, iters, u, v, dens, u_prev, v_prev, dens_prev):
    for a in (u, v, dens, u_prev, v_prev, dens_prev):
        if a.dtype != np.float32 or not a.flags.c_contiguous or a.shape != (N + 2, N + 2):
            raise ValueError("fields must be C-contiguous float32 of shape (N+2, N+2)")
    capi.check(capi.lib().step_src(N, dt, diff, visc, iters, u, v, dens, u_prev, v_prev, dens_prev))
```

include/fluid_amd.h:

```cpp
#ifndef FLUID_AMD_H
#define FLUID_AMD_H

#include <stddef.h>

#ifdef __cplusplus
extern "C" {
#endif

#define FLUID_OK        0
#define FLUID_E_INVALID 1
#define FLUID_E_NOMEM   2
#define FLUID_E_HIP     3
#define FLUID_E_COMM    4

enum {
    FLUID_U = 0, FLUID_V = 1, FLUID_DENS = 2,
    FLUID_U_PREV = 3, FLUID_V_PREV = 4, FLUID_DENS_PREV = 5,
    FLUID_TMP0 = 6, FLUID_TMP1 = 7, FLUID_TMP2 = 8,
    FLUID_TMP3 = 9, FLUID_TMP4 = 10, FLUID_TMP5 = 11,
    FLUID_NFIELDS = 12
};

enum { FLUID_JACOBI_STREAM = 0, FLUID_JACOBI_LDS = 1, FLUID_JACOBI_NAIVE = 2, FLUID_JACOBI_TB = 3 };

enum {
    FLUID_PARAM_TB_MAX_SWEEPS = 0,
    FLUID_PARAM_TB_ROWS = 1,
    FLUID_PARAM_HALO = 2,
    FLUID_PARAM_TB_FAST_DIVISION = 3
    ,FLUID_PARAM_TB_EDGE_ROWS_PCT = 5
    ,FLUID_PARAM_TB_LANE_COLUMNS = 6
    ,FLUID_PARAM_TB_T16_MIN_CELLS = 7
    ,FLUID_PARAM_TB_AUTOTUNE = 8
    ,FLUID_PARAM_SLAB_OVERLAP = 10
    ,FLUID_PARAM_EARLY_ADVECT = 11
    ,FLUID_PARAM_FUSE_DIVERGENCE = 9
    ,FLUID_PARAM_FUSE_ADD_SOURCE = 12
    ,FLUID_PARAM_XCHG_OVERLAP = 13
    ,FLUID_PARAM_F16_PRESSURE_SCALE = 14
    ,FLUID_PARAM_TB_FILL = 15
    ,FLUID_PARAM_TB_MIN_CELLS = 4
};

typedef struct fluid_ctx fluid_ctx;

const char *fluid_last_error(void);

int step(int N, float dt, float diff, float visc, float *u, float *v, float *dens);
int step_src(int N, float dt, float diff, float visc, int iters,
             float *u, float *v, float *dens,
             float *u_prev, float *v_prev, float *dens_prev);
int fluid_release_cached(void);

int fluid_coefficients(int N, float dt, float coef, float *alpha, float *beta);

typedef struct fluid_config {
    int n;
    int rank, nranks;
    int halo;
    int jacobi_variant;
    void *stream;
    void *arena;
    size_t arena_bytes;
    int storage;
} fluid_config;

enum { FLUID_STORAGE_F32 = 0, FLUID_STORAGE_F16 = 1 };

size_t fluid_arena_bytes(int N);
size_t fluid_arena_bytes_ex(int N, int storage);
int fluid_layout(int N, int *pitch, int *xoff, size_t *field_floats);

int fluid_create(int N, fluid_ctx **out);
int fluid_create_ex(const fluid_config *cfg, fluid_ctx **out);
int fluid_destroy(fluid_ctx *ctx);
int fluid_synchronize(fluid_ctx *ctx);

int fluid_create_ensemble(const fluid_config *cfg, int members, fluid_ctx **out);
size_t fluid_arena_bytes_ensemble(int N, int storage, int members);
int fluid_members(fluid_ctx *ctx, int *members);
int fluid_upload_member(fluid_ctx *ctx, int member, int field, const float *host);
int fluid_download_member(fluid_ctx *ctx, int member, int field, float *host);
int fluid_step_members(fluid_ctx *ctx, const float *dt, const float *diff, const float *visc, int iters,
                       int nsteps, int use_sources);
int fluid_vel_step_members(fluid_ctx *ctx, const float *dt, const float *visc, int iters);
int fluid_dens_step_members(fluid_ctx *ctx, const float *dt, const float *diff, int iters);
int fluid_op_add_source_members(fluid_ctx *ctx, int x, int s, const float *dt);
int fluid_op_jacobi_sweep_members(fluid_ctx *ctx, int b, int x, int x0, int out,
                                  const float *alpha, const float *beta);
int fluid_op_diffuse_members(fluid_ctx *ctx, int b, int x, int x0, const float *alpha, const float *beta,
                             int iters);
int fluid_op_advect_members(fluid_ctx *ctx, int b, int d, int d0, int u, int v, const float *dt);

int fluid_owned_rows(fluid_ctx *ctx, int *row_lo, int *row_hi);
int fluid_field_ptr(fluid_ctx *ctx, int field, void **dev_ptr);
int fluid_scalar_ptr(fluid_ctx *ctx, void **dev_ptr);

int fluid_upload(fluid_ctx *ctx, int field, const float *host);
int fluid_download(fluid_ctx *ctx, int field, float *host);
int fluid_upload_rows(fluid_ctx *ctx, int field, const float *host, int row_lo, int row_hi);
int fluid_download_rows(fluid_ctx *ctx, int field, float *host, int row_lo, int row_hi);
int fluid_fill(fluid_ctx *ctx, int field, float value);

int fluid_step(fluid_ctx *ctx, float dt, float diff, float visc, int iters,
               int nsteps, int use_sources);
int fluid_vel_step(fluid_ctx *ctx, float dt, float visc, int iters);
int fluid_dens_step(fluid_ctx *ctx, float dt, float diff, int iters);

int fluid_op_set_bnd(fluid_ctx *ctx, int b, int x);
int fluid_op_add_source(fluid_ctx *ctx, int x, int s, float dt);
int fluid_op_jacobi_sweep(fluid_ctx *ctx, int b, int x, int x0, int out,
                          float alpha, float beta);
int fluid_op_diffuse(fluid_ctx *ctx, int b, int x, int x0, float alpha, float beta,
                     int iters);
int fluid_op_advect(fluid_ctx *ctx, int b, int d, int d0, int u, int v, float dt);
int fluid_op_divergence(fluid_ctx *ctx, int u, int v, int p, int div);
int fluid_op_subtract_gradient(fluid_ctx *ctx, int u, int v, int p);

int fluid_residual(fluid_ctx *ctx, int x, int x0, float alpha, float beta, float *out);
int fluid_absmax_velocity(fluid_ctx *ctx, int u, int v, float *out);

int fluid_residual_members(fluid_ctx *ctx, int x, int x0, const float *alpha, const float *beta, float *out);
int fluid_absmax_velocity_members(fluid_ctx *ctx, int u, int v, float *out);
int fluid_member_moments(fluid_ctx *ctx, int field, double *sum, double *sumsq);
int fluid_ensemble_stats(fluid_ctx *ctx, int field, float *mean, float *variance);
int fluid_ensemble_stats_ptr(fluid_ctx *ctx, void **mean_dev, void **variance_dev);

int fluid_pack_members(fluid_ctx *ctx, int field, int first, int count, void *dst_dev, size_t member_stride);
int fluid_unpack_members(fluid_ctx *ctx, int field, int first, int count, const void *src_dev, size_t member_stride);
int fluid_download_members(fluid_ctx *ctx, int field, float *host);
int fluid_upload_members(fluid_ctx *ctx, int field, const float *host);
typedef struct fluid_run_plan {
    int iters, nsteps, use_sources;
    const void *sources;
    int every;
    const int *fields;
    int nfields;
    void *snapshots;
    size_t capacity;
} fluid_run_plan;
int fluid_run(fluid_ctx *ctx, float dt, float diff, float visc, const fluid_run_plan *plan, int *snapshots_written);
int fluid_run_members(fluid_ctx *ctx, const float *dt, const float *diff, const float *visc, const fluid_run_plan *plan,
                      int *snapshots_written);

int fluid_set_jacobi_variant(fluid_ctx *ctx, int variant);
int fluid_division_mode(fluid_ctx *ctx, float alpha, float beta, int *mode);
int fluid_plan_sweeps(int N, int rows, int storage, int pressure_form, int iters, int max_sweeps, int t16_min_cells,
                      int *depths, int capacity, int *count);
int fluid_autotune_pending(fluid_ctx *ctx, int *shapes_open);
int fluid_set_param(fluid_ctx *ctx, int key, int value);

enum {
    FLUID_TIME_SOURCE = 0, FLUID_TIME_DIFFUSION = 1, FLUID_TIME_DIVERGENCE = 2,
    FLUID_TIME_PROJECTION = 3, FLUID_TIME_ADVECTION = 4, FLUID_TIMING_CATEGORIES = 5
};
typedef struct fluid_timing {
    double jacobi_ms;
    long long sweeps;
    long long solves;
    double category_ms[FLUID_TIMING_CATEGORIES];
    long long category_calls[FLUID_TIMING_CATEGORIES];
    long long jacobi_launches;
    long long jacobi_field_launches;
    double pressure_ms;
    long long pressure_sweeps;
} fluid_timing;
int fluid_timing_enable(fluid_ctx *ctx, int on);
int fluid_timing_read(fluid_ctx *ctx, fluid_timing *out, int reset);

int fluid_op_diffuse_tol(fluid_ctx *ctx, int b, int x, int x0, float alpha, float beta,
                         float tol, int max_iters, int check_every,
                         int *iters_done, float *residual);

enum { FLUID_XCHG_HALO = 0, FLUID_XCHG_GATHER = 1, FLUID_XCHG_MAX = 2, FLUID_XCHG_MAX_BEGIN = 3,
       FLUID_XCHG_MAX_END = 4 };
typedef int (*fluid_exchange_fn)(void *user, int kind, const int *fields, int nfields,
                                 int depth, float *scalar);
int fluid_set_exchange(fluid_ctx *ctx, fluid_exchange_fn fn, void *user);
int fluid_exchange_stream(fluid_ctx *ctx, void **stream);
int fluid_split_launches(fluid_ctx *ctx, long long *count);
int fluid_exchange_now(fluid_ctx *ctx, int kind, const int *fields, int nfields, int depth);

#define FLUID_RCCL_ID_BYTES 128
int fluid_rccl_available(void);
int fluid_rccl_unique_id(void *id, size_t bytes);
int fluid_exchange_rccl_attach(fluid_ctx *ctx, const void *id, size_t bytes);
int fluid_exchange_rccl_attach_comm(fluid_ctx *ctx, void *nccl_comm);
int fluid_exchange_rccl_detach(fluid_ctx *ctx);
int fluid_exchange_rccl_calls(fluid_ctx *ctx, long long *halo, long long *gather, long long *max);

#ifdef __cplusplus
}
#endif
#endif
```

Baseline: 4.302 million.

## Fuse pressure gradient subtraction into final temporally blocked Jacobi pass

New measurement: 4.109 million. -4.5%, worse.

```diff
diff --git a/fluidsimulationcuda_amd/capi.py b/fluidsimulationcuda_amd/capi.py
--- a/fluidsimulationcuda_amd/capi.py
+++ b/fluidsimulationcuda_amd/capi.py
@@ -21,6 +21,7 @@
 PARAM_XCHG_OVERLAP = 13
 PARAM_F16_PRESSURE_SCALE = 14
 PARAM_TB_FILL = 15
+PARAM_FUSE_GRADIENT = 16
 XCHG_HALO, XCHG_GATHER, XCHG_MAX, XCHG_MAX_BEGIN, XCHG_MAX_END = 0, 1, 2, 3, 4
 RCCL_ID_BYTES = 128
 FIELD_NAMES = ("u", "v", "dens", "u_prev", "v_prev", "dens_prev", "tmp0", "tmp1", "tmp2", "tmp3", "tmp4", "tmp5")
@@ -102,6 +103,7 @@
     "fluid_op_advect": [_ctx, _i, _i, _i, _i, _i, _f],
     "fluid_op_divergence": [_ctx, _i, _i, _i, _i],
     "fluid_op_subtract_gradient": [_ctx, _i, _i, _i],
+    "fluid_op_project": [_ctx, _i, _i, _i, _i, _i],
     "fluid_residual": [_ctx, _i, _i, _f, _f, C.POINTER(_f)],
     "fluid_absmax_velocity": [_ctx, _i, _i, C.POINTER(_f)],
     "fluid_residual_members": [_ctx, _i, _i, _MF, _MF, _MF],
@@ -127,6 +129,7 @@
     "fluid_exchange_now": [_ctx, _i, C.POINTER(_i), _i, _i],
     "fluid_exchange_stream": [_ctx, C.POINTER(C.c_void_p)],
     "fluid_split_launches": [_ctx, C.POINTER(C.c_longlong)],
+    "fluid_gradient_launches": [_ctx, C.POINTER(C.c_longlong), C.POINTER(C.c_longlong)],
     "fluid_rccl_available": [],
     "fluid_rccl_unique_id": [C.c_void_p, C.c_size_t],
     "fluid_exchange_rccl_attach": [_ctx, C.c_void_p, C.c_size_t],
diff --git a/fluidsimulationcuda_amd/csrc/fluid_ctx.h b/fluidsimulationcuda_amd/csrc/fluid_ctx.h
--- a/fluidsimulationcuda_amd/csrc/fluid_ctx.h
+++ b/fluidsimulationcuda_amd/csrc/fluid_ctx.h
@@ -63,6 +63,7 @@
     int src_of = 0;
     MemberVal src_dt;
     float fscale = 1.0f;
+    bool doomed = false, dead = false;
 };
 
 struct ConstRing {
@@ -105,6 +106,7 @@
     bool xchg_overlap = true;
     unsigned xowed = 0;
     long long split_launches = 0;
+    long long grad_fused = 0, grad_separate = 0;
     bool early_advect = true;
     float vmax_prev[2] = {-1.0f, -1.0f};
     FieldState field[FLUID_NFIELDS];
@@ -134,6 +136,7 @@
     int fast_div = 2;
     int rank = 0, nranks = 1, own0 = 1, own1 = 1, min_slab = 0, halo = 1;
     bool fuse_add_source = true;
+    int fuse_gradient = -1;
     float pscale = 1.0f;
     fluid_exchange_fn xchg = nullptr;
     void* xchg_user = nullptr;
diff --git a/fluidsimulationcuda_amd/csrc/fluid_kernels.h b/fluidsimulationcuda_amd/csrc/fluid_kernels.h
--- a/fluidsimulationcuda_amd/csrc/fluid_kernels.h
+++ b/fluidsimulationcuda_amd/csrc/fluid_kernels.h
@@ -46,13 +46,21 @@
     size_t tile_mstride;
     const TbMemberK* mk;
 };
+struct TbGrad {
+    void* u;
+    void* v;
+    float h, pinv;
+    float r, hi, lo;
+    int out_dead;
+};
 
 void launch_set_bnd(hipStream_t s, int st, void* f, int pitch, int n, int b, Members mb = {});
+void launch_set_bnd2(hipStream_t s, int st, void* fa, int ba, void* fb, int bb, int pitch, int n, Members mb = {});
 void launch_add_source(hipStream_t s, int st, void* x, const void* src, int pitch, int row_lo, int row_hi, float dt, Members mb = {},
                        const float* mdt = nullptr);
 void launch_jacobi(hipStream_t s, int st, int variant, const void* x, const void* x0, void* out, int pitch, int n,
                    int row_lo, int row_hi, float alpha, float beta, int b, Members mb = {}, const float2* mab = nullptr);
-enum TbForm { TB_PLAIN = 0, TB_DIVSRC = 1, TB_ADDSRC = 2 };
+enum TbForm { TB_PLAIN = 0, TB_DIVSRC = 1, TB_ADDSRC = 2, TB_GRAD = 3 };
 struct TbShape { int T, divmode, nv, form; };
 inline constexpr TbShape kTbShapes[] = {
     {2, 0, 2, TB_PLAIN},   {2, 2, 2, TB_PLAIN},   {2, 3, 2, TB_PLAIN},   {2, 4, 2, TB_PLAIN},   {2, 5, 2, TB_PLAIN},
@@ -65,6 +73,7 @@
     {16, 0, 2, TB_PLAIN},  {16, 2, 2, TB_PLAIN},  {16, 3, 2, TB_PLAIN},  {16, 4, 2, TB_PLAIN},  {16, 5, 2, TB_PLAIN},
     {8, 4, 2, TB_DIVSRC},  {12, 4, 2, TB_DIVSRC}, {16, 4, 2, TB_DIVSRC}, {8, 0, 2, TB_ADDSRC},  {8, 2, 2, TB_ADDSRC},  {8, 5, 2, TB_ADDSRC},
     {12, 0, 2, TB_ADDSRC}, {12, 2, 2, TB_ADDSRC}, {12, 5, 2, TB_ADDSRC}, {16, 0, 2, TB_ADDSRC}, {16, 2, 2, TB_ADDSRC}, {16, 5, 2, TB_ADDSRC},
+    {8, 4, 2, TB_GRAD},    {12, 4, 2, TB_GRAD},   {16, 4, 2, TB_GRAD},
 };
 constexpr int kTbShapeCount = sizeof(kTbShapes) / sizeof(kTbShapes[0]);
 constexpr int jacobi_tb_index(int T, int divmode, int nv, int form)
@@ -80,11 +89,11 @@
 {
     return i == kTbShapeCount || (jacobi_tb_index(kTbShapes[i].T, kTbShapes[i].divmode, kTbShapes[i].nv, kTbShapes[i].form) == i && tb_shapes_unique(i + 1));
 }
-static_assert(kTbShapeCount == 52 && tb_shapes_unique(), "52 distinct shapes: adding or removing one is a change of this table");
+static_assert(kTbShapeCount == 55 && tb_shapes_unique(), "55 distinct shapes: adding or removing one is a change of this table");
 inline constexpr int kTbDepths[] = {16, 12, 8, 4, 2};
 constexpr bool is_tb_depth(int T) { for (int d : kTbDepths) if (d == T) return true; return false; }
 bool launch_jacobi_tb(hipStream_t s, int st, int T, int divmode, int nv, int form, const TbBatch& batch, int pitch, int n, int row_lo,
-                      int row_hi, int rb, int rb_edge, int hole_lo = 0, int hole_hi = 0, bool fill = true);
+                      int row_hi, int rb, int rb_edge, int hole_lo = 0, int hole_hi = 0, bool fill = true, const TbGrad* grad = nullptr);
 constexpr int kTileRows = 32, kTileCols = 64;
 inline int tile_rows(int n) { return (n + kTileRows - 1) / kTileRows; }
 inline int tile_pitch(int n) { return (n + kTileCols - 1) / kTileCols; }
diff --git a/fluidsimulationcuda_amd/csrc/fluid_kernels.hip b/fluidsimulationcuda_amd/csrc/fluid_kernels.hip
--- a/fluidsimulationcuda_amd/csrc/fluid_kernels.hip
+++ b/fluidsimulationcuda_amd/csrc/fluid_kernels.hip
@@ -87,10 +87,14 @@
 }
 
 template <typename S>
-__global__ __launch_bounds__(256) void k_set_bnd(S* __restrict__ f, int pitch, int n, int b, size_t ms)
+__global__ __launch_bounds__(256) void k_set_bnd(S* __restrict__ f, int pitch, int n, int b, size_t ms, S* __restrict__ f2, int b2)
 {
     const int k = 1 + blockIdx.x * 256 + threadIdx.x;
     if (k > n) return;
+    if (blockIdx.z == 1) {
+        f = f2;
+        b = b2;
+    }
     f += blockIdx.y * ms;
     const size_t P = (size_t)pitch;
     const bool nx = (b == 1), ny = (b == 2);
@@ -421,6 +425,12 @@
     int s_lo, s_hi;
     unsigned sx, sy;
     float x0_inc;
+    S* uc;
+    S* vc;
+    __amdgpu_buffer_rsrc_t bu, bv;
+    unsigned sg_off;
+    float gh, gpinv;
+    DivK gk;
     bool st_rg_lane, is_lg;
     bool fill;
 };
@@ -587,6 +597,41 @@
     return d;
 }
 
+template <typename S, int NV>
+__device__ __forceinline__ void tb_gradient(const Vec<NV>& p_up, const Vec<NV>& p_me, const Vec<NV>& p_dn, const Vec<NV>& u,
+                                            const Vec<NV>& v, const TbArgs<S, NV>& a, Vec<NV>& nu, Vec<NV>& nv)
+{
+    float gx[NV], gy[NV], qx[NV], qy[NV];
+#pragma unroll
+    for (int c = 0; c < NV; ++c) {
+        const float pr = c < NV - 1 ? p_me.c[c + 1] : lane_above0(p_me.c[0]);
+        const float pl = c > 0 ? p_me.c[c - 1] : lane_below0(p_me.c[NV - 1]);
+        gx[c] = 0.5f * (pr - pl);
+        gy[c] = 0.5f * (p_dn.c[c] - p_up.c[c]);
+    }
+    v2f nf = {0.f, 0.f};
+#pragma unroll
+    for (int p = 0; p < NV; p += 2) {
+        const v2f x = tb_div2<5>((v2f){gx[p], gx[p + 1]}, a.gk), y = tb_div2<5>((v2f){gy[p], gy[p + 1]}, a.gk);
+        qx[p] = x.x; qx[p + 1] = x.y;
+        qy[p] = y.x; qy[p + 1] = y.y;
+        nf = __builtin_elementwise_fma(x, (v2f){0.f, 0.f}, nf);
+        nf = __builtin_elementwise_fma(y, (v2f){0.f, 0.f}, nf);
+    }
+    if (__builtin_expect(__builtin_amdgcn_ballot_w64(__builtin_isunordered(nf.x, nf.y)) != 0ull, 0)) {
+#pragma unroll
+        for (int c = 0; c < NV; ++c) {
+            qx[c] = gx[c] / a.gh;
+            qy[c] = gy[c] / a.gh;
+        }
+    }
+#pragma unroll
+    for (int c = 0; c < NV; ++c) {
+        nu.c[c] = u.c[c] - qx[c] * a.gpinv;
+        nv.c[c] = v.c[c] - qy[c] * a.gpinv;
+    }
+}
+
 template <int NV>
 __device__ __forceinline__ Vec<NV> take(const Vec<NV>& v)
 {
@@ -620,8 +665,8 @@
 }
 
 template <int T, int DIVMODE, bool EDGE, bool WALL, bool GEN, int PH, typename S, int NV, bool DIVSRC = false, bool ADDSRC = false,
-          bool PART = false>
-__device__ __forceinline__ void tb_step(int t, Vec<NV> (&W)[T][3], Vec<NV> (&Q)[T + 1], Vec<NV> (&PX)[3], Vec<NV> (&PQ)[3],
+          bool GRAD = false, bool PART = false>
+__device__ __forceinline__ void tb_step(int t, Vec<NV> (&W)[T + (GRAD ? 1 : 0)][3], Vec<NV> (&Q)[T + 1], Vec<NV> (&PX)[3], Vec<NV> (&PQ)[3],
                                         const TbArgs<S, NV>& a, Vec<NV> (&UR)[3], Vec<NV> (&VR)[3], v2f& nf, int smax = T)
 {
     static_assert(!(PART && GEN), "the general body runs every stage");
@@ -683,7 +728,13 @@
                 for (int c = 0; c < NV; ++c) G.c[c] = __builtin_nondeterministic_value(W[s - 1][FR].c[c]);
             }
             if (s < T) W[s][FR] = G;
-            else tb_store<EDGE, WALL, S, NV>(G, q, run & (q >= a.q_lo) & (q < a.q_hi), a, v1, vn);
+            else {
+                tb_store<EDGE, WALL, S, NV>(G, q, run & (q >= a.q_lo) & (q < a.q_hi), a, v1, vn);
+                if constexpr (GRAD) {
+#pragma unroll
+                    for (int c = 0; c < NV; ++c) W[T][FR].c[c] = as_stored<S>(G.c[c]);
+                }
+            }
         }
     } else {
 #pragma unroll
@@ -706,22 +757,48 @@
             } else {
                 tb_sticky<DIVMODE, NV>(G, nf);
                 tb_store<EDGE, true, S, NV>(G, q, interior & (q >= a.q_lo) & (q < a.q_hi), a, v1, vn);
+                if constexpr (GRAD) {
+                    Vec<NV> gs;
+#pragma unroll
+                    for (int c = 0; c < NV; ++c) gs.c[c] = as_stored<S>(G.c[c]);
+                    const Vec<NV> me = W[T][ME];
+                    const Vec<NV> flipped_me = fxorv<NV>(me, a.sy), flipped_g = fxorv<NV>(gs, a.sy);
+                    const bool bot_ghost = (q == a.n + 1), top_ghost = (q == 1);
+#pragma unroll
+                    for (int c = 0; c < NV; ++c) {
+                        W[T][FR].c[c] = bot_ghost ? flipped_me.c[c] : gs.c[c];
+                        W[T][ME].c[c] = top_ghost ? flipped_g.c[c] : me.c[c];
+                    }
+                }
             }
         }
     }
+    if constexpr (GRAD) {
+        const int g = t - T - 1;
+        auto off = [&](int r) { return (((r >= a.q_lo) & (r < a.q_hi)) ? a.sg_off : kBufOff) + (unsigned)r * a.row_bytes; };
+        Vec<NV> nu, nv;
+        tb_gradient<S, NV>(W[T][UP], W[T][ME], W[T][FR], UR[PH], VR[PH], a, nu, nv);
+        buf_stv<NV>(a.uc, a.bu, off(g), nu);
+        buf_stv<NV>(a.vc, a.bv, off(g), nv);
+        __builtin_amdgcn_sched_barrier(0);
+        UR[PH] = buf_ldv<NV>(a.uc, a.bu, off(g + 3));
+        VR[PH] = buf_ldv<NV>(a.vc, a.bv, off(g + 3));
+    }
     tb_qshift<T, T + 1, NV>(Q);
 }
 
-template <int T, int DIVMODE, bool EDGE, bool WALL, typename S, int NV, bool DIVSRC = false, bool ADDSRC = false>
+template <int T, int DIVMODE, bool EDGE, bool WALL, typename S, int NV, bool DIVSRC = false, bool ADDSRC = false, bool GRAD = false>
 __device__ __forceinline__ bool tb_march(int t0, int t1, const TbArgs<S, NV>& a)
 {
-    Vec<NV> W[T][3], Q[T + 1], PX[3], PQ[3], UR[3], VR[3];
+    constexpr int TW = T + (GRAD ? 1 : 0);
+    constexpr int TC = T + (GRAD ? 1 : 0);
+    Vec<NV> W[TW][3], Q[T + 1], PX[3], PQ[3], UR[3], VR[3];
     v2f nf = {0.f, 0.f};
     Vec<NV> zero;
 #pragma unroll
     for (int c = 0; c < NV; ++c) zero.c[c] = 0.f;
 #pragma unroll
-    for (int s = 0; s < T; ++s) { W[s][0] = zero; W[s][1] = zero; W[s][2] = zero; }
+    for (int s = 0; s < TW; ++s) { W[s][0] = zero; W[s][1] = zero; W[s][2] = zero; }
 #pragma unroll
     for (int s = 0; s <= T; ++s) Q[s] = zero;
 #pragma unroll
@@ -733,54 +810,60 @@
         PQ[d] = buf_ldv<NV>(a.rc, a.br, off);
         buf_stv<NV>(a.oc, a.bo, kBufOff, zero);
         if constexpr (DIVSRC || ADDSRC) buf_stv<NV>(a.dc, a.bd, kBufOff, zero);
+        if constexpr (GRAD) {
+            buf_stv<NV>(a.uc, a.bu, kBufOff, zero);
+            buf_stv<NV>(a.vc, a.bv, kBufOff, zero);
+            UR[d] = buf_ldv<NV>(a.uc, a.bu, kBufOff);
+            VR[d] = buf_ldv<NV>(a.vc, a.bv, kBufOff);
+        }
         __builtin_amdgcn_sched_barrier(0);
     }
     int t = t0;
     if constexpr (WALL) {
-        for (; t <= t1 && t < T + 1; t += 3) {
-            tb_step<T, DIVMODE, EDGE, WALL, true, 0, S, NV, DIVSRC, ADDSRC>(t, W, Q, PX, PQ, a, UR, VR, nf);
-            tb_step<T, DIVMODE, EDGE, WALL, true, 1, S, NV, DIVSRC, ADDSRC>(t + 1, W, Q, PX, PQ, a, UR, VR, nf);
-            tb_step<T, DIVMODE, EDGE, WALL, true, 2, S, NV, DIVSRC, ADDSRC>(t + 2, W, Q, PX, PQ, a, UR, VR, nf);
-        }
-    }
-    const int fill_end = (a.fill && t0 == a.q_lo - T) ? t0 + 3 * ((2 * T + 2) / 3) : t0;
+        for (; t <= t1 && t < TC + 1; t += 3) {
+            tb_step<T, DIVMODE, EDGE, WALL, true, 0, S, NV, DIVSRC, ADDSRC, GRAD>(t, W, Q, PX, PQ, a, UR, VR, nf);
+            tb_step<T, DIVMODE, EDGE, WALL, true, 1, S, NV, DIVSRC, ADDSRC, GRAD>(t + 1, W, Q, PX, PQ, a, UR, VR, nf);
+            tb_step<T, DIVMODE, EDGE, WALL, true, 2, S, NV, DIVSRC, ADDSRC, GRAD>(t + 2, W, Q, PX, PQ, a, UR, VR, nf);
+        }
+    }
+    const int fill_end = (a.fill && t0 == a.q_lo - TC) ? t0 + 3 * ((2 * T + 2) / 3) : t0;
     const int full_end = a.fill ? t1 - 2 : t1;
     auto stages = [&](int u) { return u > t1 ? 0 : u < fill_end ? (u - t0) >> 1 : T; };
     for (; t <= t1 && t < fill_end && (!WALL || t + 1 <= a.n); t += 3) {
-        tb_step<T, DIVMODE, EDGE, WALL, false, 0, S, NV, DIVSRC, ADDSRC, true>(t, W, Q, PX, PQ, a, UR, VR, nf, stages(t));
-        tb_step<T, DIVMODE, EDGE, WALL, false, 1, S, NV, DIVSRC, ADDSRC, true>(t + 1, W, Q, PX, PQ, a, UR, VR, nf, stages(t + 1));
-        tb_step<T, DIVMODE, EDGE, WALL, false, 2, S, NV, DIVSRC, ADDSRC, true>(t + 2, W, Q, PX, PQ, a, UR, VR, nf, stages(t + 2));
+        tb_step<T, DIVMODE, EDGE, WALL, false, 0, S, NV, DIVSRC, ADDSRC, GRAD, true>(t, W, Q, PX, PQ, a, UR, VR, nf, stages(t));
+        tb_step<T, DIVMODE, EDGE, WALL, false, 1, S, NV, DIVSRC, ADDSRC, GRAD, true>(t + 1, W, Q, PX, PQ, a, UR, VR, nf, stages(t + 1));
+        tb_step<T, DIVMODE, EDGE, WALL, false, 2, S, NV, DIVSRC, ADDSRC, GRAD, true>(t + 2, W, Q, PX, PQ, a, UR, VR, nf, stages(t + 2));
     }
     for (; t <= full_end && (!WALL || t + 1 <= a.n); t += 3) {
-        tb_step<T, DIVMODE, EDGE, WALL, false, 0, S, NV, DIVSRC, ADDSRC>(t, W, Q, PX, PQ, a, UR, VR, nf);
-        tb_step<T, DIVMODE, EDGE, WALL, false, 1, S, NV, DIVSRC, ADDSRC>(t + 1, W, Q, PX, PQ, a, UR, VR, nf);
-        tb_step<T, DIVMODE, EDGE, WALL, false, 2, S, NV, DIVSRC, ADDSRC>(t + 2, W, Q, PX, PQ, a, UR, VR, nf);
+        tb_step<T, DIVMODE, EDGE, WALL, false, 0, S, NV, DIVSRC, ADDSRC, GRAD>(t, W, Q, PX, PQ, a, UR, VR, nf);
+        tb_step<T, DIVMODE, EDGE, WALL, false, 1, S, NV, DIVSRC, ADDSRC, GRAD>(t + 1, W, Q, PX, PQ, a, UR, VR, nf);
+        tb_step<T, DIVMODE, EDGE, WALL, false, 2, S, NV, DIVSRC, ADDSRC, GRAD>(t + 2, W, Q, PX, PQ, a, UR, VR, nf);
     }
     for (; t <= t1 && (!WALL || t + 1 <= a.n); t += 3) {
-        tb_step<T, DIVMODE, EDGE, WALL, false, 0, S, NV, DIVSRC, ADDSRC, true>(t, W, Q, PX, PQ, a, UR, VR, nf, stages(t));
-        tb_step<T, DIVMODE, EDGE, WALL, false, 1, S, NV, DIVSRC, ADDSRC, true>(t + 1, W, Q, PX, PQ, a, UR, VR, nf, stages(t + 1));
-        tb_step<T, DIVMODE, EDGE, WALL, false, 2, S, NV, DIVSRC, ADDSRC, true>(t + 2, W, Q, PX, PQ, a, UR, VR, nf, stages(t + 2));
+        tb_step<T, DIVMODE, EDGE, WALL, false, 0, S, NV, DIVSRC, ADDSRC, GRAD, true>(t, W, Q, PX, PQ, a, UR, VR, nf, stages(t));
+        tb_step<T, DIVMODE, EDGE, WALL, false, 1, S, NV, DIVSRC, ADDSRC, GRAD, true>(t + 1, W, Q, PX, PQ, a, UR, VR, nf, stages(t + 1));
+        tb_step<T, DIVMODE, EDGE, WALL, false, 2, S, NV, DIVSRC, ADDSRC, GRAD, true>(t + 2, W, Q, PX, PQ, a, UR, VR, nf, stages(t + 2));
     }
     if constexpr (WALL) {
         for (; t <= t1; t += 3) {
-            tb_step<T, DIVMODE, EDGE, WALL, true, 0, S, NV, DIVSRC, ADDSRC>(t, W, Q, PX, PQ, a, UR, VR, nf);
-            tb_step<T, DIVMODE, EDGE, WALL, true, 1, S, NV, DIVSRC, ADDSRC>(t + 1, W, Q, PX, PQ, a, UR, VR, nf);
-            tb_step<T, DIVMODE, EDGE, WALL, true, 2, S, NV, DIVSRC, ADDSRC>(t + 2, W, Q, PX, PQ, a, UR, VR, nf);
+            tb_step<T, DIVMODE, EDGE, WALL, true, 0, S, NV, DIVSRC, ADDSRC, GRAD>(t, W, Q, PX, PQ, a, UR, VR, nf);
+            tb_step<T, DIVMODE, EDGE, WALL, true, 1, S, NV, DIVSRC, ADDSRC, GRAD>(t + 1, W, Q, PX, PQ, a, UR, VR, nf);
+            tb_step<T, DIVMODE, EDGE, WALL, true, 2, S, NV, DIVSRC, ADDSRC, GRAD>(t + 2, W, Q, PX, PQ, a, UR, VR, nf);
         }
     }
     if constexpr (DIVMODE == 5) return __builtin_amdgcn_ballot_w64((nf.x != nf.x) | (nf.y != nf.y)) != 0ull;
     else return false;
 }
 
-template <int T, int DIVMODE, typename S, int NV, bool DIVSRC = false, bool ADDSRC = false>
+template <int T, int DIVMODE, typename S, int NV, bool DIVSRC = false, bool ADDSRC = false, bool GRAD = false>
 __device__ __forceinline__ bool tb_march_any(bool edge, bool wall, int t0, int t1, const TbArgs<S, NV>& a)
 {
     if (edge) {
-        if (wall) return tb_march<T, DIVMODE, true, true, S, NV, DIVSRC, ADDSRC>(t0, t1, a);
-        return tb_march<T, DIVMODE, true, false, S, NV, DIVSRC, ADDSRC>(t0, t1, a);
-    }
-    if (wall) return tb_march<T, DIVMODE, false, true, S, NV, DIVSRC, ADDSRC>(t0, t1, a);
-    return tb_march<T, DIVMODE, false, false, S, NV, DIVSRC, ADDSRC>(t0, t1, a);
+        if (wall) return tb_march<T, DIVMODE, true, true, S, NV, DIVSRC, ADDSRC, GRAD>(t0, t1, a);
+        return tb_march<T, DIVMODE, true, false, S, NV, DIVSRC, ADDSRC, GRAD>(t0, t1, a);
+    }
+    if (wall) return tb_march<T, DIVMODE, false, true, S, NV, DIVSRC, ADDSRC, GRAD>(t0, t1, a);
+    return tb_march<T, DIVMODE, false, false, S, NV, DIVSRC, ADDSRC, GRAD>(t0, t1, a);
 }
 
 struct TbGrid {
@@ -788,14 +871,17 @@
     int hole_lo, hole_hi;
 };
 
-constexpr int tb_waves_per_simd(int T, int NV) { return NV == 2 ? (T <= 8 ? 4 : T <= 12 ? 3 : 2) : (T <= 4 ? 3 : 2); }
-
-template <int T, int DIVMODE, int NV, typename S, bool DIVSRC = false, bool ADDSRC = false>
-__global__ __launch_bounds__(256, tb_waves_per_simd(T, NV)) void k_jacobi_tb(TbBatch batch, int pitch, int n, int row_lo,
-                                                                             int row_hi, int rb, int rb_edge, TbGrid g, int fill)
+constexpr int tb_cone(int T, bool grad) { return T + (grad ? 1 : 0); }
+constexpr int tb_waves_per_simd(int T, int NV, bool wide = false) { return NV == 2 ? (T <= 8 && !wide ? 4 : T <= 12 ? 3 : 2) : (T <= 4 ? 3 : 2); }
+
+template <int T, int DIVMODE, int NV, typename S, bool DIVSRC = false, bool ADDSRC = false, bool GRAD = false>
+__global__ __launch_bounds__(256, tb_waves_per_simd(T, NV, GRAD && sizeof(S) == 4)) void k_jacobi_tb(TbBatch batch, int pitch, int n, int row_lo,
+                                                                             int row_hi, int rb, int rb_edge, TbGrid g, int fill,
+                                                                             TbGrad gr)
 {
     static_assert(!DIVSRC || DIVMODE == 4, "the divergence-sourced launch is the first launch of a pressure solve");
     static_assert(!(DIVSRC && ADDSRC) && (!ADDSRC || DIVMODE != 3), "one second store per launch; mode 3's tiles are taken from the summed field");
+    static_assert(!GRAD || (DIVMODE == 4 && !DIVSRC && !ADDSRC), "the gradient-subtracting launch is the last launch of a pressure solve");
     const unsigned per_xcd = gridDim.x >> 3;
     unsigned vid = (blockIdx.x & 7u) * per_xcd + (blockIdx.x >> 3);
     if (vid >= (unsigned)(g.inner_blocks + g.edge_blocks)) return;
@@ -832,7 +918,8 @@
         if (DIVMODE == 3) tile_thr = mk->tile_thr;
     }
     const int b = batch.b[sv];
-    constexpr int HL = (T + NV - 1) / NV;
+    constexpr int TC = tb_cone(T, GRAD);
+    constexpr int HL = (TC + NV - 1) / NV;
     constexpr int VS = 64 - 2 * HL;
     constexpr int C0 = (XOFF + 1) / NV;
     static_assert((XOFF + 1) % NV == 0 && HL <= C0, "window overlap must fit the row's left pad");
@@ -870,7 +957,7 @@
         const unsigned field_bytes = (unsigned)((size_t)(n + 2) * (size_t)pitch * sizeof(S));
         a.bx = __builtin_amdgcn_make_buffer_rsrc(const_cast<S*>(x), 0, (batch.x_zero[sv] && !DIVSRC) ? 0u : field_bytes, 0x00020000);
         a.br = __builtin_amdgcn_make_buffer_rsrc(const_cast<S*>(x0), 0, field_bytes, 0x00020000);
-        a.bo = __builtin_amdgcn_make_buffer_rsrc(out, 0, field_bytes, 0x00020000);
+        a.bo = __builtin_amdgcn_make_buffer_rsrc(out, 0, (GRAD && gr.out_dead) ? 0u : field_bytes, 0x00020000);
         S* dv = (DIVSRC || ADDSRC) ? static_cast<S*>(batch.div[sv]) + mofs : out;
         a.dc = dv + cofs;
         a.bd = __builtin_amdgcn_make_buffer_rsrc(dv, 0, field_bytes, 0x00020000);
@@ -890,13 +977,29 @@
 #pragma unroll
     for (int c = 0; c < NV; ++c) a.m_r[c] = (is_rg && a.cg == c) ? 0xFFFFFFFFu : 0u;
     a.st_off = (ld_ok && (st_int || a.is_lg || a.st_rg_lane)) ? a.ld_off : kBufOff;
+    if constexpr (GRAD) {
+        const unsigned field_bytes = (unsigned)((size_t)(n + 2) * (size_t)pitch * sizeof(S));
+        S* gu = static_cast<S*>(gr.u) + mofs;
+        S* gv = static_cast<S*>(gr.v) + mofs;
+        a.sg_off = (ld_ok && st_int) ? a.ld_off : kBufOff;
+        a.uc = gu + cofs;
+        a.vc = gv + cofs;
+        a.bu = __builtin_amdgcn_make_buffer_rsrc(gu, 0, field_bytes, 0x00020000);
+        a.bv = __builtin_amdgcn_make_buffer_rsrc(gv, 0, field_bytes, 0x00020000);
+        a.gh = gr.h;
+        a.gpinv = gr.pinv;
+        a.gk.beta = gr.r;
+        a.gk.hi = gr.hi;
+        a.gk.lo = gr.lo;
+        a.gk.yd = 0.0;
+    }
     a.sx = (b == 1) ? 0x80000000u : 0u;
     a.sy = (b == 2) ? 0x80000000u : 0u;
     a.alpha = alpha;
     a.k.beta = beta;
     a.fill = fill != 0;
-    const int t0 = max(0, a.q_lo - T), t1 = a.q_hi - 1 + T;
-    const bool wall = (a.q_lo < T) || (a.q_hi - 1 + T > n + 1);
+    const int t0 = max(0, a.q_lo - TC), t1 = a.q_hi - 1 + TC;
+    const bool wall = (a.q_lo < TC) || (a.q_hi - 1 + TC > n + 1);
     constexpr int DM = DIVMODE == 3 ? 2 : DIVMODE;
     bool two_term = false;
     if constexpr (DIVMODE == 3) {
@@ -915,7 +1018,7 @@
     if (two_term) {
         tb_march_any<T, DIVMODE, S, NV>(edge, wall, t0, t1, a);
     } else {
-        const bool again = tb_march_any<T, DM, S, NV, DIVSRC, ADDSRC>(edge, wall, t0, t1, a);
+        const bool again = tb_march_any<T, DM, S, NV, DIVSRC, ADDSRC, GRAD>(edge, wall, t0, t1, a);
         if constexpr (DIVMODE == 5) {
             if (again) tb_march_any<T, 2, S, NV, false, ADDSRC>(edge, wall, t0, t1, a);
         }
@@ -1566,7 +1669,14 @@
 
 void launch_set_bnd(hipStream_t s, int st, void* f, int pitch, int n, int b, Members mb)
 {
-    FLUID_BY_STORAGE(st, hipLaunchKernelGGL(k_set_bnd<S>, dim3(cdiv(n, 256), mb.count), dim3(256), 0, s, (S*)f, pitch, n, b, mb.stride));
+    FLUID_BY_STORAGE(st, hipLaunchKernelGGL(k_set_bnd<S>, dim3(cdiv(n, 256), mb.count), dim3(256), 0, s, (S*)f, pitch, n, b, mb.stride,
+                                            (S*)nullptr, 0));
+}
+
+void launch_set_bnd2(hipStream_t s, int st, void* fa, int ba, void* fb, int bb, int pitch, int n, Members mb)
+{
+    FLUID_BY_STORAGE(st, hipLaunchKernelGGL(k_set_bnd<S>, dim3(cdiv(n, 256), mb.count, 2), dim3(256), 0, s, (S*)fa, pitch, n, ba, mb.stride,
+                                            (S*)fb, bb));
 }
 
 void launch_add_source(hipStream_t s, int st, void* x, const void* src, int pitch, int row_lo, int row_hi, float dt, Members mb,
@@ -1613,28 +1723,28 @@
     }
 }
 
-using TbKernel = void (*)(TbBatch, int, int, int, int, int, int, TbGrid, int);
+using TbKernel = void (*)(TbBatch, int, int, int, int, int, int, TbGrid, int, TbGrad);
 template <typename S, size_t... I>
 static std::array<TbKernel, kTbShapeCount> tb_kernels(std::index_sequence<I...>)
 {
     return {&k_jacobi_tb<kTbShapes[I].T, kTbShapes[I].divmode, kTbShapes[I].nv, S, kTbShapes[I].form == TB_DIVSRC,
-                         kTbShapes[I].form == TB_ADDSRC>...};
+                         kTbShapes[I].form == TB_ADDSRC, kTbShapes[I].form == TB_GRAD>...};
 }
 
 bool launch_jacobi_tb(hipStream_t s, int st, int T, int divmode, int nv, int form, const TbBatch& batch, int pitch, int n, int row_lo,
-                      int row_hi, int rb, int rb_edge, int hole_lo, int hole_hi, bool fill)
+                      int row_hi, int rb, int rb_edge, int hole_lo, int hole_hi, bool fill, const TbGrad* grad)
 {
     static const auto f32 = tb_kernels<float>(std::make_index_sequence<kTbShapeCount>());
     static const auto f16 = tb_kernels<half_t>(std::make_index_sequence<kTbShapeCount>());
     const int shape = jacobi_tb_index(T, divmode, nv, form);
-    if (shape < 0) return false;
+    if (shape < 0 || (form == TB_GRAD) != (grad != nullptr) || (grad && batch.count != 1)) return false;
     const int rows = row_hi - row_lo;
     if (rows <= 0 || batch.count <= 0 || batch.members <= 0) return true;
     if (hole_lo < row_lo) hole_lo = row_lo;
     if (hole_hi > row_hi) hole_hi = row_hi;
     const bool hole = hole_lo < hole_hi;
     if (hole && hole_lo == row_lo && hole_hi == row_hi) return true;
-    const int HL = (T + nv - 1) / nv, VS = 64 - 2 * HL;
+    const int HL = (tb_cone(T, form == TB_GRAD) + nv - 1) / nv, VS = 64 - 2 * HL;
     const unsigned nvec = (n + nv - 1) / nv;
     rb_edge = rb_edge < 1 ? rb : (rb_edge > rb ? rb : rb_edge);
     const int nwin = (int)cdiv(nvec, VS), kg = n / nv;
@@ -1652,7 +1762,7 @@
     g.edge_blocks = g.edge_wins * (int)cdiv(strips(rb_edge), 4);
     const dim3 grid(8 * cdiv(g.inner_blocks + g.edge_blocks, 8), 1, batch.count * batch.members), block(256);
     const TbKernel k = (st == STORAGE_F16 ? f16 : f32)[shape];
-    hipLaunchKernelGGL(k, grid, block, 0, s, batch, pitch, n, row_lo, row_hi, rb, rb_edge, g, fill ? 1 : 0);
+    hipLaunchKernelGGL(k, grid, block, 0, s, batch, pitch, n, row_lo, row_hi, rb, rb_edge, g, fill ? 1 : 0, grad ? *grad : TbGrad{});
     return true;
 }
 
diff --git a/fluidsimulationcuda_amd/csrc/fluid_solver.hip b/fluidsimulationcuda_amd/csrc/fluid_solver.hip
--- a/fluidsimulationcuda_amd/csrc/fluid_solver.hip
+++ b/fluidsimulationcuda_amd/csrc/fluid_solver.hip
@@ -6,6 +6,7 @@
 #include <cstdio>
 #include <cstring>
 #include <functional>
+#include <limits>
 #include <mutex>
 #include <new>
 #include <string>
@@ -357,7 +358,10 @@
     c->field[f].pend = false;
     c->field[f].src_of = 0;
     c->field[f].fscale = 1.0f;
-}
+    c->field[f].doomed = c->field[f].dead = false;
+}
+
+void doom(fluid_ctx* c, int f) { c->field[f].doomed = true; }
 
 void trade(fluid_ctx* c, int a, int b) { std::swap(c->field[a], c->field[b]); }
 
@@ -421,6 +425,7 @@
 
 int settle(fluid_ctx* c, int f, bool keep_scale = false)
 {
+    if (c->field[f].dead) return fail(FLUID_E_INVALID, "field %d was read while it holds nothing (its stores were left out)", f);
     if (!keep_scale) TRY(unscale(c, f));
     if (c->field[f].src_of) return settle_source(c, f);
     if (!c->field[f].pend) return FLUID_OK;
@@ -682,11 +687,17 @@
     int u, v;
     float scale;
 };
+struct GradSink {
+    int u, v;
+    bool p_dead;
+    bool done;
+};
 
 struct Batch {
     const Solve* sv;
     int count, iters, final_reach;
     const DivSource* ds;
+    GradSink* gs;
     int scratch_base;
     const int* scratch;
     const int* sum;
@@ -910,13 +921,14 @@
     return rb;
 }
 
-int launch_fused(fluid_ctx* c, const fluid::TbBatch& bt, int T, int divmode, bool divsrc, bool addsrc, int lo, int hi)
+int launch_fused(fluid_ctx* c, const fluid::TbBatch& bt, int T, int divmode, bool divsrc, bool addsrc, int lo, int hi,
+                 const fluid::TbGrad* grad = nullptr)
 {
     const bool owed = c->nranks > 1 && (c->xowed & stream_bit(c));
     const int in_lo = owed && c->rank > 0 ? std::max(lo, c->own0 + T) : lo;
     const int in_hi = owed && c->rank < c->nranks - 1 ? std::min(hi, c->own1 - T) : hi;
     const bool split = owed && in_hi - in_lo >= 2 * T && (in_lo > lo || in_hi < hi);
-    const int form = divsrc ? fluid::TB_DIVSRC : addsrc ? fluid::TB_ADDSRC : fluid::TB_PLAIN;
+    const int form = grad ? fluid::TB_GRAD : divsrc ? fluid::TB_DIVSRC : addsrc ? fluid::TB_ADDSRC : fluid::TB_PLAIN;
     for (int part = split ? 0 : 1; part < 2; ++part) {
         const int plo = part ? lo : in_lo, phi = part ? hi : in_hi;
         const int hole_lo = part && split ? in_lo : 0, hole_hi = part && split ? in_hi : 0;
@@ -926,12 +938,12 @@
         int trial = -1;
         unsigned long long key = 0;
         if (c->tb_rows <= 0 && c->autotune) {
-            key = tune_key(c, T, bt.count + (divsrc ? 8 : 0) + (addsrc ? 16 : 0) + (hole_hi > hole_lo ? 32 : 0), divmode, rows_n);
+            key = tune_key(c, T, bt.count + (divsrc ? 8 : 0) + (addsrc ? 16 : 0) + (hole_hi > hole_lo ? 32 : 0) + (grad ? 64 : 0), divmode, rows_n);
             rb = tune_pick(c, key, rb, T, rows_n, &trial, bt.count, form, divmode);
         }
         if (trial >= 0) TRY(tune_begin(c, key, trial));
         if (!fluid::launch_jacobi_tb(c->stream, c->st, T, divmode, c->tb_nv, form, bt, c->pitch, c->n, plo, phi, rb,
-                                     std::min(rb, edge_rows(c, T, rb)), hole_lo, hole_hi, c->tb_fill))
+                                     std::min(rb, edge_rows(c, T, rb)), hole_lo, hole_hi, c->tb_fill, grad))
             return fail(FLUID_E_INVALID, "no fused Jacobi kernel: %d sweeps, division mode %d, %d-column lanes, form %d", T, divmode, c->tb_nv, form);
         if (trial >= 0) TRY(tune_end(c));
     }
@@ -1006,7 +1018,20 @@
                 const bool divsrc = B.ds != nullptr && k == 0, addsrc = B.add_src && k == 0;
                 fluid::TbBatch bt;
                 TRY(fill_batch(c, B, first, last, divsrc, addsrc, &bt));
-                TRY(launch_fused(c, bt, T, B.plan[first][0].mode, divsrc, addsrc, lo, hi));
+                const bool grad = B.gs != nullptr && k + T == B.iters && !divsrc && B.count == 1 && !multi && B.plan[0][0].mode == 4 &&
+                                  fluid::jacobi_tb_exists(T, 4, c->tb_nv, fluid::TB_GRAD);
+                fluid::TbGrad tg{};
+                if (grad) {
+                    const float h = 1.0f / (float)c->n;
+                    const DivPlan over_h = division_mode(c, h, 0.0f);
+                    const bool proven = over_h.mode == 5;
+                    const float none = std::numeric_limits<float>::quiet_NaN();
+                    tg = {c->ptr(B.gs->u), c->ptr(B.gs->v), h, 1.0f / B.out_scale[0], proven ? over_h.arg : none, proven ? over_h.hi : none,
+                          proven ? over_h.lo : none, B.gs->p_dead ? 1 : 0};
+                    B.gs->done = true;
+                    c->grad_fused += 1;
+                }
+                TRY(launch_fused(c, bt, T, B.plan[first][0].mode, divsrc, addsrc, lo, hi, grad ? &tg : nullptr));
                 if (c->timing) {
                     c->launches += 1;
                     c->field_launches += (long long)(last - first) * c->members;
@@ -1021,9 +1046,9 @@
 }
 
 int op_diffuse_batch(fluid_ctx* c, const Solve* sv, int count, int iters, int final_reach = 0, const DivSource* ds = nullptr,
-                     int scratch_base = 0)
-{
-    Batch B{sv, count, iters, final_reach, ds, scratch_base};
+                     int scratch_base = 0, GradSink* gs = nullptr)
+{
+    Batch B{sv, count, iters, final_reach, ds, gs, scratch_base};
     TRY(batch_prepare(c, B));
     if (iters == 0) return FLUID_OK;
     hipEvent_t stop;
@@ -1039,10 +1064,11 @@
     return timing_end(c, stop, iters * count * c->members);
 }
 
-int op_diffuse(fluid_ctx* c, int b, int x, int x0, const Coeffs& k, int iters, int final_reach = 0, const DivSource* ds = nullptr)
+int op_diffuse(fluid_ctx* c, int b, int x, int x0, const Coeffs& k, int iters, int final_reach = 0, const DivSource* ds = nullptr,
+               GradSink* gs = nullptr)
 {
     const Solve one{b, x, x0, &k};
-    return op_diffuse_batch(c, &one, 1, iters, final_reach, ds);
+    return op_diffuse_batch(c, &one, 1, iters, final_reach, ds, 0, gs);
 }
 
 int vmax_begin(fluid_ctx* c, int u, int v, bool have_max = false)
@@ -1159,6 +1185,7 @@
     TRY(materialize(c, p, true));
     TRY(need(c, {p}, 1));
     with_max = with_max && c->nranks > 1 && c->d_partials;
+    c->grad_separate += 1;
     TIMED(c, FLUID_TIME_PROJECTION,
           fluid::launch_subtract_gradient(c->stream, c->st, c->ptr(u), c->ptr(v), c->ptr(p), c->pitch, c->n, c->own0, c->own1, h,
                                           c->d_partials, with_max ? c->d_scalar : nullptr, 1.0f / c->field[p].fscale, c->mb()));
@@ -1178,6 +1205,7 @@
     TRY(materialize(c, p, true));
     const float* mdt0 = nullptr;
     TRY(member_dt0(c, dt, &mdt0));
+    c->grad_separate += 1;
     TIMED(c, FLUID_TIME_PROJECTION,
           fluid::launch_gradient_advect(c->stream, c->st, c->ptr(u), c->ptr(v), c->ptr(p), c->ptr(d), c->ptr(d0), c->pitch, c->n, c->own0,
                                         c->own1, h, dt.at(0) * (float)c->n, b, 1.0f / c->field[p].fscale, c->mb(), mdt0));
@@ -1224,10 +1252,13 @@
     return division_mode(c, 4.0f, 1.0f).mode == 4;
 }
 
+constexpr long long kFuseGradientMinCells = 16000000;
+
 int project(fluid_ctx* c, int u, int v, int p, int div, int iters, const AdvectAfter* then_advect = nullptr, bool with_max = false)
 {
     const int reach = c->nranks > 1 ? std::max(0, std::min(std::min(iters, c->halo - 1), exchange_cap(c) - 1)) : 0;
     const bool fused = divergence_fuses(c, iters, reach);
+    const bool p_doomed = c->field[p].doomed;
     const DivSource ds{u, v, (-0.5f * (1.0f / (float)c->n)) * c->pscale};
     if (fused) {
         if (p == u || p == v || div == u || div == v || p == div)
@@ -1240,15 +1271,40 @@
     } else {
         TRY(op_divergence(c, u, v, p, div, std::min(iters, c->halo - 1), c->pscale));
     }
+    GradSink gs{u, v, p_doomed, false};
+    const int level = c->fuse_gradient >= 0 ? c->fuse_gradient : ((long long)c->n * c->n >= kFuseGradientMinCells ? 1 : 0);
+    const bool sink = level >= (then_advect ? 2 : 1) && c->nranks == 1 && c->variant == fluid::JACOBI_TB && u != v && p != u && p != v && div != u && div != v;
+    if (sink) TRY(materialize(c, {u, v}));
     c->in_pressure_solve = true;
     const Coeffs pressure{1.0f, 4.0f};
-    const int rc_solve = op_diffuse(c, 0, p, div, pressure, iters, 1, fused ? &ds : nullptr);
+    const int rc_solve = op_diffuse(c, 0, p, div, pressure, iters, 1, fused ? &ds : nullptr, sink ? &gs : nullptr);
     c->in_pressure_solve = false;
     TRY(rc_solve);
     if (fused) {
         TRY(xchg_join(c));
         wrote(c, div, 0);
         c->field[div].fscale = c->pscale;
+    }
+    if (gs.done) {
+        const AdvectAfter* a = then_advect;
+        if (a && (a->d == a->d0 || a->d == u || a->d == v || a->d == p || a->d0 == u || a->d0 == v))
+            return fail(FLUID_E_INVALID, "advect: output must not alias an input");
+        wrote(c, u, 0);
+        wrote(c, v, 0);
+        c->field[p].dead = gs.p_dead;
+        const float* mdt0 = nullptr;
+        if (a) {
+            TRY(materialize(c, a->d0));
+            TRY(member_dt0(c, a->dt, &mdt0));
+        }
+        TIMED(c, FLUID_TIME_PROJECTION, {
+            fluid::launch_set_bnd2(c->stream, c->st, c->ptr(u), 1, c->ptr(v), 2, c->pitch, c->n, c->mb());
+            if (a)
+                fluid::launch_advect(c->stream, c->st, c->ptr(a->d), c->ptr(a->d0), c->ptr(u), c->ptr(v), c->pitch, c->n, c->own0, c->own1,
+                                     a->dt.at(0) * (float)c->n, a->b, c->mb(), mdt0);
+        });
+        if (a) wrote(c, a->d, 0);
+        return FLUID_OK;
     }
     if (then_advect) return op_gradient_advect(c, u, v, p, then_advect->b, then_advect->d, then_advect->d0, then_advect->dt);
     return op_subtract_gradient(c, u, v, p, with_max);
@@ -1295,6 +1351,7 @@
     const Solve all[3] = {{1, U0, U, &cv}, {2, V0, V, &cv}, {0, D0, D, &cd}};
     if (c->nranks == 1) {
         TRY(op_diffuse_batch(c, all, 3, iters));
+        doom(c, U);
         TRY(project(c, U0, V0, U, V, iters));
         TRY(op_advect2(c, 1, U, U0, 2, V, V0, U0, V0, dt));
         const AdvectAfter dens{0, D, D0, dt};
@@ -1617,6 +1674,15 @@
     TRY(check_ctx(c));
     if (!count) return fail(FLUID_E_INVALID, "null pointer");
     *count = c->split_launches;
+    return FLUID_OK;
+}
+
+int fluid_gradient_launches(fluid_ctx* c, long long* fused, long long* separate)
+{
+    TRY(check_ctx(c));
+    if (!fused || !separate) return fail(FLUID_E_INVALID, "null output pointer");
+    *fused = c->grad_fused;
+    *separate = c->grad_separate;
     return FLUID_OK;
 }
 
@@ -1783,6 +1849,10 @@
     case FLUID_PARAM_FUSE_ADD_SOURCE:
         c->fuse_add_source = value != 0;
         return FLUID_OK;
+    case FLUID_PARAM_FUSE_GRADIENT:
+        if (value < -1 || value > 2) return fail(FLUID_E_INVALID, "FUSE_GRADIENT must be 0, 1 or 2, or -1 for the default rule");
+        c->fuse_gradient = value;
+        return FLUID_OK;
     case FLUID_PARAM_F16_PRESSURE_SCALE: {
         for (int f = 0; f < FLUID_NFIELDS; ++f) TRY(unscale(c, f));
         int e = 0;
@@ -2089,6 +2159,19 @@
     return FLUID_OK;
 }
 
+int fluid_op_project(fluid_ctx* c, int u, int v, int p, int div, int iters)
+{
+    TRY(check_ctx(c));
+    TRY(check_fields(c, {u, v, p, div}));
+    TRY(check_iters(iters));
+    for (int f : {u, v, p, div})
+        if (f >= FLUID_TMP0) return fail(FLUID_E_INVALID, "project: scratch fields are the solve's own");
+    if (u == v || p == div || p == u || p == v || div == u || div == v) return fail(FLUID_E_INVALID, "project: fields must be distinct");
+    TRY(project(c, u, v, p, div, iters));
+    HIP_TRY(hipGetLastError());
+    return FLUID_OK;
+}
+
 int fluid_residual(fluid_ctx* c, int x, int x0, float alpha, float beta, float* out)
 {
     TRY(check_ctx(c));
diff --git a/fluidsimulationcuda_amd/solver.py b/fluidsimulationcuda_amd/solver.py
--- a/fluidsimulationcuda_amd/solver.py
+++ b/fluidsimulationcuda_amd/solver.py
@@ -241,6 +241,9 @@
     def lastProject(self, u, v, p, div=None):
         capi.check(capi.lib().fluid_op_subtract_gradient(self._h, _fid(u), _fid(v), _fid(p)))
 
+    def project(self, u, v, p, div, iters=ITERS):
+        capi.check(capi.lib().fluid_op_project(self._h, _fid(u), _fid(v), _fid(p), _fid(div), iters))
+
     def vel_step(self, visc=VIS, dt=DT, iters=ITERS):
         self._call("vel_step", (), dict(dt=dt, visc=visc), (iters,))
 
@@ -326,6 +329,11 @@
         capi.check(capi.lib().fluid_op_diffuse_tol(self._h, b, _fid(x), _fid(x0), alpha, beta, tol, max_iters,
                                                    check_every, C.byref(it), C.byref(res)))
         return it.value, res.value
+
+    def gradient_launches(self):
+        a, b = C.c_longlong(), C.c_longlong()
+        capi.check(capi.lib().fluid_gradient_launches(self._h, C.byref(a), C.byref(b)))
+        return a.value, b.value
 
     def split_launches(self):
         m = C.c_longlong()
diff --git a/include/fluid_amd.h b/include/fluid_amd.h
--- a/include/fluid_amd.h
+++ b/include/fluid_amd.h
@@ -39,6 +39,7 @@
     ,FLUID_PARAM_XCHG_OVERLAP = 13
     ,FLUID_PARAM_F16_PRESSURE_SCALE = 14
     ,FLUID_PARAM_TB_FILL = 15
+    ,FLUID_PARAM_FUSE_GRADIENT = 16
     ,FLUID_PARAM_TB_MIN_CELLS = 4
 };
 
@@ -116,6 +117,7 @@
 int fluid_op_advect(fluid_ctx *ctx, int b, int d, int d0, int u, int v, float dt);
 int fluid_op_divergence(fluid_ctx *ctx, int u, int v, int p, int div);
 int fluid_op_subtract_gradient(fluid_ctx *ctx, int u, int v, int p);
+int fluid_op_project(fluid_ctx *ctx, int u, int v, int p, int div, int iters);
 
 int fluid_residual(fluid_ctx *ctx, int x, int x0, float alpha, float beta, float *out);
 int fluid_absmax_velocity(fluid_ctx *ctx, int u, int v, float *out);
@@ -179,6 +181,7 @@
 int fluid_set_exchange(fluid_ctx *ctx, fluid_exchange_fn fn, void *user);
 int fluid_exchange_stream(fluid_ctx *ctx, void **stream);
 int fluid_split_launches(fluid_ctx *ctx, long long *count);
+int fluid_gradient_launches(fluid_ctx *ctx, long long *fused, long long *separate);
 int fluid_exchange_now(fluid_ctx *ctx, int kind, const int *fields, int nfields, int depth);
 
 #define FLUID_RCCL_ID_BYTES 128
```
